# nju-websoft/OpenEA

Hardware: AMD Instinct MI355X
Metric: training triples/sec (k=10 truncated negatives + limited loss + Adagrad) (higher is better)
Workload: dtype f32; 1 GPU; BootEA/AlignE translational step, EN-FR-100K-V1 shape (synthetic), dim=100, GLOBAL batch=20000 positives (weak scaling: 20000 per GPU x 1 GPU), k=10, truncated eps=0.98; the same workload at every N (; global_batch=20000, entities=200000, parallelism=single

## Files before the change

### include/openea_hip.h

```cpp
#ifndef OPENEA_HIP_H
#define OPENEA_HIP_H

#include <stddef.h>
#include <stdint.h>

#ifdef __cplusplus
extern "C" {
#endif

#define OEA_OK 0
#define OEA_EINVAL (-1)
#define OEA_EHIP (-2)
#define OEA_ENOMEM (-3)
#define OEA_EUNSUPPORTED (-4)

int oea_version(void);
const char *oea_last_error(void);
int oea_device_count(void);

int oea_profile_begin(int32_t stride);
int oea_profile_end(int32_t group, double *out_ms_host, int32_t *n_calls_host);

typedef struct oea_store *oea_store_t;
int oea_store_create(int64_t rows, int32_t dim, oea_store_t *out);
// ... 6 lines not shown
int oea_store_save_host(oea_store_t s, float *dst_host, void *stream);

int oea_gather_rows(const float *table, int32_t dim, int32_t ld, const int32_t *ids, int64_t n,
                    int32_t normalize, float *out, int32_t out_ld, void *stream);
int oea_normalize_rows(float *table, int64_t rows, int32_t dim, int32_t ld, int32_t sk, void *stream);
int oea_fill_f32(float *p, int64_t n, float value, void *stream);
int oea_copy_to_host(const void *dev, void *host, size_t bytes, void *stream);
int oea_copy_from_host(void *dev, const void *host, size_t bytes, void *stream);

enum { OEA_LOSS_MARGIN = 0, OEA_LOSS_LIMITED = 1, OEA_LOSS_LOGISTIC = 2, OEA_LOSS_POSITIVE = 3,
       OEA_LOSS_ALIGN = 4 };
enum { OEA_OPT_SGD = 0, OEA_OPT_ADAGRAD = 1, OEA_OPT_ADAM = 2, OEA_OPT_ADADELTA = 3 };
enum { OEA_SCORE_TRANSE = 0, OEA_SCORE_TRANSH = 1, OEA_SCORE_TRANSD = 2 };

typedef struct oea_step_cfg {
    int32_t loss_kind;
    int32_t l1;
    float margin;
    float pos_margin;
    float neg_margin;
    float balance;
    int32_t ent_l2_norm;
    int32_t rel_l2_norm;
    int32_t opt_kind;
    float lr;
    int32_t neg_group_k;
    int32_t score_kind;
    float *normal;
    float *normal_acc;
    int32_t ent_transfer_base;
    int32_t rel_transfer_base;
    float beta1;
    float beta2;
    float eps;
    int32_t opt_t;
} oea_step_cfg;

size_t oea_step_workspace_bytes(int64_t n_ent, int64_t n_rel, int32_t ld);

int oea_triple_step(float *ent, float *ent_acc, int64_t n_ent, float *rel, float *rel_acc,
                    int64_t n_rel, int32_t dim, int32_t ld, const int32_t *pos, int64_t n_pos,
                    const int32_t *neg, int64_t n_neg, const oea_step_cfg *cfg, void *workspace,
                    double *loss_accum, void *stream);

enum { OEA_PHASE_BOTH = 0, OEA_PHASE_GRAD = 1, OEA_PHASE_APPLY = 2 };
size_t oea_step_exchange_floats(int64_t n_ent, int64_t n_rel, int32_t ld);
int32_t oea_step_scratch_elem_bytes(void);
int oea_triple_step_phase(float *ent, float *ent_acc, int64_t n_ent, float *rel, float *rel_acc,
                          int64_t n_rel, int32_t dim, int32_t ld, const int32_t *pos, int64_t n_pos,
                          const int32_t *neg, int64_t n_neg, const oea_step_cfg *cfg, void *workspace,
                          double *loss_accum, int32_t phase, void *stream);

int64_t oea_step_items(const oea_step_cfg *cfg, int64_t n_pos, int64_t n_neg);

int64_t oea_part_rows_per_rank(int64_t n_ent, int32_t world);
size_t oea_part_send_floats(int64_t n_ent, int32_t ld, int32_t world);
int oea_part_pack(void *workspace, int64_t n_ent, int64_t n_rel, int32_t ld, int32_t world, void *send, void *rel_x,
                  void *stream);
int oea_part_apply(float *ent, float *acc_own, int64_t n_ent, float *rel, float *rel_acc, int64_t n_rel, int32_t ld,
                   int32_t world, int32_t rank, void *own, void *rel_x, float *upd, const oea_step_cfg *cfg, void *workspace,
                   int64_t n_items, double *loss_accum, void *stream);
int oea_part_unpack(float *ent, int64_t n_ent, int32_t ld, int32_t world, int32_t rank, const float *all, void *stream);
int oea_step_normal_scratch(int64_t n_ent, int64_t n_rel, int32_t ld, int64_t *grad_offset_bytes, int64_t *touched_offset_bytes);
int oea_step_apply_normals(int64_t n_ent, int64_t n_rel, int32_t ld, const oea_step_cfg *cfg, void *workspace, void *stream);


int oea_step_scatter_ent_rows(void *workspace, int64_t n_ent, int64_t n_rel, int32_t ld, const int32_t *ids,
                              int64_t n, const float *src, int32_t src_ld, void *stream);

typedef struct oea_rotate_cfg {
    double gamma;
    double phase_scale;
    double lr;
    double beta1, beta2, eps;
    int64_t t;
    int32_t ent_l2_norm;
    int32_t rel_l2_norm;
    int32_t opt_kind;
    int32_t reserved;
} oea_rotate_cfg;
size_t oea_rotate_workspace_bytes(int64_t n_ent, int64_t n_rel, int32_t ld);
size_t oea_rotate_exchange_doubles(int64_t n_ent, int64_t n_rel, int32_t ld);
int oea_rotate_step(double *ent, double *ent_state, int64_t n_ent, double *rel, double *rel_state, int64_t n_rel,
                    int32_t dim, int32_t ld, const int32_t *pos, int64_t n_pos, const int32_t *neg, int64_t n_neg,
                    int32_t neg_group_k, const oea_rotate_cfg *cfg, void *workspace, double *loss_accum, int32_t phase,
                    void *stream);
int oea_rotate_lookup(const double *ent, int64_t n_ent, int32_t dim, int32_t ld, const int32_t *ids, int64_t n,
                      int32_t part_norm, int32_t sum_norm, float *out, int32_t out_ld, void *stream);

size_t oea_mapping_workspace_floats(int64_t n_links, int32_t ld, int32_t dim);
int oea_mapping_step(const float *ent, int32_t ld, int32_t dim, int32_t ent_l2_norm, const int32_t *ids1,
                     const int32_t *ids2, int64_t n, float *M, float *M_acc, float alpha, float lr, int32_t opt_kind,
                     void *ent_grad, void *ent_touched, float *work, double *loss_accum, void *stream);
int oea_mapping_epoch(float *ent, float *ent_acc, int64_t n_ent, float *rel, float *rel_acc, int64_t n_rel, int32_t dim,
                      int32_t ld, int32_t ent_l2_norm, const int32_t *batches, int32_t steps, int64_t n, float *M, float *M_acc,
                      float alpha, float lr, int32_t opt_kind, const oea_step_cfg *cfg, void *workspace, float *work,
                      double *mapping_loss_accum, double *step_loss_accum, void *stream);
size_t oea_sea_mapping_workspace_floats(int64_t n_l, int64_t n_u, int32_t ld, int32_t dim);
int oea_sea_mapping_step(const float *ent, int32_t ld, int32_t dim, const int32_t *ids_l1, const int32_t *ids_l2, int64_t n_l,
                         const int32_t *ids_u1, const int32_t *ids_u2, int64_t n_u, float *M1, float *M2, float *M_state,
                         float alpha_1, float alpha_2, const oea_step_cfg *cfg, void *ent_grad, void *ent_touched, float *work,
                         double *loss_accum, void *stream);
int oea_sea_mapping_epoch(float *ent, float *ent_acc, int64_t n_ent, float *rel, float *rel_acc, int64_t n_rel, int32_t dim,
                          int32_t ld, const int32_t *batches, int32_t steps, int64_t n_l, int64_t n_u, float *M1, float *M2,
                          float *M_state, float alpha_1, float alpha_2, const oea_step_cfg *cfg, void *workspace, float *work,
                          double *mapping_loss_accum, double *step_loss_accum, void *stream);
size_t oea_transr_workspace_bytes(int64_t n_ent, int64_t n_rel, int32_t dim, int64_t max_pos);
int oea_transr_step(float *ent, float *ent_acc, int64_t n_ent, float *rel, float *rel_acc, int64_t n_rel, float *rel_matrix,
                    float *rel_matrix_acc, int32_t dim, int32_t ld, const int32_t *pos, int64_t n_pos, const int32_t *neg,
                    int64_t n_neg, const oea_step_cfg *cfg, void *step_workspace, void *transr_workspace, double *loss_accum,
                    void *stream);
enum { OEA_SEMANTIC_HOLE = 0, OEA_SEMANTIC_SIMPLE = 1 };
int oea_semantic_step(int32_t model, float *ent, float *ent_acc, int64_t n_ent, float *rel, float *rel_acc, int64_t n_rel,
                      int32_t dim, int32_t ld, const int32_t *pos, int64_t n_pos, const int32_t *neg, int64_t n_neg,
                      const oea_step_cfg *cfg, void *step_workspace, double *loss_accum, void *stream);
int oea_step_entity_scratch(void *workspace, int64_t n_ent, int64_t n_rel, int32_t ld, void **ent_grad,
                            void **ent_touched);

uint64_t oea_tripleset_capacity(int64_t n);
int oea_tripleset_build(const int32_t *triples, int64_t n, uint64_t *table, uint64_t capacity,
                        void *stream);
int oea_sample_negatives(const int32_t *pos, int64_t n_pos, int32_t k, const uint64_t *table,
                         uint64_t capacity, const int32_t *entity_list, int32_t n_ent_list,
                         const int32_t *ent_pos, const int32_t *nbr, int32_t nbr_k, uint64_t seed,
                         uint32_t step, uint32_t pos_offset, int32_t max_try, int32_t *out,
                         int32_t *err_flag, void *stream);

int oea_sample_negatives_replay(const int32_t *pos, int64_t n_pos, int32_t k, const uint64_t *table, uint64_t capacity,
                                const int32_t *entity_list, int32_t n_ent_list, const int32_t *ent_pos, const int32_t *nbr,
                                int32_t nbr_k, int32_t max_try, const int32_t *replay, int32_t *out, int32_t *err_flag, void *stream);

typedef struct oea_sampler_side {
    const uint64_t *table;
    uint64_t capacity;
    const int32_t *entity_list;
    const int32_t *ent_pos;
    const int32_t *nbr;
    int32_t n_ent_list;
    int32_t nbr_k;
    const uint32_t *filter;
    uint64_t filter_bits;
} oea_sampler_side;
uint64_t oea_tripleset_filter_bits(uint64_t capacity);
int oea_tripleset_filter_build(const int32_t *triples, int64_t n, uint32_t *filter, uint64_t filter_bits, void *stream);
int oea_sample_negatives_pair(const int32_t *pos, int64_t n_pos, int64_t n_split, int32_t k,
                              const oea_sampler_side *side0, const oea_sampler_side *side1, uint64_t seed,
                              uint32_t step, uint32_t pos_offset, int32_t max_try, int32_t *out,
                              int32_t *err_flag, void *stream);

int oea_sample_negatives_epoch(const int32_t *pos_all, int64_t n_rows, const int64_t *offsets_dev,
                               const int64_t *splits_dev, int32_t steps, int32_t k, const oea_sampler_side *side0,
                               const oea_sampler_side *side1, uint64_t seed, uint32_t step_base, int32_t max_try,
                               int32_t *out_all, int32_t *err_flag, void *stream);

int oea_triple_epoch(float *ent, float *ent_acc, int64_t n_ent, float *rel, float *rel_acc, int64_t n_rel,
                     int32_t dim, int32_t ld, const int32_t *pos_all, const int64_t *offsets_host,
                     const int64_t *splits_host, int32_t steps, int32_t k, const oea_sampler_side *side0,
                     const oea_sampler_side *side1, uint64_t seed, uint32_t step_base, int32_t *neg_buf,
                     int32_t *err_flag, const oea_step_cfg *cfg, void *workspace, double *loss_accum,
                     const int64_t *offsets_dev, const int64_t *splits_dev, void *stream);
int oea_triple_epoch_range(float *ent, float *ent_acc, int64_t n_ent, float *rel, float *rel_acc, int64_t n_rel,
                           int32_t dim, int32_t ld, const int32_t *pos_all, const int64_t *offsets_host,
                           const int64_t *splits_host, int32_t steps, int32_t step_begin, int32_t step_end, int32_t k,
                           const oea_sampler_side *side0, const oea_sampler_side *side1, uint64_t seed,
                           uint32_t step_base, int32_t *neg_buf, int32_t *err_flag, const oea_step_cfg *cfg,
                           void *workspace, double *loss_accum, const int64_t *offsets_dev, const int64_t *splits_dev,
                           void *stream);

size_t oea_epoch_layout_bytes(int64_t n);
int oea_epoch_layout(const int32_t *triples, int64_t n1, int64_t n2, const int64_t *slot, int64_t n_slots, uint64_t seed, uint32_t epoch,
                     int32_t *dall, void *workspace, size_t ws_bytes, void *stream);

int32_t oea_step_plan_supported(const oea_step_cfg *cfg, int64_t n_ent, int64_t n_rel, int32_t ld, int32_t k);
size_t oea_step_plan_bytes(int64_t n_total, int32_t steps, int64_t max_batch, int64_t n_ent, int32_t ld);
int oea_step_plan_build(const int32_t *pos_all, const int32_t *neg_all, int32_t k, const int64_t *offsets_dev, int64_t n_total,
                        int32_t steps, int64_t max_batch, int64_t n_ent, int32_t ld, void *plan, size_t plan_bytes, void *stream);
int oea_step_plan_offsets(int64_t n_total, int32_t steps, int64_t max_batch, int64_t n_ent, int32_t ld, int64_t *out);
int oea_step_plan_rel_order_offset(int64_t n_total, int32_t steps, int64_t max_batch, int64_t n_ent, int32_t ld, int64_t *out);
int oea_triple_epoch_range_plan(float *ent, float *ent_acc, int64_t n_ent, float *rel, float *rel_acc, int64_t n_rel,
                                int32_t dim, int32_t ld, const int32_t *pos_all, const int64_t *offsets_host,
                                const int64_t *splits_host, int32_t steps, int32_t step_begin, int32_t step_end, int32_t k,
                                const oea_sampler_side *side0, const oea_sampler_side *side1, uint64_t seed,
                                uint32_t step_base, int32_t *neg_buf, int32_t *err_flag, const oea_step_cfg *cfg,
                                void *workspace, double *loss_accum, const int64_t *offsets_dev, const int64_t *splits_dev,
                                void *plan, size_t plan_bytes, int32_t plan_built, void *stream);

int oea_triple_epoch_range_shard(float *ent, float *ent_acc, int64_t n_ent, float *rel, float *rel_acc, int64_t n_rel,
                                 int32_t dim, int32_t ld, const int32_t *pos_all, const int64_t *offsets_host,
                                 const int64_t *splits_host, int32_t steps, int32_t step_begin, int32_t step_end, int32_t k,
                                 const oea_sampler_side *side0, const oea_sampler_side *side1, uint64_t seed,
                                 uint32_t step_base, int32_t *neg_buf, int32_t *err_flag, const oea_step_cfg *cfg,
                                 void *workspace, double *loss_accum, const int64_t *offsets_dev, const int64_t *splits_dev,
                                 int32_t rank, int32_t world, void *stream);

struct oea_comm;
int oea_triple_epoch_range_comm(struct oea_comm *comm, float *ent, float *acc_own, int64_t n_ent, float *rel, float *rel_acc,
                                int64_t n_rel, int32_t dim, int32_t ld, const int32_t *pos_all, const int64_t *offsets_host,
                                const int64_t *splits_host, int32_t steps, int32_t step_begin, int32_t step_end, int32_t k,
                                const oea_sampler_side *side0, const oea_sampler_side *side1, uint64_t seed, uint32_t step_base,
                                int32_t *neg_buf, int32_t *err_flag, const oea_step_cfg *cfg, void *workspace, double *loss_accum,
                                const int64_t *offsets_dev, const int64_t *splits_dev, void *send, void *own, void *rel_x,
                                float *upd, float *all, void *stream);


uint32_t oea_perm_index(uint32_t i, uint32_t n, uint32_t key);
int oea_sample_link_negatives(const int32_t *pos_links, int64_t n_pos, int32_t k, const int32_t *ents1, int32_t n1,
                              const int32_t *ents2, int32_t n2, const int32_t *nbr1, const int32_t *row1,
                              const int32_t *nbr2, const int32_t *row2, int32_t nbr_k, const uint64_t *exclude,
                              uint64_t exclude_cap, uint64_t seed, uint32_t step, int32_t *out_pairs, float *out_valid,
                              uint64_t *scratch_keys, int32_t *scratch_vals, uint64_t scratch_cap, void *stream);

int oea_greedy_matching(const int32_t *left, const int32_t *right, const float *weight, int64_t n_edges,
                        uint8_t *selected);
int oea_pair_dots(const float *e1, int32_t ld1, const float *e2, int32_t ld2, int32_t dim, const int32_t *ii,
                  const int32_t *jj, int64_t n, float *out, void *stream);

int oea_row_rank_select_f32(const float *vals, int64_t n_rows, int32_t nc, int64_t ld, int32_t k, int32_t largest, const int32_t *ids,
                            int64_t ld_ids, int32_t *out_sel, float *out_kth, void *stream);
int oea_row_rank_select_f64(const double *vals, int64_t n_rows, int32_t nc, int64_t ld, int32_t k, int32_t largest, const int32_t *ids,
                            int64_t ld_ids, int32_t *out_sel, double *out_kth, void *stream);

size_t oea_topk_workspace_bytes(int64_t nq, int64_t nc);
size_t oea_topk_sym_workspace_bytes(int64_t n, int32_t k);
int oea_topk_inner(const float *q, int64_t nq, int32_t ldq, const float *c, int64_t nc, int32_t ldc,
                   int32_t dim, int32_t k, const int32_t *id_map, int32_t *out_idx, void *workspace,
                   size_t ws_bytes, void *stream);

int oea_topk_rows(const float *s, int64_t n_rows, int64_t nc, int64_t ld, int32_t k, const int32_t *id_map,
                  int32_t *out_idx, void *stream);

enum { OEA_METRIC_INNER = 0, OEA_METRIC_MANHATTAN = 1, OEA_METRIC_EUCLIDEAN = 2,
       OEA_METRIC_MANHATTAN_F32 = 3  };
size_t oea_rank_workspace_bytes(int64_t n1);
int oea_rank_eval(const float *e1, int64_t n1, int32_t ld1, const float *e2, int64_t n2, int32_t ld2,
                  int32_t dim, int32_t metric, const float *csls_r, const float *csls_c, int64_t gold_offset,
                  int32_t *rank, int32_t *argmax, void *workspace, void *stream);
size_t oea_rank_eval_bf16_workspace_bytes(int64_t n1, int32_t dim);
int oea_rank_eval_bf16(const float *e1, int64_t n1, int32_t ld1, const float *e2, int64_t n2, int32_t ld2, int32_t dim,
                       int64_t gold_offset, int32_t *rank, int32_t *argmax, int32_t *status, void *workspace, void *stream);
int oea_rank_eval_bf16_csls(const float *e1, int64_t n1, int32_t ld1, const float *e2, int64_t n2, int32_t ld2, int32_t dim,
                            const float *csls_r, const float *csls_c, int64_t gold_offset, int32_t *rank, int32_t *argmax,
                            int32_t *status, void *workspace, void *stream);
int oea_rank_eval_metrics_bf16(const float *e1, int64_t n1, int32_t ld1, const float *e2, int64_t n2, int32_t ld2, int32_t dim,
                               const float *csls_r, const float *csls_c, int64_t gold_offset, const int32_t *top_k_host, int32_t nk,
                               int32_t *rank, int32_t *argmax, int64_t *out_dev, void *workspace, void *stream);
int oea_sim_bf16_matrix(const float *e1, int64_t n1, int32_t ld1, const float *e2, int64_t n2, int32_t ld2, int32_t dim, float *out,
                        int64_t ld_out, void *stream);
size_t oea_rank_eval_metrics_workspace_bytes(int64_t n1);
int oea_rank_eval_metrics(const float *e1, int64_t n1, int32_t ld1, const float *e2, int64_t n2, int32_t ld2, int32_t dim,
                          const float *csls_r, const float *csls_c, int64_t gold_offset, const int32_t *top_k_host, int32_t nk,
                          int32_t *rank, int32_t *argmax, int64_t *hits_and_rank_sum_dev, double *rr_sum_dev, void *workspace,
                          void *stream);
int oea_rank_metrics(const int32_t *rank, int64_t n, const int32_t *top_k_host, int32_t nk,
                     int64_t *hits_dev, int64_t *rank_sum_dev, double *rr_sum_dev, void *stream);

int oea_rank_rows(const float *s, int64_t n_rows, int64_t nc, int64_t ld, const int32_t *gold_idx,
                  int32_t *rank, int32_t *argmax, void *stream);

int oea_sim_matrix(const float *e1, int64_t n1, int32_t ld1, const float *e2, int64_t n2,
                   int32_t ld2, int32_t dim, int32_t metric, float *out, int64_t ld_out,
                   void *stream);
int oea_quantize_rows_u16(const float *src, int64_t n, int32_t ld, int32_t dim, float lo, float inv_step, uint16_t *dst,
                          int32_t ldq, void *stream);
int oea_l1_u16_strip(const uint16_t *q, int64_t nq, const uint16_t *c, int64_t nc, int32_t ldq, float *out, int64_t ld_out,
                     void *stream);
int oea_rank_l1_grid_rows(const float *strip, int64_t rows, int64_t row0, int64_t nc, int64_t ld, const float *e1, int32_t ld1,
                          const float *e2, int32_t ld2, int32_t dim, int64_t gold_offset, float step, float err, int32_t *rank,
                          int32_t *argmax, int32_t *n_exact_rows, void *stream);
int oea_rank_l1_grid_rows_csls(const float *strip, int64_t rows, int64_t row0, int64_t nc, int64_t ld, const float *e1, int32_t ld1,
                               const float *e2, int32_t ld2, int32_t dim, int64_t gold_offset, float step, float err,
                               const float *csls_r, const float *csls_c, int32_t *rank, int32_t *argmax, int32_t *n_exact_rows,
                               void *stream);
int oea_pair_l1_sim(const float *q, int64_t nq, int32_t ldq, const float *table, int64_t n, int32_t ldt, int32_t dim,
                    const int32_t *cand, int32_t c, float *out, void *stream);
int oea_pair_l1_f64(const float *q, int64_t nq, int32_t ldq, const float *table, int64_t n, int32_t ldt, int32_t dim,
                    const int32_t *cand, int32_t c, double *out, void *stream);

int oea_row_topk_mean(const float *s, int64_t n1, int64_t n2, int64_t ld, int32_t k, float *out,
                      void *stream);
size_t oea_csls_means_workspace_bytes(int64_t n1, int64_t n2, int32_t k);
int oea_csls_means(const float *e1, int64_t n1, int32_t ld1, const float *e2, int64_t n2, int32_t ld2, int32_t dim, int32_t k,
                   float *r_out, float *c_out, void *workspace, size_t ws_bytes, void *stream);
int oea_csls_apply(float *s, int64_t n1, int64_t n2, int64_t ld, const float *r, const float *c,
                   void *stream);

typedef struct oea_csr_split {
    const int32_t *chunk_row;
    const int32_t *chunk_e0;
    const int32_t *chunk_e1;
    const int32_t *rows;
    int32_t n_chunks, n_rows, threshold;
    const int32_t *row_chunk0;
    float *partials;
    int64_t partials_floats;
    uint32_t *tickets;
} oea_csr_split;
int oea_spmm_csr(const int32_t *rowptr, const int32_t *colidx, const float *vals, int64_t n_rows,
                 const float *x, int32_t dim, int32_t ldx, int32_t act, const float *mask_from,
                 float *y, int32_t ldy, const oea_csr_split *split, void *stream);

typedef struct oea_attn_graph {
    const int32_t *sub_ptr;
    const int32_t *sub_seg;
    const int32_t *seg_sub_ptr;
    const int32_t *seg_row;
    const int32_t *colidx;
    int64_t n_sub, n_seg, nnz;
    const int32_t *agg_rowptr;
    const int32_t *agg_colidx;
    const int32_t *agg_edge;
    int64_t agg_rows;
    const oea_csr_split *agg_split;
    const int32_t *t_rowptr;
    const int32_t *t_row;
    const int32_t *t_edge;
    int64_t t_rows;
    const oea_csr_split *t_split;
    int64_t sub0, sub1, seg0, seg1;
    int64_t agg_row0, agg_row1, agg_slot0, agg_slot1;
    int64_t t_row0, t_row1, t_slot0, t_slot1;
} oea_attn_graph;
#define OEA_ATTN_ALPHA 1
#define OEA_ATTN_AGGREGATE 2
#define OEA_ATTN_DZ 1
#define OEA_ATTN_DV 2
size_t oea_sparse_attn_workspace_floats(const oea_attn_graph *g);
int oea_sparse_attn_fwd(const oea_attn_graph *g, const float *z, const float *v, int32_t dim, int32_t ld,
                        float lrelu_slope, float *out, float *alpha, float *workspace, int32_t phases, void *stream);
int oea_sparse_attn_bwd(const oea_attn_graph *g, const float *z, const float *v, const float *alpha,
// ... 132 lines not shown
```

### openea_amd/_lib.py

```python
import ctypes as C
import os

_HERE = os.path.dirname(os.path.abspath(__file__))
DETERMINISTIC = os.environ.get("OEA_STEP_DETERMINISTIC", "0")[:1] == "1"
LIB_PATH = os.environ.get("OPENEA_HIP_LIB") or os.path.join(_HERE, "csrc",
                                                            "libopenea_hip_det.so" if DETERMINISTIC else "libopenea_hip.so")


class OpenEAHipError(RuntimeError):
    pass


class StepCfg(C.Structure):
    _fields_ = [("loss_kind", C.c_int32), ("l1", C.c_int32), ("margin", C.c_float),
                ("pos_margin", C.c_float), ("neg_margin", C.c_float), ("balance", C.c_float),
                ("ent_l2_norm", C.c_int32), ("rel_l2_norm", C.c_int32), ("opt_kind", C.c_int32),
                ("lr", C.c_float), ("neg_group_k", C.c_int32), ("score_kind", C.c_int32),
                ("normal", C.c_void_p), ("normal_acc", C.c_void_p),
                ("ent_transfer_base", C.c_int32), ("rel_transfer_base", C.c_int32),
                ("beta1", C.c_float), ("beta2", C.c_float), ("eps", C.c_float), ("opt_t", C.c_int32)]


class SamplerSide(C.Structure):
    _fields_ = [("table", C.c_void_p), ("capacity", C.c_uint64), ("entity_list", C.c_void_p),
                ("ent_pos", C.c_void_p), ("nbr", C.c_void_p), ("n_ent_list", C.c_int32), ("nbr_k", C.c_int32),
                ("filter", C.c_void_p), ("filter_bits", C.c_uint64)]


class CsrSplit(C.Structure):
    _fields_ = [("chunk_row", C.c_void_p), ("chunk_e0", C.c_void_p), ("chunk_e1", C.c_void_p), ("rows", C.c_void_p),
                ("n_chunks", C.c_int32), ("n_rows", C.c_int32), ("threshold", C.c_int32),
                ("row_chunk0", C.c_void_p), ("partials", C.c_void_p), ("partials_floats", C.c_int64), ("tickets", C.c_void_p)]


class AttnGraph(C.Structure):
    _fields_ = [("sub_ptr", C.c_void_p), ("sub_seg", C.c_void_p), ("seg_sub_ptr", C.c_void_p), ("seg_row", C.c_void_p),
                ("colidx", C.c_void_p), ("n_sub", C.c_int64), ("n_seg", C.c_int64), ("nnz", C.c_int64),
                ("agg_rowptr", C.c_void_p), ("agg_colidx", C.c_void_p), ("agg_edge", C.c_void_p), ("agg_rows", C.c_int64),
                ("agg_split", C.POINTER(CsrSplit)),
                ("t_rowptr", C.c_void_p), ("t_row", C.c_void_p), ("t_edge", C.c_void_p), ("t_rows", C.c_int64),
                ("t_split", C.POINTER(CsrSplit)),
                ("sub0", C.c_int64), ("sub1", C.c_int64), ("seg0", C.c_int64), ("seg1", C.c_int64),
                ("agg_row0", C.c_int64), ("agg_row1", C.c_int64), ("agg_slot0", C.c_int64), ("agg_slot1", C.c_int64),
                ("t_row0", C.c_int64), ("t_row1", C.c_int64), ("t_slot0", C.c_int64), ("t_slot1", C.c_int64)]


class GcnUnit(C.Structure):
    _fields_ = ([(pre + suf, t) for pre in ("a_", "at_", "f_", "ft_")
                 for suf, t in (("rowptr", C.c_void_p), ("colidx", C.c_void_p), ("vals", C.c_void_p), ("split", C.POINTER(CsrSplit)))]
                + [(nm, C.c_void_p) for nm in ("row_ids", "ill", "neg_left", "neg_right", "neg2_left", "neg2_right", "pair_rowptr",
                                               "pair_other", "pair_slot")]
                + [("n", C.c_int64), ("w_rows", C.c_int64), ("t", C.c_int64), ("dim", C.c_int32), ("ld", C.c_int32), ("k", C.c_int32),
                   ("gamma", C.c_float), ("lr", C.c_float)])


class GcnUnitBuffers(C.Structure):
    _fields_ = [(nm, C.c_void_p) for nm in ("t", "x", "h1", "out", "g_out", "g_pre1", "g_x", "g_t", "coef")]


class RotateCfg(C.Structure):
    _fields_ = [("gamma", C.c_double), ("phase_scale", C.c_double), ("lr", C.c_double), ("beta1", C.c_double),
                ("beta2", C.c_double), ("eps", C.c_double), ("t", C.c_int64), ("ent_l2_norm", C.c_int32),
                ("rel_l2_norm", C.c_int32), ("opt_kind", C.c_int32), ("reserved", C.c_int32)]


LOSS_KIND = {"margin-based": 0, "limited": 1, "logistic": 2, "positive": 3, "align": 4}
OPT_KIND = {"SGD": 0, "Adagrad": 1, "Adam": 2, "Adadelta": 3}
METRIC = {"inner": 0, "manhattan": 1, "euclidean": 2, "manhattan_f32": 3}

_vp, _i32, _i64, _u32, _u64, _f32, _sz = (C.c_void_p, C.c_int32, C.c_int64, C.c_uint32, C.c_uint64,
                                          C.c_float, C.c_size_t)

PROTOTYPES = {
    "oea_version": (C.c_int, []),
    "oea_last_error": (C.c_char_p, []),
    "oea_device_count": (C.c_int, []),
    "oea_profile_begin": (C.c_int, [_i32]),
    "oea_profile_end": (C.c_int, [_i32, C.POINTER(C.c_double), C.POINTER(_i32)]),
    "oea_store_create": (C.c_int, [_i64, _i32, C.POINTER(_vp)]),
    "oea_store_destroy": (C.c_int, [_vp]),
    "oea_store_rows": (_i64, [_vp]),
    "oea_store_dim": (_i32, [_vp]),
    "oea_store_ld": (_i32, [_vp]),
    "oea_store_rows_ptr": (_vp, [_vp]),
    "oea_store_load_host": (C.c_int, [_vp, _vp, _vp]),
    "oea_store_save_host": (C.c_int, [_vp, _vp, _vp]),
    "oea_gather_rows": (C.c_int, [_vp, _i32, _i32, _vp, _i64, _i32, _vp, _i32, _vp]),
    "oea_normalize_rows": (C.c_int, [_vp, _i64, _i32, _i32, _i32, _vp]),
    "oea_fill_f32": (C.c_int, [_vp, _i64, _f32, _vp]),
    "oea_copy_to_host": (C.c_int, [_vp, _vp, _sz, _vp]),
    "oea_copy_from_host": (C.c_int, [_vp, _vp, _sz, _vp]),
    "oea_step_workspace_bytes": (_sz, [_i64, _i64, _i32]),
    "oea_triple_step": (C.c_int, [_vp, _vp, _i64, _vp, _vp, _i64, _i32, _i32, _vp, _i64, _vp, _i64,
                                  C.POINTER(StepCfg), _vp, _vp, _vp]),
    "oea_step_exchange_floats": (_sz, [_i64, _i64, _i32]),
    "oea_step_scratch_elem_bytes": (_i32, []),
    "oea_triple_step_phase": (C.c_int, [_vp, _vp, _i64, _vp, _vp, _i64, _i32, _i32, _vp, _i64, _vp, _i64,
                                        C.POINTER(StepCfg), _vp, _vp, _i32, _vp]),
    "oea_part_rows_per_rank": (_i64, [_i64, _i32]),
    "oea_part_send_floats": (_sz, [_i64, _i32, _i32]),
    "oea_part_pack": (C.c_int, [_vp, _i64, _i64, _i32, _i32, _vp, _vp, _vp]),
    "oea_part_apply": (C.c_int, [_vp, _vp, _i64, _vp, _vp, _i64, _i32, _i32, _i32, _vp, _vp, _vp, C.POINTER(StepCfg), _vp, _i64,
                                 _vp, _vp]),
    "oea_step_normal_scratch": (C.c_int, [_i64, _i64, _i32, _vp, _vp]),
    "oea_step_apply_normals": (C.c_int, [_i64, _i64, _i32, _vp, _vp, _vp]),
    "oea_part_unpack": (C.c_int, [_vp, _i64, _i32, _i32, _i32, _vp, _vp]),
    "oea_step_scatter_ent_rows": (C.c_int, [_vp, _i64, _i64, _i32, _vp, _i64, _vp, _i32, _vp]),
    "oea_tripleset_capacity": (_u64, [_i64]),
    "oea_tripleset_build": (C.c_int, [_vp, _i64, _vp, _u64, _vp]),
    "oea_sample_negatives": (C.c_int, [_vp, _i64, _i32, _vp, _u64, _vp, _i32, _vp, _vp, _i32, _u64,
                                       _u32, _u32, _i32, _vp, _vp, _vp]),
    "oea_sample_negatives_replay": (C.c_int, [_vp, _i64, _i32, _vp, _u64, _vp, _i32, _vp, _vp, _i32, _i32, _vp, _vp, _vp, _vp]),
    "oea_tripleset_filter_bits": (C.c_uint64, [_u64]),
    "oea_tripleset_filter_build": (C.c_int, [_vp, _i64, _vp, _u64, _vp]),
    "oea_sample_negatives_pair": (C.c_int, [_vp, _i64, _i64, _i32, C.POINTER(SamplerSide), C.POINTER(SamplerSide),
                                            _u64, _u32, _u32, _i32, _vp, _vp, _vp]),
    "oea_sample_negatives_epoch": (C.c_int, [_vp, _i64, _vp, _vp, _i32, _i32, C.POINTER(SamplerSide),
                                             C.POINTER(SamplerSide), _u64, _u32, _i32, _vp, _vp, _vp]),
    "oea_triple_epoch": (C.c_int, [_vp, _vp, _i64, _vp, _vp, _i64, _i32, _i32, _vp, _vp, _vp, _i32, _i32,
                                   C.POINTER(SamplerSide), C.POINTER(SamplerSide), _u64, _u32, _vp, _vp,
                                   C.POINTER(StepCfg), _vp, _vp, _vp, _vp, _vp]),
    "oea_triple_epoch_range": (C.c_int, [_vp, _vp, _i64, _vp, _vp, _i64, _i32, _i32, _vp, _vp, _vp, _i32, _i32, _i32, _i32,
                                         C.POINTER(SamplerSide), C.POINTER(SamplerSide), _u64, _u32, _vp, _vp,
                                         C.POINTER(StepCfg), _vp, _vp, _vp, _vp, _vp]),
    "oea_triple_epoch_range_shard": (C.c_int, [_vp, _vp, _i64, _vp, _vp, _i64, _i32, _i32, _vp, _vp, _vp, _i32, _i32, _i32, _i32,
                                         C.POINTER(SamplerSide), C.POINTER(SamplerSide), _u64, _u32, _vp, _vp,
                                         C.POINTER(StepCfg), _vp, _vp, _vp, _vp, _i32, _i32, _vp]),
    "oea_epoch_layout_bytes": (_sz, [_i64]),
    "oea_epoch_layout": (C.c_int, [_vp, _i64, _i64, _vp, _i64, _u64, _u32, _vp, _vp, _sz, _vp]),
    "oea_step_plan_supported": (_i32, [C.POINTER(StepCfg), _i64, _i64, _i32, _i32]),
    "oea_step_plan_bytes": (_sz, [_i64, _i32, _i64, _i64, _i32]),
    "oea_step_plan_offsets": (C.c_int, [_i64, _i32, _i64, _i64, _i32, _vp]),
    "oea_step_plan_rel_order_offset": (C.c_int, [_i64, _i32, _i64, _i64, _i32, _vp]),
    "oea_step_plan_build": (C.c_int, [_vp, _vp, _i32, _vp, _i64, _i32, _i64, _i64, _i32, _vp, _sz, _vp]),
    "oea_triple_epoch_range_plan": (C.c_int, [_vp, _vp, _i64, _vp, _vp, _i64, _i32, _i32, _vp, _vp, _vp, _i32, _i32, _i32, _i32,
                                        C.POINTER(SamplerSide), C.POINTER(SamplerSide), _u64, _u32, _vp, _vp,
                                        C.POINTER(StepCfg), _vp, _vp, _vp, _vp, _vp, _sz, _i32, _vp]),
    "oea_triple_epoch_range_comm": (C.c_int, [_vp, _vp, _vp, _i64, _vp, _vp, _i64, _i32, _i32, _vp, _vp, _vp, _i32, _i32, _i32, _i32,
                                        C.POINTER(SamplerSide), C.POINTER(SamplerSide), _u64, _u32, _vp, _vp,
                                        C.POINTER(StepCfg), _vp, _vp, _vp, _vp, _vp, _vp, _vp, _vp, _vp, _vp]),
    "oea_rotate_workspace_bytes": (_sz, [_i64, _i64, _i32]),
    "oea_rotate_exchange_doubles": (_sz, [_i64, _i64, _i32]),
    "oea_rotate_step": (C.c_int, [_vp, _vp, _i64, _vp, _vp, _i64, _i32, _i32, _vp, _i64, _vp, _i64, _i32,
                                  C.POINTER(RotateCfg), _vp, _vp, _i32, _vp]),
    "oea_rotate_lookup": (C.c_int, [_vp, _i64, _i32, _i32, _vp, _i64, _i32, _i32, _vp, _i32, _vp]),
    "oea_mapping_workspace_floats": (_sz, [_i64, _i32, _i32]),
    "oea_mapping_step": (C.c_int, [_vp, _i32, _i32, _i32, _vp, _vp, _i64, _vp, _vp, C.c_float, C.c_float, _i32, _vp, _vp,
                                   _vp, _vp, _vp]),
    "oea_mapping_epoch": (C.c_int, [_vp, _vp, _i64, _vp, _vp, _i64, _i32, _i32, _i32, _vp, _i32, _i64, _vp, _vp, _f32, _f32, _i32,
                                    C.POINTER(StepCfg), _vp, _vp, _vp, _vp, _vp]),
    "oea_sea_mapping_workspace_floats": (_sz, [_i64, _i64, _i32, _i32]),
    "oea_sea_mapping_step": (C.c_int, [_vp, _i32, _i32, _vp, _vp, _i64, _vp, _vp, _i64, _vp, _vp, _vp, _f32, _f32, C.POINTER(StepCfg),
                                       _vp, _vp, _vp, _vp, _vp]),
    "oea_sea_mapping_epoch": (C.c_int, [_vp, _vp, _i64, _vp, _vp, _i64, _i32, _i32, _vp, _i32, _i64, _i64, _vp, _vp, _vp, _f32, _f32,
                                        C.POINTER(StepCfg), _vp, _vp, _vp, _vp, _vp]),
    "oea_step_entity_scratch": (C.c_int, [_vp, _i64, _i64, _i32, C.POINTER(C.c_void_p), C.POINTER(C.c_void_p)]),
    "oea_transr_workspace_bytes": (_sz, [_i64, _i64, _i32, _i64]),
    "oea_transr_step": (C.c_int, [_vp, _vp, _i64, _vp, _vp, _i64, _vp, _vp, _i32, _i32, _vp, _i64, _vp, _i64, C.POINTER(StepCfg),
                                  _vp, _vp, _vp, _vp]),
    "oea_semantic_step": (C.c_int, [_i32, _vp, _vp, _i64, _vp, _vp, _i64, _i32, _i32, _vp, _i64, _vp, _i64, C.POINTER(StepCfg),
                                    _vp, _vp, _vp]),
    "oea_greedy_matching": (C.c_int, [_vp, _vp, _vp, _i64, _vp]),
    "oea_pair_dots": (C.c_int, [_vp, _i32, _vp, _i32, _i32, _vp, _vp, _i64, _vp, _vp]),
    "oea_perm_index": (_u32, [_u32, _u32, _u32]),
    "oea_sample_link_negatives": (C.c_int, [_vp, _i64, _i32, _vp, _i32, _vp, _i32, _vp, _vp, _vp, _vp, _i32, _vp, _u64,
                                            _u64, _u32, _vp, _vp, _vp, _vp, _u64, _vp]),
    "oea_topk_sym_workspace_bytes": (_sz, [_i64, _i32]),
    "oea_topk_workspace_bytes": (_sz, [_i64, _i64]),
    "oea_topk_inner": (C.c_int, [_vp, _i64, _i32, _vp, _i64, _i32, _i32, _i32, _vp, _vp, _vp, _sz, _vp]),
    "oea_row_rank_select_f32": (C.c_int, [_vp, _i64, _i32, _i64, _i32, _i32, _vp, _i64, _vp, _vp, _vp]),
    "oea_row_rank_select_f64": (C.c_int, [_vp, _i64, _i32, _i64, _i32, _i32, _vp, _i64, _vp, _vp, _vp]),
    "oea_topk_rows": (C.c_int, [_vp, _i64, _i64, _i64, _i32, _vp, _vp, _vp]),
    "oea_rank_rows": (C.c_int, [_vp, _i64, _i64, _i64, _vp, _vp, _vp, _vp]),
    "oea_rank_workspace_bytes": (_sz, [_i64]),
    "oea_rank_eval": (C.c_int, [_vp, _i64, _i32, _vp, _i64, _i32, _i32, _i32, _vp, _vp, _i64, _vp, _vp, _vp, _vp]),
    "oea_quantize_rows_u16": (C.c_int, [_vp, _i64, _i32, _i32, C.c_float, C.c_float, _vp, _i32, _vp]),
    "oea_l1_u16_strip": (C.c_int, [_vp, _i64, _vp, _i64, _i32, _vp, _i64, _vp]),
    "oea_rank_l1_grid_rows": (C.c_int, [_vp, _i64, _i64, _i64, _i64, _vp, _i32, _vp, _i32, _i32, _i64, C.c_float, C.c_float, _vp, _vp, _vp, _vp]),
    "oea_pair_l1_f64": (C.c_int, [_vp, _i64, _i32, _vp, _i64, _i32, _i32, _vp, _i32, _vp, _vp]),
    "oea_rank_l1_grid_rows_csls": (C.c_int, [_vp, _i64, _i64, _i64, _i64, _vp, _i32, _vp, _i32, _i32, _i64, C.c_float, C.c_float, _vp, _vp,
                                             _vp, _vp, _vp, _vp]),
    "oea_pair_l1_sim": (C.c_int, [_vp, _i64, _i32, _vp, _i64, _i32, _i32, _vp, _i32, _vp, _vp]),
    "oea_rank_metrics": (C.c_int, [_vp, _i64, _vp, _i32, _vp, _vp, _vp, _vp]),
    "oea_rank_eval_bf16_workspace_bytes": (_sz, [_i64, _i32]),
    "oea_rank_eval_bf16": (C.c_int, [_vp, _i64, _i32, _vp, _i64, _i32, _i32, _i64, _vp, _vp, _vp, _vp, _vp]),
    "oea_rank_eval_bf16_csls": (C.c_int, [_vp, _i64, _i32, _vp, _i64, _i32, _i32, _vp, _vp, _i64, _vp, _vp, _vp, _vp, _vp]),
    "oea_sim_bf16_matrix": (C.c_int, [_vp, _i64, _i32, _vp, _i64, _i32, _i32, _vp, _i64, _vp]),
    "oea_rank_eval_metrics_bf16": (C.c_int, [_vp, _i64, _i32, _vp, _i64, _i32, _i32, _vp, _vp, _i64, _vp, _i32, _vp, _vp, _vp, _vp, _vp]),
    "oea_rank_eval_metrics_workspace_bytes": (_sz, [_i64]),
    "oea_rank_eval_metrics": (C.c_int, [_vp, _i64, _i32, _vp, _i64, _i32, _i32, _vp, _vp, _i64, _vp, _i32, _vp, _vp, _vp, _vp, _vp, _vp]),
    "oea_sim_matrix": (C.c_int, [_vp, _i64, _i32, _vp, _i64, _i32, _i32, _i32, _vp, _i64, _vp]),
    "oea_row_topk_mean": (C.c_int, [_vp, _i64, _i64, _i64, _i32, _vp, _vp]),
    "oea_csls_means_workspace_bytes": (_sz, [_i64, _i64, _i32]),
    "oea_csls_means": (C.c_int, [_vp, _i64, _i32, _vp, _i64, _i32, _i32, _i32, _vp, _vp, _vp, _sz, _vp]),
    "oea_csls_apply": (C.c_int, [_vp, _i64, _i64, _i64, _vp, _vp, _vp]),
    "oea_spmm_csr": (C.c_int, [_vp, _vp, _vp, _i64, _vp, _i32, _i32, _i32, _vp, _vp, _i32, C.POINTER(CsrSplit), _vp]),
    "oea_sparse_attn_workspace_floats": (_sz, [C.POINTER(AttnGraph)]),
    "oea_sparse_attn_fwd": (C.c_int, [C.POINTER(AttnGraph), _vp, _vp, _i32, _i32, _f32, _vp, _vp, _vp, _i32, _vp]),
    "oea_sparse_attn_bwd": (C.c_int, [C.POINTER(AttnGraph), _vp, _vp, _vp, _vp, _i32, _i32, _f32, _vp, _vp, _vp, _i32, _vp]),
    "oea_sparse_attn_dz": (C.c_int, [C.POINTER(AttnGraph), _vp, _vp, _vp, _f32, _vp, _vp]),
    "oea_concat_l2n_fwd": (C.c_int, [_vp, _vp, _vp, _i32, _i64, _vp, _i32, _vp, _vp, _vp]),
    "oea_concat_l2n_bwd": (C.c_int, [_vp, _vp, _vp, _i32, _i64, _vp, _vp, _i32, _vp, _vp, _vp]),
    "oea_pair_loss_l2_fwd": (C.c_int, [_vp, _i64, _i32, _i32, _vp, _i64, _i64, _vp, _f32, _f32, _vp, _vp, _vp]),
    "oea_pair_grad_rows": (C.c_int, [_vp, _i64, _i32, _i32, _vp, _vp, _vp, _vp, _vp, _i32, _vp, _vp]),
    "oea_align_loss_l1_coef": (C.c_int, [_vp, _i64, _i32, _i32, _vp, _i64, _i32, _f32, _vp, _vp, _vp, _vp, _vp, _vp, _vp, _vp]),
    "oea_segment_sum_f32": (C.c_int, [_vp, _vp, _vp, _i64, _vp, _vp]),
    "oea_pair_rows_build": (C.c_int, [_vp, _i64, _i64, _vp, _vp, _vp, _vp]),
    "oea_colsum_blocks": (_i32, [_i64]),
    "oea_highway_fwd": (C.c_int, [_vp, _vp, _vp, _vp, _vp, _i64, _i32, _vp, _vp]),
    "oea_highway_bwd": (C.c_int, [_vp, _vp, _vp, _vp, _vp, _vp, _vp, _i64, _i32, _vp, _vp, _vp, _vp, _vp]),
    "oea_gemm_tn_workspace_floats": (C.c_size_t, [_i64, _i32, _i32]),
    "oea_gemm_tn_f32": (C.c_int, [_vp, _i32, _i32, _vp, _i32, _i32, _i64, _vp, _i32, _vp, _vp]),
    "oea_gemm_tn_plan": (C.c_int, [_i64, _i32, _i32, C.POINTER(_i32), C.POINTER(_i64)]),
    "oea_gemm_tn_partial": (C.c_int, [_vp, _i32, _i32, _vp, _i32, _i32, _i64, _i32, _i32, _vp, _vp]),
    "oea_gemm_tn_reduce": (C.c_int, [_vp, _i32, _i32, _i32, _vp, _i32, _vp]),
    "oea_sigmoid_mix_fwd": (C.c_int, [_vp, _vp, _vp, _vp, _i64, _i32, _vp, _vp]),
    "oea_sigmoid_mix_bwd": (C.c_int, [_vp, _vp, _vp, _vp, _vp, _i64, _i32, _i32, _vp, _vp, _vp, _vp, _vp]),
    "oea_relu_axpy_fwd": (C.c_int, [_vp, _vp, C.c_float, _i64, _vp, _vp]),
    "oea_relu_axpy_bwd": (C.c_int, [_vp, _vp, C.c_float, _i64, _vp, _vp]),
    "oea_colsum_prod": (C.c_int, [_vp, _vp, _i64, _i32, _vp, _vp]),
    "oea_bias_tanh_fwd": (C.c_int, [_vp, _vp, _i64, _i32, _vp, _vp]),
    "oea_bias_tanh_bwd": (C.c_int, [_vp, _vp, _i64, _i32, _vp, _vp, _vp]),
    "oea_adam_dense": (C.c_int, [_vp, _vp, _vp, _vp, _i64, _f32, _f32, _f32, _f32, _i64, _vp]),
    "oea_align_loss_l1": (C.c_int, [_vp, _i64, _i32, _i32, _vp, _i64, _i32, _f32, _vp, _vp, _vp, _vp,
                                    _vp, _vp, _vp]),
    "oea_sgd_rows": (C.c_int, [_vp, _vp, _i64, _i32, _i32, _i32, _f32, _vp]),
    "oea_gcn_unit_epoch": (C.c_int, [C.POINTER(GcnUnit), _vp, C.POINTER(GcnUnitBuffers), _vp, _vp]),
    "oea_build_unweighted_adj": (C.c_int, [_vp, _i64, _i64, _vp, _vp, _vp, _i64, _vp, _vp]),
    "oea_build_weighted_adj": (C.c_int, [_vp, _i64, _i64, _i64, _vp, _vp, _vp, _vp, _vp, _vp, _vp, _vp, _vp, _i64, _vp, _vp]),
    "oea_build_primal_adj": (C.c_int, [_vp, _i64, _i64, _vp, _vp, _vp, _i64, _vp, _vp]),
    "oea_build_dual_adj": (C.c_int, [_vp, _i64, _i64, _vp, _vp]),
    "oea_build_2hop": (C.c_int, [_vp, _i64, _vp, _i64, _i64, _i64, _i32, _vp, _i64, _vp, C.POINTER(_i64), _vp]),
    "oea_comm_unique_id": (C.c_int, [_vp]),
    "oea_comm_init": (C.c_int, [_vp, _i32, _i32, C.POINTER(_vp)]),
    "oea_comm_destroy": (C.c_int, [_vp]),
    "oea_comm_rank": (_i32, [_vp]),
    "oea_comm_size": (_i32, [_vp]),
    "oea_allgather_rows": (C.c_int, [_vp, _vp, _vp, _i64, _i32, _vp]),
    "oea_comm_reduce_scatter_f32": (C.c_int, [_vp, _vp, _vp, _i64, _vp]),
    "oea_allreduce_f32": (C.c_int, [_vp, _vp, _i64, _vp]),
    "oea_allreduce_f64": (C.c_int, [_vp, _vp, _i64, _vp]),
    "oea_allreduce_i64": (C.c_int, [_vp, _vp, _i64, _vp]),
    "oea_comm_init_callbacks": (C.c_int, [_i32, _i32, _vp, _vp, C.POINTER(_vp)]),
    "oea_comm_allgather": (C.c_int, [_vp, _vp, _vp, _i64, _i32, _vp]),
    "oea_comm_reduce_scatter": (C.c_int, [_vp, _vp, _vp, _i64, _i32, _vp]),
    "oea_comm_allreduce": (C.c_int, [_vp, _vp, _i64, _i32, _vp]),
    "oea_step_items": (_i64, [C.POINTER(StepCfg), _i64, _i64]),
    "oea_comm_set_alltoallv": (C.c_int, [_vp, _vp]),
    "oea_comm_alltoallv": (C.c_int, [_vp, _vp, _vp, _vp, _vp, _vp, _vp, _i32, _vp]),
    "oea_halo_workspace_bytes": (_sz, [_i64, _i32, _i32, _i64, _i32]),
    "oea_halo_buffer_bytes": (_sz, [_i64, _i32, _i64, _i32, _i32]),
    "oea_halo_plan": (C.c_int, [_vp, _vp, _i32, _vp, _vp, _i32, _i32, _i32, _i64, _i32, _vp, _sz, _vp, _vp, C.POINTER(_i64), _vp]),
    "oea_triple_epoch_range_halo": (C.c_int, [_vp, _vp, _vp, _i64, _vp, _vp, _i64, _i32, _i32, _vp, _vp, _vp, _i32, _i32, _i32, _i32,
                                        C.POINTER(SamplerSide), C.POINTER(SamplerSide), _u64, _u32, _vp, _vp,
                                        C.POINTER(StepCfg), _vp, _vp, _vp, _vp, _vp, _sz, _vp, _vp, _sz, _vp, _vp, _vp, _vp, _vp]),
    "oea_comm_profile_begin": (C.c_int, [_vp]),
    "oea_comm_profile_end": (C.c_int, [_vp, C.POINTER(C.c_double), C.POINTER(_i32)]),
}

COMM_CALLBACK = C.CFUNCTYPE(C.c_int, _vp, _i32, _vp, _vp, _i64, _i32, _vp)
COMM_ALLTOALLV_CALLBACK = C.CFUNCTYPE(C.c_int, _vp, _vp, C.POINTER(_i64), C.POINTER(_i64), _vp, C.POINTER(_i64), C.POINTER(_i64), _i32, _vp)
COMM_ALLREDUCE, COMM_ALLGATHER, COMM_REDUCE_SCATTER = 0, 1, 2
COMM_F32, COMM_F64, COMM_I64 = 0, 1, 2
COMM_PHASES = ("grad", "pack", "reduce_scatter", "apply", "all_gather", "unpack")

_lib = None


def load(require_device=True):
    global _lib
    if _lib is None:
        if not os.path.exists(LIB_PATH):
            raise OpenEAHipError(
                "libopenea_hip.so not found at %s -- run `python -c 'import __graft_entry__ as g; "
                "g.build()'` (there is no CPU fallback)" % LIB_PATH)
        try:
            lib = C.CDLL(LIB_PATH)
        except OSError as e:
            raise OpenEAHipError("cannot load %s: %s" % (LIB_PATH, e))
        for name, (res, args) in PROTOTYPES.items():
            fn = getattr(lib, name)
            fn.restype = res
            fn.argtypes = args
        _lib = lib
    if require_device and _lib.oea_device_count() <= 0:
        raise OpenEAHipError("no HIP device visible: the OpenEA hot path runs on MI355X only "
                             "(there is no CPU fallback)")
# ... 8 lines not shown
```

### openea_amd/csrc/sampler.hip

```cpp
#include <stdlib.h>

#include <algorithm>

#include "common.h"

namespace {

__global__ void tripleset_clear(uint64_t *table, uint64_t capacity) {
    for (uint64_t i = (uint64_t)blockIdx.x * blockDim.x + threadIdx.x; i < capacity; i += (uint64_t)gridDim.x * blockDim.x)
        table[i] = OEA_EMPTY_KEY;
}

__global__ void tripleset_insert(const int32_t *__restrict__ triples, int64_t n, uint64_t *table, uint64_t capacity) {
    for (int64_t i = (int64_t)blockIdx.x * blockDim.x + threadIdx.x; i < n; i += (int64_t)gridDim.x * blockDim.x) {
        const uint64_t key = oea::pack_triple((uint32_t)triples[3 * i], (uint32_t)triples[3 * i + 1], (uint32_t)triples[3 * i + 2]);
        uint64_t s = oea::mix64(key) & (capacity - 1);
        for (;;) {
            const unsigned long long prev = atomicCAS((unsigned long long *)&table[s], (unsigned long long)OEA_EMPTY_KEY, (unsigned long long)key);
            if (prev == OEA_EMPTY_KEY || prev == key) break;
            s = (s + 1) & (capacity - 1);
        }
    }
}

__device__ __forceinline__ uint64_t filter_bit(uint64_t key, uint64_t bits) { return oea::mix64(key ^ 0x9E3779B97F4A7C15ull) & (bits - 1); }

__global__ void tripleset_filter_insert(const int32_t *__restrict__ triples, int64_t n, uint32_t *__restrict__ filter, uint64_t bits) {
    for (int64_t i = (int64_t)blockIdx.x * blockDim.x + threadIdx.x; i < n; i += (int64_t)gridDim.x * blockDim.x) {
        const uint64_t b = filter_bit(oea::pack_triple((uint32_t)triples[3 * i], (uint32_t)triples[3 * i + 1], (uint32_t)triples[3 * i + 2]), bits);
        atomicOr(&filter[b >> 5], 1u << (b & 31));
    }
}

__device__ __forceinline__ bool contains(const uint64_t *__restrict__ table, uint64_t capacity, const uint32_t *__restrict__ filter,
                                         uint64_t filter_bits, uint32_t h, uint32_t r, uint32_t t) {
    const uint64_t key = oea::pack_triple(h, r, t);
    if (filter) {
        const uint64_t b = filter_bit(key, filter_bits);
        if (!((filter[b >> 5] >> (b & 31)) & 1u)) return false;
    }
    uint64_t s = oea::mix64(key) & (capacity - 1);
    for (;;) {
        const uint64_t cur = table[s];
        if (cur == key) return true;
        if (cur == OEA_EMPTY_KEY) return false;
        s = (s + 1) & (capacity - 1);
    }
}

constexpr int kMaxK = 64;

template <int G>
__global__ __launch_bounds__(256) void sample_negatives_kernel(
    const int32_t *__restrict__ pos, int64_t n_pos, int64_t n_split, int k, oea_sampler_side side0,
    oea_sampler_side side1, uint32_t k0, uint32_t k1, uint32_t step, uint32_t pos_offset,
    int max_try, int32_t *__restrict__ out, int32_t *__restrict__ err_flag,
    const int64_t *__restrict__ seg_off, const int64_t *__restrict__ seg_split, int n_seg, const int32_t *__restrict__ replay) {
    const int lane = threadIdx.x % G;
    const uint32_t step_in = step;
    const int64_t n_split_in = n_split;
    for (int64_t p = ((int64_t)blockIdx.x * blockDim.x + threadIdx.x) / G; p < n_pos; p += (int64_t)gridDim.x * blockDim.x / G) {
    step = step_in;
    n_split = n_split_in;
    int64_t pl = p;
    if (seg_off) {
        const int64_t p0 = ((int64_t)(uint32_t)__builtin_amdgcn_readfirstlane((int)(p >> 32)) << 32) | (uint32_t)__builtin_amdgcn_readfirstlane((int)p);
        int lo = 0, hi = n_seg;
        while (hi - lo > 1) {
            const int mid = (lo + hi) >> 1;
            if (seg_off[mid] <= p0) lo = mid; else hi = mid;
        }
        int64_t first = seg_off[lo], split = seg_split[lo];
        int seg = lo;
        if (p >= seg_off[lo + 1]) {
            int l2 = lo;
            hi = n_seg;
            while (hi - l2 > 1) {
                const int mid = (l2 + hi) >> 1;
                if (seg_off[mid] <= p) l2 = mid; else hi = mid;
            }
            seg = l2; first = seg_off[l2]; split = seg_split[l2];
        }
        pl = p - first;
        n_split = split;
        step += (uint32_t)seg;
    }
    const oea_sampler_side &sd = pl < n_split ? side0 : side1;
    const uint64_t *__restrict__ table = sd.table;
    const uint64_t capacity = sd.capacity;
    const int32_t *__restrict__ entity_list = sd.entity_list;
    const int32_t *__restrict__ ent_pos = sd.ent_pos;
    const int32_t *__restrict__ nbr = sd.nbr;
    const uint32_t *__restrict__ filter = sd.filter;
    const uint64_t filter_bits = sd.filter_bits;
    const int n_ent_list = sd.n_ent_list, nbr_k = sd.nbr_k;
    const int32_t h = pos[3 * p], r = pos[3 * p + 1], t = pos[3 * p + 2];
    const bool h_has = nbr && ent_pos[h] >= 0, t_has = nbr && ent_pos[t] >= 0;
    const int32_t *hc = h_has ? nbr + (int64_t)ent_pos[h] * nbr_k : entity_list;
    const int32_t *tc = t_has ? nbr + (int64_t)ent_pos[t] * nbr_k : entity_list;
    const int hn = h_has ? nbr_k : n_ent_list, tn = t_has ? nbr_k : n_ent_list;
    const uint32_t c0 = (uint32_t)pl + pos_offset;
    const int gbase = (threadIdx.x & 63) / G * G;
    const unsigned long long gmask = (G == 64 ? ~0ull : ((1ull << G) - 1ull)) << gbase;
    int got = 0;
    for (int tr = 0; tr < max_try && got < k; ++tr) {
        const bool spare = k < G;
        uint4 w = oea::philox4x32_10(c0, step, (uint32_t)tr, (spare && lane != G - 1) ? 1u + (uint32_t)lane : 0u, k0, k1);
        const uint32_t side_word = spare ? (uint32_t)__shfl((int)w.x, (int)((threadIdx.x & 63) / G * G) + G - 1, 64) : w.x;
        const int32_t *rp = replay ? replay + ((int64_t)p * max_try + tr) * (1 + k) : nullptr;
        const bool corrupt_head = rp ? rp[0] != 0 : (side_word & 1u) != 0u;
        const int32_t *cand = corrupt_head ? hc : tc;
        const int nc = corrupt_head ? hn : tn;
        const int need = k - got;
        if (need > nc) { if (lane == 0) *err_flag = 1; break; }
        const bool active = lane < need;
        uint32_t att = 0;
        int32_t v = -1 - lane;
        if (active) {
            if (!spare) w = oea::philox4x32_10(c0, step, (uint32_t)tr, 1u + (uint32_t)lane, k0, k1);
            v = rp ? rp[1 + lane] : (int32_t)__umulhi(w.x, (uint32_t)nc);
            if (rp && (v < 0 || v >= nc)) { *err_flag = 2; v = 0; }
        }
        for (;;) {
            bool conflict = false;
            for (int q = 0; q < need; ++q) {
                const int32_t vq = __shfl(v, gbase + q, 64);
                conflict |= (q < lane) && (vq == v);
            }
            conflict &= active;
            if ((__ballot(conflict) & gmask) == 0ull) break;
            if (conflict) {
                ++att;
                w = oea::philox4x32_10(c0, step, (uint32_t)tr, 1u + (uint32_t)lane + 64u * att, k0, k1);
                v = (int32_t)__umulhi(w.x, (uint32_t)nc);
            }
        }
        bool accept = false;
        int32_t nh = h, nt = t;
        if (active) {
            const int32_t e = cand[v];
            nh = corrupt_head ? e : h;
            nt = corrupt_head ? t : e;
            accept = (tr == max_try - 1) || !contains(table, capacity, filter, filter_bits, (uint32_t)nh, (uint32_t)r, (uint32_t)nt);
        }
        const unsigned long long acc_mask = (__ballot(accept) & gmask) >> gbase;
        if (accept) {
            const int slot = got + __popcll(acc_mask & ((1ull << lane) - 1ull));
            struct __attribute__((packed, aligned(4))) Triple { int32_t h, r, t; };
            *reinterpret_cast<Triple *>(out + ((int64_t)p * k + slot) * 3) = Triple{nh, r, nt};
        }
        got += __popcll(acc_mask);
    }
    }
}

}

extern "C" {

uint64_t oea_tripleset_capacity(int64_t n) {
    uint64_t cap = 16;
    while (cap < 2ull * (uint64_t)(n > 1 ? n : 1)) cap *= 2;
    return cap;
}

int oea_tripleset_build(const int32_t *triples, int64_t n, uint64_t *table, uint64_t capacity, void *stream) {
    OEA_REQUIRE(table && (triples || n == 0), "null pointer");
    OEA_REQUIRE(capacity >= 2ull * (uint64_t)n && (capacity & (capacity - 1)) == 0, "capacity: power of two >= 2n");
    hipStream_t st = oea::as_stream(stream);
    tripleset_clear<<<1024, 256, 0, st>>>(table, capacity);
    if (n > 0) tripleset_insert<<<(unsigned)std::min<int64_t>(oea::ceil_div(n, 256), 4096), 256, 0, st>>>(triples, n, table, capacity);
    OEA_CHECK_HIP(hipGetLastError());
    return OEA_OK;
}

uint64_t oea_tripleset_filter_bits(uint64_t capacity) { return 8ull * capacity; }

int oea_tripleset_filter_build(const int32_t *triples, int64_t n, uint32_t *filter, uint64_t filter_bits, void *stream) {
    OEA_REQUIRE(filter && (triples || n == 0), "null pointer");
    OEA_REQUIRE(filter_bits >= 32 && (filter_bits & (filter_bits - 1)) == 0, "filter_bits: a power of two >= 32");
    hipStream_t st = oea::as_stream(stream);
    OEA_CHECK_HIP(hipMemsetAsync(filter, 0, (size_t)(filter_bits / 8), st));
    if (n > 0) tripleset_filter_insert<<<(unsigned)std::min<int64_t>(oea::ceil_div(n, 256), 4096), 256, 0, st>>>(triples, n, filter, filter_bits);
    OEA_CHECK_HIP(hipGetLastError());
    return OEA_OK;
}

int oea_sample_negatives(const int32_t *pos, int64_t n_pos, int32_t k, const uint64_t *table,
                         uint64_t capacity, const int32_t *entity_list, int32_t n_ent_list,
                         const int32_t *ent_pos, const int32_t *nbr, int32_t nbr_k, uint64_t seed,
                         uint32_t step, uint32_t pos_offset, int32_t max_try, int32_t *out,
                         int32_t *err_flag, void *stream) {
    oea_sampler_side sd{};
    sd.table = table; sd.capacity = capacity; sd.entity_list = entity_list; sd.ent_pos = ent_pos; sd.nbr = nbr;
    sd.n_ent_list = n_ent_list; sd.nbr_k = nbr_k;
    return oea_sample_negatives_pair(pos, n_pos, n_pos, k, &sd, &sd, seed, step, pos_offset, max_try, out, err_flag,
                                     stream);
}

static int check_side(const oea_sampler_side *s, int k) {
    OEA_REQUIRE(s && s->table && s->entity_list, "sampler side: null pointer");
    OEA_REQUIRE(s->nbr == nullptr || (s->ent_pos != nullptr && s->nbr_k > 0), "nbr needs ent_pos and nbr_k");
    OEA_REQUIRE((s->nbr ? s->nbr_k : s->n_ent_list) >= k && s->n_ent_list >= k, "Sample larger than population");
    return OEA_OK;
}

static int sample_impl(const int32_t *pos, int64_t n_pos, int64_t n_split, int32_t k,
                       const oea_sampler_side *side0, const oea_sampler_side *side1, uint64_t seed,
                       uint32_t step, uint32_t pos_offset, int32_t max_try, int32_t *out,
                       int32_t *err_flag, const int64_t *seg_off_dev, const int64_t *seg_split_dev, int n_seg,
                       void *stream, const int32_t *replay = nullptr) {
    OEA_REQUIRE(pos && out && err_flag, "null pointer");
    OEA_REQUIRE(k >= 1 && k <= kMaxK, "1 <= k <= 64");
    OEA_REQUIRE(max_try >= 1, "max_try >= 1");
    OEA_REQUIRE(n_split >= 0 && n_split <= n_pos, "0 <= n_split <= n_pos");
    int rc = check_side(side0, k);
    if (rc != OEA_OK) return rc;
    rc = check_side(side1, k);
    if (rc != OEA_OK) return rc;
    if (n_pos == 0) return OEA_OK;
    hipStream_t st = oea::as_stream(stream);
    static const int64_t cap_env = [] { const char *e = getenv("OEA_SAMPLER_CAP"); return e ? (int64_t)atoll(e) : (int64_t)0; }();
    const int64_t cap = (seg_off_dev && cap_env > 0) ? cap_env : ((int64_t)1 << 30);
    if (k <= 16)
        sample_negatives_kernel<16><<<(unsigned)std::min<int64_t>(oea::ceil_div(n_pos, 256 / 16), cap), 256, 0, st>>>(
            pos, n_pos, n_split, k, *side0, *side1, (uint32_t)seed, (uint32_t)(seed >> 32), step, pos_offset, max_try,
            out, err_flag, seg_off_dev, seg_split_dev, n_seg, replay);
    else
        sample_negatives_kernel<64><<<(unsigned)std::min<int64_t>(oea::ceil_div(n_pos, 256 / 64), cap), 256, 0, st>>>(
            pos, n_pos, n_split, k, *side0, *side1, (uint32_t)seed, (uint32_t)(seed >> 32), step, pos_offset, max_try,
            out, err_flag, seg_off_dev, seg_split_dev, n_seg, replay);
    OEA_CHECK_HIP(hipGetLastError());
    return OEA_OK;
}

int oea_sample_negatives_pair(const int32_t *pos, int64_t n_pos, int64_t n_split, int32_t k,
                              const oea_sampler_side *side0, const oea_sampler_side *side1, uint64_t seed,
                              uint32_t step, uint32_t pos_offset, int32_t max_try, int32_t *out,
                              int32_t *err_flag, void *stream) {
    return sample_impl(pos, n_pos, n_split, k, side0, side1, seed, step, pos_offset, max_try, out, err_flag, nullptr,
                       nullptr, 0, stream);
}

int oea_sample_negatives_replay(const int32_t *pos, int64_t n_pos, int32_t k, const uint64_t *table, uint64_t capacity,
                                const int32_t *entity_list, int32_t n_ent_list, const int32_t *ent_pos, const int32_t *nbr,
                                int32_t nbr_k, int32_t max_try, const int32_t *replay, int32_t *out, int32_t *err_flag, void *stream) {
    OEA_REQUIRE(replay, "replay record");
    oea_sampler_side sd{};
    sd.table = table; sd.capacity = capacity; sd.entity_list = entity_list; sd.ent_pos = ent_pos; sd.nbr = nbr;
    sd.n_ent_list = n_ent_list; sd.nbr_k = nbr_k;
    return sample_impl(pos, n_pos, n_pos, k, &sd, &sd, 0, 0u, 0u, max_try, out, err_flag, nullptr, nullptr, 0, stream, replay);
}

int oea_sample_negatives_epoch(const int32_t *pos_all, int64_t n_rows, const int64_t *offsets_dev,
                               const int64_t *splits_dev, int32_t steps, int32_t k, const oea_sampler_side *side0,
                               const oea_sampler_side *side1, uint64_t seed, uint32_t step_base, int32_t max_try,
                               int32_t *out_all, int32_t *err_flag, void *stream) {
    OEA_REQUIRE(offsets_dev && splits_dev && steps >= 1, "offsets / splits / steps");
    return sample_impl(pos_all, n_rows, 0, k, side0, side1, seed, step_base, 0u, max_try, out_all, err_flag, offsets_dev,
                       splits_dev, steps, stream);
}

}
```

### openea_amd/csrc/step_plan.h

```cpp
#pragma once
#include <hip/hip_runtime.h>
#include <stddef.h>
#include <stdint.h>

namespace oea {

struct StepPlanView {
    uint64_t *keys_a, *keys_b;
    uint32_t *vals_a, *vals_b;
    uint64_t *ukeys;
    uint32_t *ucount;
    uint32_t *uoff;
    int32_t *n_unique;
    int32_t *step_first;
    uint32_t *pflags;
    uint4 *recs;
    uint8_t *inplan;
    float *contrib;
    void *temp;
    size_t temp_bytes;
    uint32_t *rel_order;
    int row_bits;
};

constexpr uint32_t kPlanHubEntries = 8;

size_t step_plan_layout(int64_t n_total, int32_t steps, int64_t max_batch, int64_t n_ent, int32_t ld, void *base, StepPlanView *v);

}
```

### openea_amd/csrc/step_plan.hip

```cpp
#include <string.h>

#include <rocprim/rocprim.hpp>

#include <algorithm>

#include "common.h"
#include "step_plan.h"

namespace oea {

static size_t al256(size_t x) { return (x + 255) / 256 * 256; }
static int bits_for(uint64_t max_value) { int b = 1; while (b < 64 && (max_value >> b) != 0) ++b; return b; }

size_t step_plan_layout(int64_t n_total, int32_t steps, int64_t max_batch, int64_t n_ent, int32_t ld, void *base, StepPlanView *v) {
    const size_t m = (size_t)std::max<int64_t>(2 * n_total, 1);
    size_t off = 0;
    char *b = static_cast<char *>(base);
    auto take = [&](size_t bytes) { size_t o = off; off += al256(bytes); return b ? b + o : nullptr; };
    StepPlanView w{};
    w.keys_a = (uint64_t *)take(8 * m);
    w.keys_b = (uint64_t *)take(8 * m);
    w.vals_a = (uint32_t *)take(4 * m);
    w.vals_b = (uint32_t *)take(4 * m);
    w.ukeys = (uint64_t *)take(8 * m);
    w.ucount = (uint32_t *)take(4 * (m + 1));
    w.uoff = (uint32_t *)take(4 * (m + 1));
    w.n_unique = (int32_t *)take(4);
    w.step_first = (int32_t *)take(4 * ((size_t)steps + 1));
    w.pflags = (uint32_t *)take(4 * (size_t)std::max<int64_t>(n_total, 1));
    w.recs = (uint4 *)take(16 * m);
    w.inplan = (uint8_t *)take((size_t)std::max<int32_t>(steps, 1) * (size_t)n_ent);
    w.contrib = (float *)take(sizeof(float) * 2 * (size_t)std::max<int64_t>(max_batch, 1) * (size_t)ld);
    size_t t1 = 0, t2 = 0, t3 = 0;
    (void)rocprim::radix_sort_pairs(nullptr, t1, (const uint64_t *)nullptr, (uint64_t *)nullptr, (const uint32_t *)nullptr,
                                    (uint32_t *)nullptr, m, 0, 64, (hipStream_t)0);
    (void)rocprim::run_length_encode(nullptr, t2, (const uint64_t *)nullptr, m, (uint64_t *)nullptr, (uint32_t *)nullptr,
                                     (int32_t *)nullptr, (hipStream_t)0);
    (void)rocprim::exclusive_scan(nullptr, t3, (const uint32_t *)nullptr, (uint32_t *)nullptr, 0u, m + 1, rocprim::plus<uint32_t>(),
                                  (hipStream_t)0);
    const size_t n1 = (size_t)std::max<int64_t>(n_total, 1);
    w.temp_bytes = std::max(std::max(t1, std::max(t2, t3)), al256(4 * n1)) + 256;
    w.temp = take(w.temp_bytes);
    w.rel_order = (uint32_t *)take(4 * n1);
    w.row_bits = bits_for((uint64_t)std::max<int64_t>(n_ent - 1, 1));
    if (v) *v = w;
    return off;
}

namespace {

__global__ void plan_emit_kernel(const int32_t *__restrict__ pos_all, const int32_t *__restrict__ neg_all, int k,
                                 const int64_t *__restrict__ offsets, int steps, int64_t n_total, int row_bits,
                                 uint64_t *__restrict__ keys, uint32_t *__restrict__ vals) {
    const int64_t p = (int64_t)blockIdx.x * blockDim.x + threadIdx.x;
    if (p >= n_total) return;
    int lo = 0, hi = steps;
    while (hi - lo > 1) {
        const int mid = (lo + hi) >> 1;
        if (offsets[mid] <= p) lo = mid; else hi = mid;
    }
    const uint32_t pl = (uint32_t)(p - offsets[lo]);
    const int h = pos_all[3 * p], r = pos_all[3 * p + 1], t = pos_all[3 * p + 2];
    unsigned bad = 0, xh = 0, xt = 0;
    const int32_t *ng = neg_all + p * k * 3;
    for (int j = 0; j < k; ++j) {
        const unsigned a = (unsigned)(ng[3 * j] ^ h), b = (unsigned)(ng[3 * j + 2] ^ t), c = (unsigned)(ng[3 * j + 1] ^ r);
        bad |= c | min(a, b);
        xh |= a;
        xt |= b;
    }
    if (bad | min(xh, xt)) {
        keys[2 * p] = keys[2 * p + 1] = (uint64_t)steps << row_bits;
        vals[2 * p] = vals[2 * p + 1] = 0u;
        return;
    }
    const bool tails = xh == 0;
    const uint64_t sk = (uint64_t)lo << row_bits;
    keys[2 * p] = sk | (uint64_t)(uint32_t)h;
    vals[2 * p] = 2u * pl + (tails ? 0u : 1u);
    keys[2 * p + 1] = sk | (uint64_t)(uint32_t)t;
    vals[2 * p + 1] = 0x80000000u | (2u * pl + (tails ? 1u : 0u));
}

constexpr int kRelSortWaves = 8, kRelDigitBits = 10, kRelBins = 1 << kRelDigitBits, kRelAhead = 8;
__global__ __launch_bounds__(kRelSortWaves * 64) void plan_rel_order_kernel(const int32_t *__restrict__ pos_all, const int64_t *__restrict__ offsets,
                                                                            uint32_t *__restrict__ tmp, uint32_t *__restrict__ rel_order) {
    __shared__ uint32_t hist[kRelSortWaves][kRelBins];
    __shared__ uint32_t dbase[kRelBins];
    __shared__ uint32_t wsum[kRelSortWaves];
    __shared__ uint32_t rmax;
    const int64_t first = offsets[blockIdx.x];
    const uint32_t n = (uint32_t)(offsets[blockIdx.x + 1] - first);
    if (n == 0) return;
    const int32_t *rel = pos_all + 3 * first + 1;
    const uint32_t t = threadIdx.x, lane = t & 63u, w = t >> 6;
    const uint32_t slice = (n + kRelSortWaves - 1) / kRelSortWaves, c0 = min(w * slice, n), c1 = min(c0 + slice, n);
    const uint32_t groups = (c1 - c0 + 63u) / 64u;
    if (t == 0) rmax = 0u;
    int passes = 1;
    uint32_t *src = nullptr, *dst = nullptr;
    for (int pass = 0; pass < passes; ++pass) {
        const int shift = pass * kRelDigitBits;
        for (uint32_t i = t; i < kRelSortWaves * kRelBins; i += blockDim.x) (&hist[0][0])[i] = 0u;
        __syncthreads();
        uint32_t m = 0u;
        for (uint32_t g0 = 0; g0 < groups; g0 += kRelAhead) {
            uint32_t r[kRelAhead];
#pragma unroll
            for (int u = 0; u < kRelAhead; ++u) {
                const uint32_t i = c0 + (g0 + u) * 64u + lane;
                r[u] = i < c1 ? (uint32_t)rel[3 * (int64_t)(src ? src[i] : i)] : 0xffffffffu;
            }
#pragma unroll
            for (int u = 0; u < kRelAhead; ++u)
                if (c0 + (g0 + u) * 64u + lane < c1) {
                    m = max(m, r[u]);
                    atomicAdd(&hist[w][(r[u] >> shift) & (kRelBins - 1)], 1u);
                }
        }
        if (pass == 0) {
            for (int o = 32; o > 0; o >>= 1) m = max(m, (uint32_t)__shfl_xor((int)m, o));
            if (lane == 0) atomicMax(&rmax, m);
        }
        __syncthreads();
        if (pass == 0) {
            while (passes * kRelDigitBits < 32 && (rmax >> (passes * kRelDigitBits)) != 0u) ++passes;
            dst = (passes & 1) ? rel_order + first : tmp + first;
        }
        constexpr int DPT = kRelBins / (kRelSortWaves * 64);
        uint32_t tot[DPT], mine = 0u;
#pragma unroll
        for (int j = 0; j < DPT; ++j) {
            uint32_t run = 0u;
            for (int x = 0; x < kRelSortWaves; ++x) { const uint32_t c = hist[x][t * DPT + j]; hist[x][t * DPT + j] = run; run += c; }
            tot[j] = run;
            mine += run;
        }
        uint32_t inc = mine;
        for (int o = 1; o < 64; o <<= 1) { const uint32_t y = (uint32_t)__shfl_up((int)inc, o); if (lane >= (uint32_t)o) inc += y; }
        if (lane == 63u) wsum[w] = inc;
        __syncthreads();
        uint32_t before = inc - mine;
        for (uint32_t x = 0; x < w; ++x) before += wsum[x];
#pragma unroll
        for (int j = 0; j < DPT; ++j) { dbase[t * DPT + j] = before; before += tot[j]; }
        __syncthreads();
        for (uint32_t g0 = 0; g0 < groups; g0 += kRelAhead) {
            uint32_t idx[kRelAhead], dg[kRelAhead];
#pragma unroll
            for (int u = 0; u < kRelAhead; ++u) {
                const uint32_t i = c0 + (g0 + u) * 64u + lane;
                idx[u] = i < c1 ? (src ? src[i] : i) : 0u;
                dg[u] = i < c1 ? ((uint32_t)rel[3 * (int64_t)idx[u]] >> shift) & (kRelBins - 1) : 0u;
            }
#pragma unroll
            for (int u = 0; u < kRelAhead; ++u) {
                const bool on = c0 + (g0 + u) * 64u + lane < c1;
                const uint32_t d = dg[u];
                unsigned long long same = __ballot(on);
#pragma unroll
                for (int b = 0; b < kRelDigitBits; ++b) {
                    const unsigned long long has = __ballot(on && ((d >> b) & 1u));
                    same &= ((d >> b) & 1u) ? has : ~has;
                }
                if (on) {
                    const uint32_t rank = (uint32_t)__popcll(same & ((1ull << lane) - 1ull));
                    const uint32_t slot = hist[w][d] + dbase[d] + rank;
                    dst[slot] = idx[u];
                    __builtin_amdgcn_wave_barrier();
                    if (rank == 0u) hist[w][d] += (uint32_t)__popcll(same);
                }
                __builtin_amdgcn_wave_barrier();
            }
        }
        __threadfence_block();
        __syncthreads();
        src = dst;
        dst = (dst == tmp + first) ? rel_order + first : tmp + first;
    }
}

__global__ void plan_step_first_kernel(const uint64_t *__restrict__ ukeys, const int32_t *__restrict__ n_unique, int steps, int row_bits,
                                       int32_t *__restrict__ step_first) {
    const int s = blockIdx.x * blockDim.x + threadIdx.x;
    if (s > steps) return;
    const uint64_t key = (uint64_t)s << row_bits;
    int lo = 0, hi = *n_unique;
    while (lo < hi) {
        const int mid = (lo + hi) >> 1;
        if (ukeys[mid] < key) lo = mid + 1; else hi = mid;
    }
    step_first[s] = lo;
}

__global__ void plan_records_kernel(const uint64_t *__restrict__ ukeys, const uint32_t *__restrict__ uoff, const uint32_t *__restrict__ vals,
                                    const int32_t *__restrict__ n_unique, int steps, int row_bits, int64_t n_ent, uint4 *__restrict__ recs,
                                    uint8_t *__restrict__ inplan) {
    const int nu = *n_unique;
    for (int64_t i = (int64_t)blockIdx.x * blockDim.x + threadIdx.x; i < nu; i += (int64_t)gridDim.x * blockDim.x) {
        const uint64_t key = ukeys[i];
        const uint32_t row = (uint32_t)(key & (((uint64_t)1 << row_bits) - 1)), e0 = uoff[i], cnt = uoff[i + 1] - e0;
        recs[i] = make_uint4(row, e0, cnt, vals[e0]);
        const int64_t step = (int64_t)(key >> row_bits);
        if (step < steps && cnt <= kPlanHubEntries) inplan[step * n_ent + row] = 1;
    }
}

__global__ void plan_hub_kernel(const uint64_t *__restrict__ keys, const uint32_t *__restrict__ vals, int64_t m,
                                const int64_t *__restrict__ offsets, int steps, int row_bits, uint32_t *__restrict__ pflags) {
    const int64_t e = (int64_t)blockIdx.x * blockDim.x + threadIdx.x;
    if (e >= m) return;
    const uint64_t key = keys[e];
    const int64_t step = (int64_t)(key >> row_bits);
    if (step >= steps) return;
    int left = 0, right = 0;
    while (left < (int)kPlanHubEntries && e - left - 1 >= 0 && keys[e - left - 1] == key) ++left;
    while (left + right < (int)kPlanHubEntries && e + right + 1 < m && keys[e + right + 1] == key) ++right;
    if (left + right < (int)kPlanHubEntries) return;
    const uint32_t v = vals[e];
    atomicOr(&pflags[offsets[step] + ((v & 0x7fffffffu) >> 1)], (v >> 31) ? 2u : 1u);
}

__device__ __forceinline__ uint32_t mix32(uint32_t x) {
    x ^= x >> 16; x *= 0x7feb352du; x ^= x >> 15; x *= 0x846ca68bu; x ^= x >> 16;
    return x;
}
__device__ __forceinline__ uint32_t feistel_perm(uint32_t i, uint32_t n, int lbits, int rbits, const uint32_t (&key)[6]) {
    const uint32_t lmask = (1u << lbits) - 1u, rmask = (1u << rbits) - 1u;
    uint32_t x = i;
    do {
        uint32_t l = x >> rbits, r = x & rmask;
#pragma unroll
        for (int q = 0; q < 6; q += 2) {
            l = (l ^ mix32(r ^ key[q])) & lmask;
            r = (r ^ mix32(l ^ key[q + 1])) & rmask;
        }
        x = (l << rbits) | r;
    } while (x >= n);
    return x;
}
__global__ void layout_perm_kernel(const int32_t *__restrict__ triples, int64_t n1, int64_t n2, const int64_t *__restrict__ slot, int64_t n_slots,
                                   uint32_t k0, uint32_t k1, uint32_t epoch, int32_t *__restrict__ dall) {
    const int64_t j = (int64_t)blockIdx.x * blockDim.x + threadIdx.x;
    if (j >= n_slots) return;
    const int64_t sj = slot[j];
    const bool second = sj >= n1;
    const uint32_t n = (uint32_t)(second ? n2 : n1), i = (uint32_t)(second ? sj - n1 : sj);
    int bits = 1;
    while (bits < 32 && (1ull << bits) < (unsigned long long)n) ++bits;
    if (bits < 2) bits = 2;
    const int rbits = bits / 2, lbits = bits - rbits;
    const uint4 wa = philox4x32_10(epoch, second ? 1u : 0u, 0x5eedu, 0u, k0, k1), wb = philox4x32_10(epoch, second ? 1u : 0u, 0x5eedu, 1u, k0, k1);
    const uint32_t key[6] = {wa.x, wa.y, wa.z, wa.w, wb.x, wb.y};
    const int64_t src = (int64_t)feistel_perm(i, n, lbits, rbits, key) + (second ? n1 : 0);
    dall[3 * j] = triples[3 * src]; dall[3 * j + 1] = triples[3 * src + 1]; dall[3 * j + 2] = triples[3 * src + 2];
}

}
}

extern "C" {

size_t oea_step_plan_bytes(int64_t n_total, int32_t steps, int64_t max_batch, int64_t n_ent, int32_t ld) {
    if (n_total < 0 || steps < 0 || max_batch < 0 || n_ent <= 0 || ld <= 0) return 0;
    return oea::step_plan_layout(n_total, steps, max_batch, n_ent, ld, nullptr, nullptr);
}

int oea_step_plan_offsets(int64_t n_total, int32_t steps, int64_t max_batch, int64_t n_ent, int32_t ld, int64_t *out) {
    OEA_REQUIRE(out && n_total >= 0 && steps >= 0 && n_ent > 0 && ld > 0, "arguments");
    oea::StepPlanView v;
    char *base = reinterpret_cast<char *>(4096);
    const size_t total = oea::step_plan_layout(n_total, steps, max_batch, n_ent, ld, base, &v);
    out[0] = (char *)v.vals_b - base; out[1] = (char *)v.ukeys - base; out[2] = (char *)v.uoff - base;
    out[3] = (char *)v.n_unique - base; out[4] = (char *)v.step_first - base; out[5] = (char *)v.contrib - base;
    out[6] = v.row_bits; out[7] = (int64_t)total; out[8] = (char *)v.pflags - base;
    return OEA_OK;
}

int oea_step_plan_rel_order_offset(int64_t n_total, int32_t steps, int64_t max_batch, int64_t n_ent, int32_t ld, int64_t *out) {
    OEA_REQUIRE(out && n_total >= 0 && steps >= 0 && n_ent > 0 && ld > 0, "arguments");
    oea::StepPlanView v;
    char *base = reinterpret_cast<char *>(4096);
    (void)oea::step_plan_layout(n_total, steps, max_batch, n_ent, ld, base, &v);
    *out = (char *)v.rel_order - base;
    return OEA_OK;
}

size_t oea_epoch_layout_bytes(int64_t n) {
    return n < 0 ? 0 : 256;
}

int oea_epoch_layout(const int32_t *triples, int64_t n1, int64_t n2, const int64_t *slot, int64_t n_slots, uint64_t seed, uint32_t epoch,
                     int32_t *dall, void *workspace, size_t ws_bytes, void *stream) {
    OEA_REQUIRE(triples && (slot || n_slots == 0) && (dall || n_slots == 0), "null pointer");
    OEA_REQUIRE(n1 >= 0 && n2 >= 0 && n_slots >= 0 && n1 < ((int64_t)1 << 32) && n2 < ((int64_t)1 << 32), "sizes");
    (void)workspace; (void)ws_bytes;
    if (n1 + n2 == 0 || n_slots == 0) return OEA_OK;
    hipStream_t st = oea::as_stream(stream);
    oea::layout_perm_kernel<<<(unsigned)oea::ceil_div(n_slots, 256), 256, 0, st>>>(triples, n1, n2, slot, n_slots, (uint32_t)seed,
                                                                                   (uint32_t)(seed >> 32), epoch, dall);
    OEA_CHECK_HIP(hipGetLastError());
    return OEA_OK;
}

int oea_step_plan_build(const int32_t *pos_all, const int32_t *neg_all, int32_t k, const int64_t *offsets_dev, int64_t n_total,
                        int32_t steps, int64_t max_batch, int64_t n_ent, int32_t ld, void *plan, size_t plan_bytes, void *stream) {
    OEA_REQUIRE(pos_all && offsets_dev && plan && (neg_all || k == 0), "null pointer");
    OEA_REQUIRE(n_total >= 0 && steps >= 1 && k >= 0 && n_ent > 0 && ld > 0, "sizes");
    OEA_REQUIRE(2 * n_total < ((int64_t)1 << 31) && 2 * max_batch < ((int64_t)1 << 31), "entries and slots are 31-bit");
    oea::StepPlanView v;
    const size_t need = oea::step_plan_layout(n_total, steps, max_batch, n_ent, ld, plan, &v);
    OEA_REQUIRE(plan_bytes >= need, "plan workspace smaller than oea_step_plan_bytes");
    hipStream_t st = oea::as_stream(stream);
    const size_t m = (size_t)(2 * n_total);
    if (m == 0) {
        OEA_CHECK_HIP(hipMemsetAsync(v.n_unique, 0, sizeof(int32_t), st));
        OEA_CHECK_HIP(hipMemsetAsync(v.step_first, 0, sizeof(int32_t) * ((size_t)steps + 1), st));
        return OEA_OK;
    }
    oea::plan_rel_order_kernel<<<(unsigned)steps, oea::kRelSortWaves * 64, 0, st>>>(pos_all, offsets_dev, (uint32_t *)v.temp, v.rel_order);
    oea::plan_emit_kernel<<<(unsigned)oea::ceil_div(n_total, 256), 256, 0, st>>>(pos_all, neg_all, k, offsets_dev, steps, n_total, v.row_bits,
                                                                                 v.keys_a, v.vals_a);
    const int end_bit = std::min(64, v.row_bits + oea::bits_for((uint64_t)steps));
    size_t tb = v.temp_bytes;
    OEA_CHECK_HIP(rocprim::radix_sort_pairs(v.temp, tb, (const uint64_t *)v.keys_a, v.keys_b, (const uint32_t *)v.vals_a, v.vals_b, m, 0,
                                            (unsigned)end_bit, st));
    OEA_CHECK_HIP(hipMemsetAsync(v.ucount, 0, sizeof(uint32_t) * (m + 1), st));
    tb = v.temp_bytes;
    OEA_CHECK_HIP(rocprim::run_length_encode(v.temp, tb, (const uint64_t *)v.keys_b, m, v.ukeys, v.ucount, v.n_unique, st));
    tb = v.temp_bytes;
    OEA_CHECK_HIP(rocprim::exclusive_scan(v.temp, tb, (const uint32_t *)v.ucount, v.uoff, 0u, m + 1, rocprim::plus<uint32_t>(), st));
    oea::plan_step_first_kernel<<<(unsigned)oea::ceil_div(steps + 1, 256), 256, 0, st>>>(v.ukeys, v.n_unique, steps, v.row_bits, v.step_first);
    OEA_CHECK_HIP(hipMemsetAsync(v.pflags, 0, sizeof(uint32_t) * (size_t)n_total, st));
    OEA_CHECK_HIP(hipMemsetAsync(v.inplan, 0, (size_t)steps * (size_t)n_ent, st));
    oea::plan_records_kernel<<<(unsigned)std::min<int64_t>(oea::ceil_div((int64_t)m, 256), 4096), 256, 0, st>>>(
        v.ukeys, v.uoff, v.vals_b, v.n_unique, steps, v.row_bits, n_ent, v.recs, v.inplan);
    oea::plan_hub_kernel<<<(unsigned)oea::ceil_div((int64_t)m, 256), 256, 0, st>>>(v.keys_b, v.vals_b, (int64_t)m, offsets_dev, steps, v.row_bits,
                                                                                   v.pflags);
    OEA_CHECK_HIP(hipGetLastError());
    return OEA_OK;
}

}
```

### openea_amd/csrc/triple_step.hip

```cpp
#include <stdlib.h>

#include <algorithm>
#include <vector>

#include "common.h"
#include "step_plan.h"

namespace {

using oea::group_sum;

using oea::flag_t;
using oea::grad_t;

struct StepWs {
    grad_t *ent_grad, *rel_grad;
    grad_t *rel_extra;
    int64_t rel_copy_stride;
    flag_t *ent_touched, *rel_touched;
    grad_t *nrm_grad, *nrm_extra;
    flag_t *nrm_touched;
    double *partials;
    __device__ __forceinline__ grad_t *rel_copy(int64_t c) const {
        return c == 0 ? rel_grad : rel_extra + (c - 1) * rel_copy_stride;
// ... 2118 lines not shown
#define OEA_CALL(G, IT) apply_normal_rows<G, IT><<<(unsigned)std::max<int64_t>(oea::ceil_div(n_rel, 256 / G), 1), 256, 0, st>>>(n_rel, ld, *cfg, ws, 1);
    OEA_PART_DISPATCH(OEA_CALL)
#undef OEA_CALL
    OEA_CHECK_HIP(hipGetLastError());
    return OEA_OK;
}

int64_t oea_step_items(const oea_step_cfg *cfg, int64_t n_pos, int64_t n_neg) { return cfg ? step_items(*cfg, n_pos, n_neg) : -1; }


int oea_part_pack(void *workspace, int64_t n_ent, int64_t n_rel, int32_t ld, int32_t world, void *send_, void *rel_x_,
                  void *stream) {
    grad_t *send = static_cast<grad_t *>(send_), *rel_x = static_cast<grad_t *>(rel_x_);
    OEA_REQUIRE(workspace && send && rel_x && world >= 1 && ld % 4 == 0, "arguments");
    StepWs ws;
    ws_layout(n_ent, n_rel, ld, workspace, &ws);
    const int64_t rpr = oea_part_rows_per_rank(n_ent, world);
    hipStream_t st = oea::as_stream(stream);
#define OEA_CALL(G, IT)                                                                                                   \
    part_pack_kernel<G, IT><<<(unsigned)std::min<int64_t>(oea::ceil_div(world * rpr + n_rel, 256 / G), 16384), 256, 0, st>>>( \
        ws, n_ent, n_rel, ld, world, rpr, send, rel_x)
    OEA_PART_DISPATCH(OEA_CALL)
#undef OEA_CALL
    OEA_CHECK_HIP(hipGetLastError());
    return OEA_OK;
}

int oea_part_apply(float *ent, float *acc_own, int64_t n_ent, float *rel, float *rel_acc, int64_t n_rel, int32_t ld,
                   int32_t world, int32_t rank, void *own_, void *rel_x_, float *upd, const oea_step_cfg *cfg, void *workspace,
                   int64_t n_items, double *loss_accum, void *stream) {
    grad_t *own = static_cast<grad_t *>(own_), *rel_x = static_cast<grad_t *>(rel_x_);
    OEA_REQUIRE(ent && rel && own && rel_x && upd && cfg && workspace && loss_accum, "null pointer");
    OEA_REQUIRE(world >= 1 && rank >= 0 && rank < world && ld % 4 == 0, "world / rank / ld");
    OEA_REQUIRE(cfg->opt_kind == OEA_OPT_SGD || (cfg->opt_kind == OEA_OPT_ADAGRAD && acc_own && rel_acc), "SGD or Adagrad (+ state)");
    OEA_REQUIRE(cfg->score_kind >= OEA_SCORE_TRANSE && cfg->score_kind <= OEA_SCORE_TRANSD, "score_kind");
    StepWs ws;
    ws_layout(n_ent, n_rel, ld, workspace, &ws);
    const int64_t rpr = oea_part_rows_per_rank(n_ent, world);
    hipStream_t st = oea::as_stream(stream);
#define OEA_CALL(G, IT)                                                                                                       \
    {                                                                                                                         \
        const int gpb = 256 / G;                                                                                              \
             \
        const int grad_gpb = 256 / (ld <= 128 ? 32 : 64);                                                                     \
        const int n_part = n_items > 0 ? (int)std::min<int64_t>(std::max<int64_t>(oea::ceil_div(n_items, grad_gpb), 1), kMaxBlocks) : 0; \
         \
        oea::launch_timed(part_apply_kernel<G, IT>, (unsigned)std::min<int64_t>(std::max<int64_t>(oea::ceil_div(rpr + n_rel, gpb), 1), 16384), 256, st, \
            ent, acc_own, n_ent, rel, rel_acc, n_rel, ld, world, rank, rpr, own, rel_x, upd, *cfg, ws, n_part, loss_accum);   \
    }
    if (ld <= 128 && apply_g16(n_ent, n_rel, ld)) {
        const int it16 = (ld + 15) / 16;
        if (it16 <= 2) OEA_CALL(16, 2)
        else if (it16 <= 4) OEA_CALL(16, 4)
        else if (it16 == 5) OEA_CALL(16, 5)
        else if (it16 == 6) OEA_CALL(16, 6)
        else if (it16 == 7) OEA_CALL(16, 7)
        else OEA_CALL(16, 8)
    } else {
        OEA_PART_DISPATCH(OEA_CALL)
    }
#undef OEA_CALL
    OEA_CHECK_HIP(hipGetLastError());
    return OEA_OK;
}

int oea_part_unpack(float *ent, int64_t n_ent, int32_t ld, int32_t world, int32_t rank, const float *all, void *stream) {
    OEA_REQUIRE(ent && all && world >= 1 && rank >= 0 && rank < world && ld % 4 == 0, "arguments");
    if (world == 1) return OEA_OK;
    const int64_t rpr = oea_part_rows_per_rank(n_ent, world);
    part_unpack_kernel<<<(unsigned)std::min<int64_t>(oea::ceil_div(n_ent * (ld / 4), 256), 16384), 256, 0, oea::as_stream(stream)>>>(
        ent, n_ent, ld, world, rank, rpr, all);
    OEA_CHECK_HIP(hipGetLastError());
    return OEA_OK;
}

int oea_triple_epoch(float *ent, float *ent_acc, int64_t n_ent, float *rel, float *rel_acc, int64_t n_rel,
                     int32_t dim, int32_t ld, const int32_t *pos_all, const int64_t *offsets_host,
                     const int64_t *splits_host, int32_t steps, int32_t k, const oea_sampler_side *side0,
                     const oea_sampler_side *side1, uint64_t seed, uint32_t step_base, int32_t *neg_buf,
                     int32_t *err_flag, const oea_step_cfg *cfg, void *workspace, double *loss_accum,
                     const int64_t *offsets_dev, const int64_t *splits_dev, void *stream) {
    return oea_triple_epoch_range(ent, ent_acc, n_ent, rel, rel_acc, n_rel, dim, ld, pos_all, offsets_host, splits_host,
                                  steps, 0, steps, k, side0, side1, seed, step_base, neg_buf, err_flag, cfg, workspace,
                                  loss_accum, offsets_dev, splits_dev, stream);
}

int oea_triple_epoch_range(float *ent, float *ent_acc, int64_t n_ent, float *rel, float *rel_acc, int64_t n_rel,
                           int32_t dim, int32_t ld, const int32_t *pos_all, const int64_t *offsets_host,
                           const int64_t *splits_host, int32_t steps, int32_t step_begin, int32_t step_end, int32_t k,
                           const oea_sampler_side *side0, const oea_sampler_side *side1, uint64_t seed,
                           uint32_t step_base, int32_t *neg_buf, int32_t *err_flag, const oea_step_cfg *cfg,
                           void *workspace, double *loss_accum, const int64_t *offsets_dev, const int64_t *splits_dev,
                           void *stream) {
    return oea_triple_epoch_range_shard(ent, ent_acc, n_ent, rel, rel_acc, n_rel, dim, ld, pos_all, offsets_host, splits_host,
                                        steps, step_begin, step_end, k, side0, side1, seed, step_base, neg_buf, err_flag, cfg,
                                        workspace, loss_accum, offsets_dev, splits_dev, 0, 1, stream);
}

static int epoch_range_impl(float *ent, float *ent_acc, int64_t n_ent, float *rel, float *rel_acc, int64_t n_rel,
                            int32_t dim, int32_t ld, const int32_t *pos_all, const int64_t *offsets_host,
                            const int64_t *splits_host, int32_t steps, int32_t step_begin, int32_t step_end, int32_t k,
                            const oea_sampler_side *side0, const oea_sampler_side *side1, uint64_t seed,
                            uint32_t step_base, int32_t *neg_buf, int32_t *err_flag, const oea_step_cfg *cfg,
                            void *workspace, double *loss_accum, const int64_t *offsets_dev, const int64_t *splits_dev,
                            int32_t rank, int32_t world, void *plan, size_t plan_bytes, int32_t plan_built, void *stream);

int oea_triple_epoch_range_shard(float *ent, float *ent_acc, int64_t n_ent, float *rel, float *rel_acc, int64_t n_rel,
                                 int32_t dim, int32_t ld, const int32_t *pos_all, const int64_t *offsets_host,
                                 const int64_t *splits_host, int32_t steps, int32_t step_begin, int32_t step_end, int32_t k,
                                 const oea_sampler_side *side0, const oea_sampler_side *side1, uint64_t seed,
                                 uint32_t step_base, int32_t *neg_buf, int32_t *err_flag, const oea_step_cfg *cfg,
                                 void *workspace, double *loss_accum, const int64_t *offsets_dev, const int64_t *splits_dev,
                                 int32_t rank, int32_t world, void *stream) {
    return epoch_range_impl(ent, ent_acc, n_ent, rel, rel_acc, n_rel, dim, ld, pos_all, offsets_host, splits_host, steps, step_begin,
                            step_end, k, side0, side1, seed, step_base, neg_buf, err_flag, cfg, workspace, loss_accum, offsets_dev,
                            splits_dev, rank, world, nullptr, 0, 0, stream);
}

int32_t oea_step_plan_supported(const oea_step_cfg *cfg, int64_t n_ent, int64_t n_rel, int32_t ld, int32_t k) {
    static const int env = [] { const char *e = getenv("OEA_STEP_PLAN"); return e ? atoi(e) : 1; }();
    if (!cfg || env == 0 || oea::kDetScratch) return 0;
    if (env != 2 && !apply_g16(n_ent, n_rel, ld)) return 0;
    return wave_rule(*cfg, n_ent, n_rel, ld) && cfg->neg_group_k == k && (cfg->opt_kind == OEA_OPT_SGD || cfg->opt_kind == OEA_OPT_ADAGRAD);
}

int oea_triple_epoch_range_plan(float *ent, float *ent_acc, int64_t n_ent, float *rel, float *rel_acc, int64_t n_rel,
                                int32_t dim, int32_t ld, const int32_t *pos_all, const int64_t *offsets_host,
                                const int64_t *splits_host, int32_t steps, int32_t step_begin, int32_t step_end, int32_t k,
                                const oea_sampler_side *side0, const oea_sampler_side *side1, uint64_t seed,
                                uint32_t step_base, int32_t *neg_buf, int32_t *err_flag, const oea_step_cfg *cfg,
                                void *workspace, double *loss_accum, const int64_t *offsets_dev, const int64_t *splits_dev,
                                void *plan, size_t plan_bytes, int32_t plan_built, void *stream) {
    return epoch_range_impl(ent, ent_acc, n_ent, rel, rel_acc, n_rel, dim, ld, pos_all, offsets_host, splits_host, steps, step_begin,
                            step_end, k, side0, side1, seed, step_base, neg_buf, err_flag, cfg, workspace, loss_accum, offsets_dev,
                            splits_dev, 0, 1, plan, plan_bytes, plan_built, stream);
}

static int epoch_range_impl(float *ent, float *ent_acc, int64_t n_ent, float *rel, float *rel_acc, int64_t n_rel,
                            int32_t dim, int32_t ld, const int32_t *pos_all, const int64_t *offsets_host,
                            const int64_t *splits_host, int32_t steps, int32_t step_begin, int32_t step_end, int32_t k,
                            const oea_sampler_side *side0, const oea_sampler_side *side1, uint64_t seed,
                            uint32_t step_base, int32_t *neg_buf, int32_t *err_flag, const oea_step_cfg *cfg,
                            void *workspace, double *loss_accum, const int64_t *offsets_dev, const int64_t *splits_dev,
                            int32_t rank, int32_t world, void *plan, size_t plan_bytes, int32_t plan_built, void *stream) {
    OEA_REQUIRE(pos_all && offsets_host && splits_host && cfg, "null pointer");
    OEA_REQUIRE(steps >= 0 && k >= 0, "steps, k >= 0");
    OEA_REQUIRE(0 <= step_begin && step_begin <= step_end && step_end <= steps, "0 <= step_begin <= step_end <= steps");
    OEA_REQUIRE((offsets_dev == nullptr) == (splits_dev == nullptr), "offsets_dev and splits_dev go together");
    OEA_REQUIRE(world >= 1 && rank >= 0 && rank < world, "0 <= rank < world");
    const bool presampled = k > 0 && side0 == nullptr && side1 == nullptr && offsets_dev != nullptr;
    OEA_REQUIRE(k == 0 || (neg_buf && (presampled || (err_flag && side0 && side1))), "sampling needs neg_buf, err_flag and both sides");
    const bool ahead = k > 0 && offsets_dev != nullptr && steps > 0;
    const bool sample_all = ahead && !presampled && step_begin == 0;
    if (sample_all) {
        const int rc = oea_sample_negatives_epoch(pos_all, offsets_host[steps], offsets_dev, splits_dev, steps, k, side0,
                                                  side1, seed, step_base, 10, neg_buf, err_flag, stream);
        if (rc != OEA_OK) return rc;
    }
    oea::StepPlanView pv;
    const bool use_plan = plan && world == 1 && ahead && (presampled || sample_all) && oea_step_plan_supported(cfg, n_ent, n_rel, ld, k);
    if (use_plan) {
        int64_t max_batch = 0;
        for (int32_t s = 0; s < steps; ++s) max_batch = std::max(max_batch, offsets_host[s + 1] - offsets_host[s]);
        const size_t need = oea::step_plan_layout(offsets_host[steps], steps, max_batch, n_ent, ld, plan, &pv);
        OEA_REQUIRE(plan_bytes >= need, "plan workspace smaller than oea_step_plan_bytes");
        if (!plan_built) {
            const int rc = oea_step_plan_build(pos_all, neg_buf, k, offsets_dev, offsets_host[steps], steps, max_batch, n_ent, ld, plan,
                                               plan_bytes, stream);
            if (rc != OEA_OK) return rc;
        }
    }
    oea_step_cfg step_cfg = *cfg;
    for (int32_t s = step_begin; s < step_end; ++s) {
        const int64_t b0 = offsets_host[s], nb = offsets_host[s + 1] - b0;
        if (nb <= 0) continue;
        const int64_t r_lo = nb * rank / world, r_hi = nb * (rank + 1) / world;
        const int64_t lo = b0 + r_lo, n = r_hi - r_lo;
        int64_t split = splits_host[s] - r_lo;
        split = split < 0 ? 0 : (split > n ? n : split);
        const int32_t *pos = pos_all + 3 * lo;
        int32_t *negs = ahead ? neg_buf + 3 * lo * (int64_t)k : neg_buf;
        if (n > 0 && k > 0 && !presampled && !sample_all) {
            const int rc = oea_sample_negatives_pair(pos, n, split, k, side0, side1, seed, step_base + (uint32_t)s,
                                                     (uint32_t)r_lo, 10, negs, err_flag, stream);
            if (rc != OEA_OK) return rc;
        }
        if (n > 0) {
            const int rc = step_phase_impl(ent, ent_acc, n_ent, rel, rel_acc, n_rel, dim, ld, pos, n,
                                           k > 0 ? negs : nullptr, n * (int64_t)k, &step_cfg, workspace, loss_accum,
                                           OEA_PHASE_BOTH, stream, use_plan ? &pv : nullptr, s, lo);
            if (rc != OEA_OK) return rc;
        }
        ++step_cfg.opt_t;
    }
    return OEA_OK;
}

int oea_triple_epoch_range_comm(oea_comm_t comm, float *ent, float *acc_own, int64_t n_ent, float *rel, float *rel_acc,
                                int64_t n_rel, int32_t dim, int32_t ld, const int32_t *pos_all, const int64_t *offsets_host,
                                const int64_t *splits_host, int32_t steps, int32_t step_begin, int32_t step_end, int32_t k,
                                const oea_sampler_side *side0, const oea_sampler_side *side1, uint64_t seed, uint32_t step_base,
                                int32_t *neg_buf, int32_t *err_flag, const oea_step_cfg *cfg, void *workspace, double *loss_accum,
                                const int64_t *offsets_dev, const int64_t *splits_dev, void *send, void *own, void *rel_x,
                                float *upd, float *all, void *stream) {
    OEA_REQUIRE(comm && pos_all && offsets_host && splits_host && cfg && send && own && rel_x && upd && all, "null pointer");
    OEA_REQUIRE(steps >= 0 && k >= 0 && 0 <= step_begin && step_begin <= step_end && step_end <= steps, "step range");
    OEA_REQUIRE((offsets_dev == nullptr) == (splits_dev == nullptr), "offsets_dev and splits_dev go together");
    OEA_REQUIRE(cfg->opt_kind == OEA_OPT_SGD || cfg->opt_kind == OEA_OPT_ADAGRAD, "the partition runs SGD / Adagrad");
    const int32_t world = oea_comm_size(comm), rank = oea_comm_rank(comm);
    const bool presampled = k > 0 && side0 == nullptr && side1 == nullptr && offsets_dev != nullptr;
    OEA_REQUIRE(k == 0 || (neg_buf && (presampled || (err_flag && side0 && side1))), "sampling needs neg_buf, err_flag and both sides");
    const bool ahead = k > 0 && offsets_dev != nullptr && steps > 0;
    const bool sample_all = ahead && !presampled && step_begin == 0;
    if (sample_all) {
        const int rc = oea_sample_negatives_epoch(pos_all, offsets_host[steps], offsets_dev, splits_dev, steps, k, side0, side1, seed,
                                                  step_base, 10, neg_buf, err_flag, stream);
        if (rc != OEA_OK) return rc;
    }
    const int64_t rpr = oea_part_rows_per_rank(n_ent, world);
    const int64_t chunk = rpr * (ld + 1);
    const bool transh = cfg->score_kind == OEA_SCORE_TRANSH;
    void *nrm_grad = nullptr, *nrm_touched = nullptr;
    if (transh) {
        int64_t g_off = 0, t_off = 0;
        int rc = oea_step_normal_scratch(n_ent, n_rel, ld, &g_off, &t_off);
        if (rc != OEA_OK) return rc;
        nrm_grad = static_cast<char *>(workspace) + g_off;
        nrm_touched = static_cast<char *>(workspace) + t_off;
    }
    const int32_t gdt = oea::kDetScratch ? OEA_COMM_I64 : OEA_COMM_F32;
    hipStream_t st = oea::as_stream(stream);
    oea_step_cfg step_cfg = *cfg;
#define OEA_TRY_RC(call) do { const int _rc = (call); if (_rc != OEA_OK) return _rc; } while (0)
    for (int32_t s = step_begin; s < step_end; ++s) {
        const int64_t b0 = offsets_host[s], nb = offsets_host[s + 1] - b0;
        if (nb <= 0) continue;
        const int64_t r_lo = nb * rank / world, r_hi = nb * (rank + 1) / world;
        const int64_t lo = b0 + r_lo, n = r_hi - r_lo;
        int64_t split = splits_host[s] - r_lo;
        split = split < 0 ? 0 : (split > n ? n : split);
        const int32_t *pos = pos_all + 3 * lo;
        int32_t *negs = ahead ? neg_buf + 3 * lo * (int64_t)k : neg_buf;
        if (n > 0 && k > 0 && !presampled && !sample_all)
            OEA_TRY_RC(oea_sample_negatives_pair(pos, n, split, k, side0, side1, seed, step_base + (uint32_t)s, (uint32_t)r_lo, 10, negs,
                                                 err_flag, stream));
        OEA_TRY_RC(oea::comm_phase_mark(comm, st));
        OEA_TRY_RC(oea_triple_step_phase(ent, nullptr, n_ent, rel, rel_acc, n_rel, dim, ld, pos, n, k > 0 ? negs : nullptr, n * (int64_t)k,
                                         &step_cfg, workspace, loss_accum, OEA_PHASE_GRAD, stream));
        OEA_TRY_RC(oea::comm_phase_mark(comm, st));
        OEA_TRY_RC(oea_part_pack(workspace, n_ent, n_rel, ld, world, send, rel_x, stream));
        OEA_TRY_RC(oea::comm_phase_mark(comm, st));
        OEA_TRY_RC(oea_comm_reduce_scatter(comm, send, own, chunk, gdt, stream));
        OEA_TRY_RC(oea_comm_allreduce(comm, rel_x, n_rel * (int64_t)(ld + 1), gdt, stream));
        if (transh) {
            OEA_TRY_RC(oea_comm_allreduce(comm, nrm_grad, n_rel * (int64_t)ld, gdt, stream));
            OEA_TRY_RC(oea_comm_allreduce(comm, nrm_touched, n_rel, gdt, stream));
        }
        OEA_TRY_RC(oea::comm_phase_mark(comm, st));
        const int64_t n_items = step_items(step_cfg, n, n * (int64_t)k);
        OEA_TRY_RC(oea_part_apply(ent, acc_own, n_ent, rel, rel_acc, n_rel, ld, world, rank, own, rel_x, upd, &step_cfg, workspace, n_items,
                                  loss_accum, stream));
        if (transh) OEA_TRY_RC(oea_step_apply_normals(n_ent, n_rel, ld, &step_cfg, workspace, stream));
        OEA_TRY_RC(oea::comm_phase_mark(comm, st));
        OEA_TRY_RC(oea_allgather_rows(comm, upd, all, rpr, ld, stream));
        OEA_TRY_RC(oea::comm_phase_mark(comm, st));
        OEA_TRY_RC(oea_part_unpack(ent, n_ent, ld, world, rank, all, stream));
        OEA_TRY_RC(oea::comm_phase_mark(comm, st));
        ++step_cfg.opt_t;
    }
#undef OEA_TRY_RC
    return OEA_OK;
}

}

static HaloGeom halo_geom(int64_t n_ent, int32_t world, int32_t rank, int64_t max_batch, int32_t k) {
    HaloGeom g;
    g.world = world; g.rank = rank;
    g.rpr = oea_part_rows_per_rank(n_ent, world);
    g.rpr32 = (g.rpr + 31) / 32 * 32;
    g.nwords = (int)((int64_t)world * g.rpr32 / 32);
    const int64_t share = oea::ceil_div(max_batch, world) + 1;
    g.cap = std::min<int64_t>(2 * share * (1 + (int64_t)k), (int64_t)world * g.rpr);
    g.cap = (g.cap + 3) / 4 * 4;
    return g;
}
struct HaloWs { uint32_t *bitmaps; int32_t *lists, *counts, *tables, *err; };
static size_t halo_ws_layout(const HaloGeom &g, int32_t steps, void *base, HaloWs *ws) {
    size_t off = 0;
    char *b = static_cast<char *>(base);
    auto take = [&](size_t bytes) { size_t o = off; off += align256(bytes); return b ? b + o : nullptr; };
    uint32_t *bm = (uint32_t *)take(4 * (size_t)steps * g.world * g.nwords);
    int32_t *li = (int32_t *)take(4 * (size_t)steps * g.world * g.cap);
    int32_t *co = (int32_t *)take(4 * (size_t)steps * g.world * g.world);
    int32_t *ta = (int32_t *)take(4 * (size_t)steps * 4 * (g.world + 1));
    int32_t *er = (int32_t *)take(256);
    if (ws) { ws->bitmaps = bm; ws->lists = li; ws->counts = co; ws->tables = ta; ws->err = er; }
    return off;
}

extern "C" {

size_t oea_halo_workspace_bytes(int64_t n_ent, int32_t world, int32_t steps, int64_t max_batch, int32_t k) {
    if (world < 1 || steps < 0) return 0;
    return halo_ws_layout(halo_geom(n_ent, world, 0, max_batch, k), steps, nullptr, nullptr);
}

size_t oea_halo_buffer_bytes(int64_t n_ent, int32_t world, int64_t max_batch, int32_t k, int32_t ld) {
    if (world < 1) return 0;
    const HaloGeom g = halo_geom(n_ent, world, 0, max_batch, k);
    const int64_t rows = std::max<int64_t>(g.cap, (int64_t)(world - 1) * std::min<int64_t>(g.cap, g.rpr));
    return align256((size_t)rows * (ld + 1) * sizeof(grad_t));
}

int oea_halo_plan(const int32_t *pos_all, const int32_t *neg_all, int32_t k, const int64_t *offsets_host, const int64_t *offsets_dev,
                  int32_t steps, int32_t step_begin, int32_t step_end, int64_t n_ent, int32_t world, void *halo_ws, size_t halo_ws_bytes,
                  int32_t *counts_host, int32_t *lists_host, int64_t *cap_out, void *stream) {
    OEA_REQUIRE(pos_all && offsets_host && offsets_dev && halo_ws && counts_host, "null pointer");
    OEA_REQUIRE(steps >= 0 && k >= 0 && (k == 0 || neg_all) && 0 <= step_begin && step_begin <= step_end && step_end <= steps && world >= 1, "arguments");
    hipStream_t st = oea::as_stream(stream);
    const int32_t nS = step_end - step_begin;
// ... 214 lines not shown
```

### openea_amd/models/trainer.py

```python
import os

import numpy as np
import torch

from .. import ops
from ..modules.train.batch import EpochBatches, TripleSampler, neighbours_device


class EmbeddingTable:

    def __init__(self, host_init, is_l2_norm, name, dev=None, visible_rows=None):
        host_init = np.asarray(host_init, np.float32)
        self.name = name
        self.rows, self.dim = host_init.shape
        self.visible_rows = self.rows if visible_rows is None else int(visible_rows)
        self.is_l2_norm = bool(is_l2_norm)
        self.var = ops.to_table(host_init, dev=dev)
        self.ld = self.var.shape[1]

    def lookup(self, ids):
        if not hasattr(ids, "is_cuda"):
            ids = ops.to_ids(np.asarray(ids, np.int32), self.var.device)
        return ops.gather_rows(self.var, self.dim, ids, normalize=self.is_l2_norm)

# ... 293 lines not shown
        self._epoch_negs_ready = False
        self._plan_ready = False

    def batch(self, step):
        if getattr(self, "_prefetch", None) is not None and self.in_epoch == 0:
            self._take_prefetch(torch.cuda.current_stream())
        pos, n_split = self.batches.pos(step)
        off = 0
        if self.world > 1:
            from .dist import shard_batch
            lo, hi, n_split = shard_batch(pos.shape[0], n_split, self.rank, self.world)
            pos, off = pos[lo:hi], lo
        neg = None
        if self.k > 0 and pos.shape[0] > 0:
            if self._sides is None:
                self._sides = (self.s1.side(), self.s2.side())
            neg = self.neg_buf[: pos.shape[0] * self.k]
            ops.sample_negatives_pair(pos, n_split, self.k, self._sides[0], self._sides[1], self.seed,
                                      self.global_step, off, neg, self.err)
        self.global_step += 1
        return pos, neg

    def run_epoch(self, trainer):
        assert self.in_epoch == 0, "run_epoch in the middle of an epoch: use run_steps"
        return self.run_steps(trainer, len(self.batches.splits))

    @property
    def in_epoch(self):
        return self.global_step - self._epoch_base

    def run_steps(self, trainer, n_steps):
        S = len(self.batches.splits)
        n = done = 0
        while done < n_steps:
            lo = self.in_epoch
            hi = min(S, lo + n_steps - done)
            n += self._run_range(trainer, lo, hi)
            done += hi - lo
        return n

    def _run_range(self, trainer, lo, hi):
        S = len(self.batches.splits)
        b = self.batches
        local = self.world > 1 and getattr(trainer, "local_epochs", False)
        c_part = getattr(trainer, "comm", None) is not None and getattr(trainer, "part", None) is not None
        if local and lo == 0:
            trainer.epoch_begin()
        if (self.world == 1 or local or c_part) and getattr(trainer, "fused_epoch", True):
            if self._sides is None:
                self._sides = (self.s1.side(), self.s2.side())
            main = torch.cuda.current_stream()
            if lo == 0:
                self._epoch_negs_ready = self._take_prefetch(main)
            if self.k:
                self._epoch_neg_buf()
            ev_start = None
            if lo == 0:
                ev_start = torch.cuda.Event()
                ev_start.record(main)
            have = self.k and self._epoch_negs_ready
            if hasattr(trainer, "count_steps"):
                trainer.count_steps(int((np.diff(b.offsets[lo:hi + 1]) > 0).sum()))
            halo_ok = (not self.k) or have or lo == 0
            if c_part and getattr(trainer, "exchange", None) == "halo" and halo_ok:
                halo = trainer.halo_buffers(S, int(np.diff(b.offsets).max()), self.k)
                if getattr(self, "_off_dev", None) is None:
                    self._off_dev = torch.from_numpy(b.offsets).to(self.dev)
                    self._spl_dev = torch.from_numpy(b.splits).to(self.dev)
                st = ops.triple_epoch_halo(trainer.comm.handle, trainer.ent.var, trainer.part['acc_own'], trainer.rel.var, trainer.rel_acc,
                                           trainer.ent.dim, b.dall, b.offsets, b.splits, self.k,
                                           None if (have or not self.k) else self._sides[0],
                                           None if (have or not self.k) else self._sides[1], self.seed, self._epoch_base,
                                           self._neg_all if self.k else None, self.err if self.k else None, trainer.cfg,
                                           trainer.ws, trainer.loss, self._off_dev, self._spl_dev, trainer.part, halo, step_range=(lo, hi))
                trainer.halo_stats = [trainer.halo_stats[0] + st[0], trainer.halo_stats[1] + st[1], max(trainer.halo_stats[2], st[2]),
                                      trainer.halo_stats[3] + st[3]]
            elif c_part:
                ops.triple_epoch_comm(trainer.comm.handle, trainer.ent.var, trainer.part['acc_own'], trainer.rel.var, trainer.rel_acc,
                                      trainer.ent.dim, b.dall, b.offsets, b.splits, self.k,
                                      None if (have or not self.k) else self._sides[0],
                                      None if (have or not self.k) else self._sides[1], self.seed, self._epoch_base,
                                      self._neg_all if self.k else None, self.err if self.k else None, trainer.cfg,
                                      trainer.ws, trainer.loss, self._off_dev if self.k else None,
                                      self._spl_dev if self.k else None, trainer.part, step_range=(lo, hi))
            else:
                plan = None
                if self.world == 1 and not local and self.k and self._plan_wanted(trainer):
                    plan = (self._plan, self._plan_ready and bool(have))
                ops.triple_epoch(trainer.ent.var, trainer.ent_acc, trainer.rel.var, trainer.rel_acc, trainer.ent.dim,
                                 b.dall, b.offsets, b.splits, self.k,
                                 None if (have or not self.k) else self._sides[0],
                                 None if (have or not self.k) else self._sides[1], self.seed, self._epoch_base,
                                 self._neg_all if self.k else None, self.err if self.k else None, trainer.cfg,
                                 trainer.ws, trainer.loss, self._off_dev if self.k else None,
                                 self._spl_dev if self.k else None, step_range=(lo, hi),
                                 shard=(self.rank, self.world) if local else (0, 1), plan=plan)
                if plan is not None and (have or lo == 0):
                    self._plan_ready = True
            if lo == 0 and self.k:
                self._epoch_negs_ready = True
            self.global_step += hi - lo
            n = int(b.offsets[hi] - b.offsets[lo])
            if local or (c_part and self.world > 1):
                nb = np.diff(b.offsets[lo:hi + 1])
                n = int((nb * (self.rank + 1) // self.world - nb * self.rank // self.world).sum())
            if ev_start is not None:
                self._prefetch_next(ev_start, trainer)
            if hi == S:
                self._epoch_base = self.global_step
                if local:
                    trainer.epoch_sync()
            return n
        n = 0
        for step in range(lo, hi):
            pos, neg = self.batch(step)
            if pos.shape[0] or trainer.dist is not None:
                trainer.step(pos, neg)
            n += pos.shape[0]
        if hi == S:
            self.end_epoch()
        return n

    def _epoch_neg_buf(self):
        b = self.batches
        if getattr(self, "_neg_all", None) is None:
            self._neg_all = torch.empty((int(b.offsets[-1]) * self.k, 3), dtype=torch.int32, device=self.dev)
            self._off_dev = torch.from_numpy(b.offsets).to(self.dev)
            self._spl_dev = torch.from_numpy(b.splits).to(self.dev)
        return self._neg_all

    def _plan_wanted(self, trainer):
        ent, rel = trainer.ent, trainer.rel
        if not ops.step_plan_supported(trainer.cfg, ent.rows, rel.rows, ent.ld, self.k):
            return False
        key = (ent.rows, ent.ld)
        if self._plan is None or self._plan_key != key:
            b = self.batches
            mb = int(np.diff(b.offsets).max()) if len(b.splits) else 0
            self._plan_dims = (int(b.offsets[-1]), len(b.splits), mb, ent.rows, ent.ld)
            self._plan = ops.step_plan_buffer(*self._plan_dims, dev=self.dev)
            self._plan_next = ops.step_plan_buffer(*self._plan_dims, dev=self.dev)
            self._plan_key, self._plan_ready = key, False
        return True

    def _prefetch_next(self, ev_start, trainer=None):
        if getattr(self, "_side", None) is None:
            self._side = torch.cuda.Stream(device=self.dev)
            self._neg_next = torch.empty_like(self._neg_all) if self.k else None
        side = self._side
        next_base = self._epoch_base + len(self.batches.splits)
        side.wait_event(ev_start)
        with torch.cuda.stream(side):
            self.batches.shuffle(self.gen, into_next=True)
            if self.k:
                ops.sample_negatives_epoch(self.batches.dall_next, self._off_dev, self._spl_dev, len(self.batches.splits), self.k,
                                           self._sides[0], self._sides[1], self.seed, next_base, self._neg_next, self.err)
            planned = False
            if (self.k and trainer is not None and self.world == 1 and not getattr(trainer, "local_epochs", False)
                    and getattr(trainer, "part", None) is None and self._plan_wanted(trainer)):
                n_total, steps, mb, n_ent, ld = self._plan_dims
                ops.step_plan_build(self.batches.dall_next, self._neg_next, self.k, self._off_dev, n_total, steps, mb, n_ent, ld,
                                    self._plan_next)
                planned = True
            self._prefetch_ev = torch.cuda.Event()
            self._prefetch_ev.record(side)
        self._prefetch = (self._sides, next_base, planned)

    def _take_prefetch(self, main):
        pf = getattr(self, "_prefetch", None)
        if pf is None:
            return False
        self._prefetch = None
        main.wait_event(self._prefetch_ev)
        self.batches.swap()
        ok = self.k > 0 and pf[0] is self._sides and pf[1] == self._epoch_base
        if ok:
            self._neg_all, self._neg_next = self._neg_next, self._neg_all
        self._plan_ready = bool(ok and len(pf) > 2 and pf[2])
        if self._plan_ready:
            self._plan, self._plan_next = self._plan_next, self._plan
        return ok

    def end_epoch(self):
        self._epoch_base = self.global_step
        self._epoch_negs_ready = False
        self._plan_ready = False
        if getattr(self, "_prefetch", None) is not None:
            self._take_prefetch(torch.cuda.current_stream())
            return
        self.batches.shuffle(self.gen)

    def check(self):
        torch.cuda.synchronize(self.dev)
        if int(self.err.item()) != 0:
            raise ValueError("Sample larger than population or is negative")


_IDS_CACHE = {}


def _entity_ids_on_device(entity_list, device):
    n = len(entity_list)
    key = (id(entity_list), str(device))
    ends = (n, int(entity_list[0]), int(entity_list[n // 2]), int(entity_list[-1])) if n else (0,)
    hit = _IDS_CACHE.get(key)
    if hit is not None and hit[0] is entity_list and hit[1] == ends:
        return hit[2]
    ids = ops.to_ids(np.asarray(entity_list, np.int32), device)
    if len(_IDS_CACHE) > 16:
        _IDS_CACHE.clear()
    _IDS_CACHE[key] = (entity_list, ends, ids)
    return ids


def refresh_is_sharded(n, k, world_size):
    if world_size <= 1:
        return False
    mode = os.environ.get("OEA_REFRESH_MODE", "")
    if mode in ("shard", "replicate"):
        return mode == "shard"
    if n < 12288:
        return True
    scale = (n / 1.0e5) ** 2
    sharded_ms = 16.0 * scale / world_size + 4.0 * n * k * (world_size - 1) / world_size / 300.0e6
    return sharded_ms < 10.3 * scale


def refresh_neighbours(ent, entity_list, k):
    ids = _entity_ids_on_device(entity_list, ent.var.device)
    emb = ent.lookup(ids)
    from . import dist as mdist
    if refresh_is_sharded(emb.shape[0], k, mdist.world()[1]):
        return mdist.sharded_neighbours(emb, ent.dim, ids, k,
                                        lambda q, cand, d, kk, id_map: ops.topk_inner(q.contiguous(), cand, d, kk, id_map=id_map))
    return neighbours_device(emb, ent.dim, ids, k)
```

### openea_amd/ops.py

```python
import ctypes as C
import os

import numpy as np
import torch

from . import _lib
from ._lib import LOSS_KIND, METRIC, OPT_KIND, OpenEAHipError, RotateCfg, StepCfg, check


def lib():
    return _lib.load(require_device=True)


def _p(t):
    if t is None:
        return None
    assert t.is_cuda and t.is_contiguous(), "device-resident contiguous tensor required"
    return C.c_void_p(t.data_ptr())


def _stream():
    return C.c_void_p(torch.cuda.current_stream().cuda_stream)


# ... 202 lines not shown
    return work


TRANSR_MAX_DIM = 128


def transr_workspace(n_ent, n_rel, dim, max_pos, dev=None):
    return torch.empty(lib().oea_transr_workspace_bytes(n_ent, n_rel, dim, max_pos), dtype=torch.uint8, device=dev or device())


def transr_step(ent, ent_acc, rel, rel_acc, rel_matrix, rel_matrix_acc, dim, pos, neg, cfg, workspace, transr_ws, loss_accum):
    assert rel_matrix.shape == (rel.shape[0], dim * dim) and rel_matrix.dtype == torch.float32
    n_neg = 0 if neg is None else neg.shape[0]
    check(lib().oea_transr_step(_p(ent), _p(ent_acc), ent.shape[0], _p(rel), _p(rel_acc), rel.shape[0], _p(rel_matrix),
                                _p(rel_matrix_acc), dim, ent.shape[1], _p(pos), pos.shape[0], _p(neg), n_neg, C.byref(cfg),
                                _p(workspace), _p(transr_ws), _p(loss_accum), _stream()))


SEMANTIC_HOLE, SEMANTIC_SIMPLE = 0, 1
SEMANTIC_MAX_DIM = 128


def semantic_step(model, ent, ent_acc, rel, rel_acc, dim, pos, neg, cfg, workspace, loss_accum):
    n_neg = 0 if neg is None else neg.shape[0]
    check(lib().oea_semantic_step(int(model), _p(ent), _p(ent_acc), ent.shape[0], _p(rel), _p(rel_acc), rel.shape[0], dim,
                                  ent.shape[1], _p(pos), pos.shape[0], _p(neg), n_neg, C.byref(cfg), _p(workspace),
                                  _p(loss_accum), _stream()))


def part_rows_per_rank(n_ent, world):
    return int(lib().oea_part_rows_per_rank(int(n_ent), int(world)))


def part_pack(workspace, n_ent, n_rel, ld, world, send, rel_x):
    check(lib().oea_part_pack(_p(workspace), n_ent, n_rel, ld, world, _p(send), _p(rel_x), _stream()))


def part_apply(ent, acc_own, rel, rel_acc, world, rank, own, rel_x, upd, cfg, workspace, n_items, loss_accum):
    check(lib().oea_part_apply(_p(ent), _p(acc_own), ent.shape[0], _p(rel), _p(rel_acc), rel.shape[0], ent.shape[1], world, rank,
                               _p(own), _p(rel_x), _p(upd), C.byref(cfg), _p(workspace), int(n_items), _p(loss_accum), _stream()))


def part_unpack(ent, world, rank, all_rows):
    check(lib().oea_part_unpack(_p(ent), ent.shape[0], ent.shape[1], world, rank, _p(all_rows), _stream()))


def step_exchange_view(workspace, n_ent, n_rel, ld):
    n = lib().oea_step_exchange_floats(n_ent, n_rel, ld)
    dt = scratch_dtype()
    return workspace[: dt.itemsize * n].view(dt)


def step_entity_flags(workspace, n_ent, n_rel, ld):
    eg, et = C.c_void_p(), C.c_void_p()
    check(lib().oea_step_entity_scratch(_p(workspace), int(n_ent), int(n_rel), int(ld), C.byref(eg), C.byref(et)))
    dt = scratch_dtype()
    off = et.value - workspace.data_ptr()
    return workspace[off: off + dt.itemsize * int(n_ent)].view(dt)


def step_normal_views(workspace, n_ent, n_rel, ld):
    g_off, t_off = C.c_int64(0), C.c_int64(0)
    check(lib().oea_step_normal_scratch(int(n_ent), int(n_rel), int(ld), C.byref(g_off), C.byref(t_off)))
    dt = scratch_dtype()
    grad = workspace[g_off.value: g_off.value + dt.itemsize * n_rel * ld].view(dt)
    touched = workspace[t_off.value: t_off.value + dt.itemsize * n_rel].view(dt)
    return grad, touched


def step_apply_normals(n_ent, n_rel, ld, cfg, workspace):
    check(lib().oea_step_apply_normals(int(n_ent), int(n_rel), int(ld), C.byref(cfg), _p(workspace), _stream()))


def profile_begin(stride=1):
    check(lib().oea_profile_begin(int(stride)))


def profile_end(group=4):
    ms = (C.c_double * (group - 1))()
    n = C.c_int32(0)
    check(lib().oea_profile_end(group, ms, C.byref(n)))
    return [float(x) for x in ms], int(n.value)




def tripleset_build(triples):
    n = triples.shape[0]
    if n:
        mx = triples.max(dim=0).values.cpu()
        if int(mx[0]) >= 1 << 24 or int(mx[2]) >= 1 << 24 or int(mx[1]) >= 1 << 16 or int(triples.min().item()) < 0:
            raise OpenEAHipError("triple ids out of range for the packed membership keys "
                                 "(entity ids < 16,777,216, relation ids < 65,536)")
    cap = lib().oea_tripleset_capacity(n)
    table = torch.empty(cap, dtype=torch.int64, device=triples.device)
    check(lib().oea_tripleset_build(_p(triples), n, _p(table), cap, _stream()))
    return table


def sample_negatives(pos, k, table, entity_list, ent_pos=None, nbr=None, seed=0, step=0,
                     pos_offset=0, max_try=10, out=None, err_flag=None):
    n_pos = pos.shape[0]
    if out is None:
        out = torch.empty((n_pos * k, 3), dtype=torch.int32, device=pos.device)
    if err_flag is None:
        err_flag = torch.zeros(1, dtype=torch.int32, device=pos.device)
    nbr_k = 0 if nbr is None else nbr.shape[1]
    check(lib().oea_sample_negatives(_p(pos), n_pos, k, _p(table), table.numel(), _p(entity_list),
                                     entity_list.numel(), _p(ent_pos), _p(nbr), nbr_k, int(seed),
                                     int(step), int(pos_offset), int(max_try), _p(out), _p(err_flag),
                                     _stream()))
    return out, err_flag


def sample_negatives_replay(pos, k, table, entity_list, replay, ent_pos=None, nbr=None, max_try=10):
    n_pos = pos.shape[0]
    out = torch.zeros((n_pos * k, 3), dtype=torch.int32, device=pos.device)
    err_flag = torch.zeros(1, dtype=torch.int32, device=pos.device)
    nbr_k = 0 if nbr is None else nbr.shape[1]
    assert tuple(replay.shape) == (n_pos, max_try, 1 + k) and replay.dtype == torch.int32 and replay.is_contiguous()
    check(lib().oea_sample_negatives_replay(_p(pos), n_pos, k, _p(table), table.numel(), _p(entity_list), entity_list.numel(),
                                            _p(ent_pos), _p(nbr), nbr_k, int(max_try), _p(replay), _p(out), _p(err_flag), _stream()))
    return out, err_flag


def tripleset_filter(triples, capacity):
    bits = int(lib().oea_tripleset_filter_bits(int(capacity)))
    filt = torch.empty(bits // 32, dtype=torch.int32, device=triples.device)
    check(lib().oea_tripleset_filter_build(_p(triples), triples.shape[0], _p(filt), bits, _stream()))
    return filt


def sampler_side(table, entity_list, ent_pos, nbr, filt=None):
    side = _lib.SamplerSide(table.data_ptr(), table.numel(), entity_list.data_ptr(),
                            ent_pos.data_ptr() if ent_pos is not None else None,
                            nbr.data_ptr() if nbr is not None else None, entity_list.numel(),
                            0 if nbr is None else nbr.shape[1],
                            filt.data_ptr() if filt is not None else None, 0 if filt is None else 32 * filt.numel())
    side._keep = (table, entity_list, ent_pos, nbr, filt)
    return side


def sample_negatives_pair(pos, n_split, k, side0, side1, seed, step, pos_offset, out, err_flag, max_try=10):
    check(lib().oea_sample_negatives_pair(_p(pos), pos.shape[0], int(n_split), k, C.byref(side0), C.byref(side1),
                                          int(seed), int(step), int(pos_offset), int(max_try), _p(out), _p(err_flag),
                                          _stream()))
    return out


def sample_negatives_epoch(pos_all, offsets_dev, splits_dev, steps, k, side0, side1, seed, step_base, out, err_flag, max_try=10):
    check(lib().oea_sample_negatives_epoch(_p(pos_all), pos_all.shape[0], _p(offsets_dev), _p(splits_dev), int(steps), int(k),
                                           C.byref(side0), C.byref(side1), int(seed), int(step_base), int(max_try), _p(out),
                                           _p(err_flag), _stream()))
    return out


def triple_epoch(ent, ent_acc, rel, rel_acc, dim, pos_all, offsets, splits, k, side0, side1, seed, step_base,
                 neg_buf, err_flag, cfg, workspace, loss_accum, offsets_dev=None, splits_dev=None, step_range=None, shard=(0, 1),
                 plan=None):
    steps = len(splits)
    lo, hi = (0, steps) if step_range is None else step_range
    if plan is not None and tuple(shard) == (0, 1):
        check(lib().oea_triple_epoch_range_plan(_p(ent), _p(ent_acc), ent.shape[0], _p(rel), _p(rel_acc), rel.shape[0], dim,
                                                ent.shape[1], _p(pos_all), offsets.ctypes.data_as(C.c_void_p),
                                                splits.ctypes.data_as(C.c_void_p), steps, int(lo), int(hi), int(k),
                                                C.byref(side0) if side0 is not None else None,
                                                C.byref(side1) if side1 is not None else None, int(seed), int(step_base),
                                                _p(neg_buf), _p(err_flag), C.byref(cfg), _p(workspace), _p(loss_accum),
                                                _p(offsets_dev), _p(splits_dev), _p(plan[0]), plan[0].numel(), int(bool(plan[1])),
                                                _stream()))
        return
    check(lib().oea_triple_epoch_range_shard(_p(ent), _p(ent_acc), ent.shape[0], _p(rel), _p(rel_acc), rel.shape[0], dim,
                                       ent.shape[1], _p(pos_all), offsets.ctypes.data_as(C.c_void_p),
                                       splits.ctypes.data_as(C.c_void_p), steps, int(lo), int(hi), int(k),
                                       C.byref(side0) if side0 is not None else None,
                                       C.byref(side1) if side1 is not None else None, int(seed), int(step_base),
                                       _p(neg_buf), _p(err_flag), C.byref(cfg), _p(workspace), _p(loss_accum),
                                       _p(offsets_dev), _p(splits_dev), int(shard[0]), int(shard[1]), _stream()))


def epoch_layout(triples, n1, n2, slot, seed, epoch, dall, workspace=None):
    n = int(n1) + int(n2)
    if workspace is None:
        workspace = torch.empty(lib().oea_epoch_layout_bytes(n), dtype=torch.uint8, device=triples.device)
    check(lib().oea_epoch_layout(_p(triples), int(n1), int(n2), _p(slot), slot.numel(), int(seed) & 0xFFFFFFFFFFFFFFFF, int(epoch) & 0xFFFFFFFF,
                                 _p(dall), _p(workspace), workspace.numel(), _stream()))
    return workspace


def step_plan_supported(cfg, n_ent, n_rel, ld, k):
    return bool(lib().oea_step_plan_supported(C.byref(cfg), int(n_ent), int(n_rel), int(ld), int(k)))


def step_plan_buffer(n_total, steps, max_batch, n_ent, ld, dev=None):
    nbytes = lib().oea_step_plan_bytes(int(n_total), int(steps), int(max_batch), int(n_ent), int(ld))
    return torch.empty(nbytes, dtype=torch.uint8, device=dev or device())


def step_plan_build(pos_all, neg_all, k, offsets_dev, n_total, steps, max_batch, n_ent, ld, plan):
    check(lib().oea_step_plan_build(_p(pos_all), _p(neg_all), int(k), _p(offsets_dev), int(n_total), int(steps), int(max_batch),
                                    int(n_ent), int(ld), _p(plan), plan.numel(), _stream()))


def step_plan_arrays(plan, n_total, steps, max_batch, n_ent, ld):
    off = (C.c_int64 * 9)()
    check(lib().oea_step_plan_offsets(int(n_total), int(steps), int(max_batch), int(n_ent), int(ld), C.cast(off, C.c_void_p)))
    raw = plan.cpu().numpy()
    m = 2 * int(n_total)
    nu = int(raw[off[3]: off[3] + 4].view(np.int32)[0])
    return dict(vals=raw[off[0]: off[0] + 4 * m].view(np.uint32).copy(), ukeys=raw[off[1]: off[1] + 8 * nu].view(np.uint64).copy(),
                uoff=raw[off[2]: off[2] + 4 * (nu + 1)].view(np.uint32).copy(),
                step_first=raw[off[4]: off[4] + 4 * (steps + 1)].view(np.int32).copy(), row_bits=int(off[6]), n_unique=nu,
                pflags=raw[off[8]: off[8] + 4 * int(n_total)].view(np.uint32).copy())


def step_plan_rel_order(plan, n_total, steps, max_batch, n_ent, ld):
    off = C.c_int64(0)
    check(lib().oea_step_plan_rel_order_offset(int(n_total), int(steps), int(max_batch), int(n_ent), int(ld), C.cast(C.byref(off), C.c_void_p)))
    n = int(n_total)
    return plan[off.value: off.value + 4 * n].cpu().numpy().view(np.uint32).copy()


def step_plan_stats(plan, n_total, steps, max_batch, n_ent, ld):
    a = step_plan_arrays(plan, n_total, steps, max_batch, n_ent, ld)
    last = int(a["step_first"][steps])
    cnt = np.diff(a["uoff"].astype(np.int64))[:last]
    listed = int(a["uoff"][last])
    hub = cnt > 8
    return dict(positives=int(n_total), outside_rule=int(n_total - listed // 2), rows_per_step=float(last) / max(steps, 1),
                refs_per_row_mean=float(cnt.mean()) if last else 0.0, refs_per_row_max=int(cnt.max()) if last else 0,
                hub_rows_per_step=float(hub.sum()) / max(steps, 1), refs_to_hub_rows=int(cnt[hub].sum()),
                refs_listed=listed)


def comm_single_or_none():
    uid = (C.c_char * 128)()
    check(lib().oea_comm_unique_id(uid))
    comm = C.c_void_p()
    check(lib().oea_comm_init(uid, 0, 1, C.byref(comm)))
    return comm


def part_buffers(n_ent, n_rel, ld, world, dev, adagrad=True):
    rpr = lib().oea_part_rows_per_rank(int(n_ent), int(world))
    chunk = rpr * (ld + 1)
    f = dict(dtype=torch.float32, device=dev)
    g = dict(dtype=scratch_dtype(), device=dev)
    return dict(rpr=rpr, chunk=chunk, send=torch.empty(world * chunk, **g), own=torch.empty(chunk, **g),
                rel_x=torch.empty(n_rel * (ld + 1), **g), upd=torch.empty((rpr, ld), **f), all=torch.empty((world, rpr, ld), **f),
                acc_own=torch.full((rpr, ld), 0.1, **f) if adagrad else None)


def triple_epoch_comm(comm, ent, acc_own, rel, rel_acc, dim, pos_all, offsets, splits, k, side0, side1, seed, step_base, neg_buf,
                      err_flag, cfg, workspace, loss_accum, offsets_dev, splits_dev, bufs, step_range=None):
    offsets, splits = np.ascontiguousarray(offsets, np.int64), np.ascontiguousarray(splits, np.int64)
    steps = len(splits)
    lo, hi = (0, steps) if step_range is None else step_range
    check(lib().oea_triple_epoch_range_comm(comm, _p(ent), _p(acc_own), ent.shape[0], _p(rel), _p(rel_acc), rel.shape[0], dim,
                                            ent.shape[1], _p(pos_all), offsets.ctypes.data_as(C.c_void_p),
                                            splits.ctypes.data_as(C.c_void_p), steps, int(lo), int(hi), int(k),
                                            C.byref(side0) if side0 is not None else None,
                                            C.byref(side1) if side1 is not None else None, int(seed), int(step_base),
                                            _p(neg_buf), _p(err_flag), C.byref(cfg), _p(workspace), _p(loss_accum),
                                            _p(offsets_dev), _p(splits_dev), _p(bufs['send']), _p(bufs['own']), _p(bufs['rel_x']),
                                            _p(bufs['upd']), _p(bufs['all']), _stream()))


def halo_buffers(n_ent, ld, world, steps, max_batch, k, dev):
    wsb = lib().oea_halo_workspace_bytes(int(n_ent), int(world), int(steps), int(max_batch), int(k))
    xb = lib().oea_halo_buffer_bytes(int(n_ent), int(world), int(max_batch), int(k), int(ld))
    u8 = dict(dtype=torch.uint8, device=dev)
    return dict(ws=torch.empty(wsb, **u8), a=torch.empty(xb, **u8), b=torch.empty(xb, **u8), key=(int(steps), int(max_batch), int(k)))


def halo_plan(pos_all, neg_all, k, offsets, n_ent, world, step_range=None, with_lists=True):
    offsets = np.ascontiguousarray(offsets, np.int64)
    steps = len(offsets) - 1
    lo, hi = (0, steps) if step_range is None else step_range
    max_batch = int(np.diff(offsets).max()) if steps else 0
    dev = pos_all.device
    ws = torch.empty(lib().oea_halo_workspace_bytes(int(n_ent), int(world), hi - lo, max_batch, int(k)), dtype=torch.uint8, device=dev)
    off_dev = torch.from_numpy(offsets).to(dev)
    counts = np.zeros((hi - lo, world, world), np.int32)
    cap = C.c_int64(0)
    check(lib().oea_halo_plan(_p(pos_all), _p(neg_all), int(k), offsets.ctypes.data_as(C.c_void_p), _p(off_dev), steps, int(lo), int(hi),
                              int(n_ent), int(world), _p(ws), ws.numel(), counts.ctypes.data_as(C.c_void_p), None, C.byref(cap), _stream()))
    lists = None
    if with_lists:
        lists = np.zeros((hi - lo, world, int(cap.value)), np.int32)
        check(lib().oea_halo_plan(_p(pos_all), _p(neg_all), int(k), offsets.ctypes.data_as(C.c_void_p), _p(off_dev), steps, int(lo), int(hi),
                                  int(n_ent), int(world), _p(ws), ws.numel(), counts.ctypes.data_as(C.c_void_p),
                                  lists.ctypes.data_as(C.c_void_p), C.byref(cap), _stream()))
    return counts, lists


def triple_epoch_halo(comm, ent, acc_own, rel, rel_acc, dim, pos_all, offsets, splits, k, side0, side1, seed, step_base, neg_buf,
                      err_flag, cfg, workspace, loss_accum, offsets_dev, splits_dev, bufs, halo, step_range=None):
    offsets, splits = np.ascontiguousarray(offsets, np.int64), np.ascontiguousarray(splits, np.int64)
    steps = len(splits)
    lo, hi = (0, steps) if step_range is None else step_range
    stats = (C.c_int64 * 4)()
    check(lib().oea_triple_epoch_range_halo(comm, _p(ent), _p(acc_own), ent.shape[0], _p(rel), _p(rel_acc), rel.shape[0], dim,
                                            ent.shape[1], _p(pos_all), offsets.ctypes.data_as(C.c_void_p),
                                            splits.ctypes.data_as(C.c_void_p), steps, int(lo), int(hi), int(k),
                                            C.byref(side0) if side0 is not None else None,
                                            C.byref(side1) if side1 is not None else None, int(seed), int(step_base),
                                            _p(neg_buf), _p(err_flag), C.byref(cfg), _p(workspace), _p(loss_accum),
                                            _p(offsets_dev), _p(splits_dev), _p(halo['ws']), halo['ws'].numel(), _p(halo['a']),
                                            _p(halo['b']), halo['a'].numel(), _p(bufs['rel_x']), _p(bufs['upd']), _p(bufs['all']),
                                            C.cast(stats, C.c_void_p), _stream()))
    return tuple(int(x) for x in stats)


def sample_link_negatives(n_pos, k, pos_links=None, ents1=None, ents2=None, nbr1=None, row1=None, nbr2=None, row2=None,
                          exclude=None, seed=0, step=0, scratch=None):
    truncated = nbr1 is not None
    m = (2 if truncated else 1) * k * n_pos
    dev = (nbr1 if truncated else ents1).device
    pairs = torch.empty((m, 2), dtype=torch.int32, device=dev)
    valid = torch.empty(m, dtype=torch.float32, device=dev)
    cap = 2
    while cap < 2 * max(m, 1):
        cap *= 2
    if scratch is None or scratch[0].numel() < cap:
        scratch = (torch.empty(cap, dtype=torch.int64, device=dev), torch.empty(cap, dtype=torch.int32, device=dev))
    check(lib().oea_sample_link_negatives(_p(pos_links), n_pos, k, _p(ents1), 0 if ents1 is None else ents1.numel(),
                                          _p(ents2), 0 if ents2 is None else ents2.numel(), _p(nbr1), _p(row1), _p(nbr2),
                                          _p(row2), nbr1.shape[1] if truncated else 0, _p(exclude),
                                          0 if exclude is None else exclude.numel(), int(seed), int(step), _p(pairs),
                                          _p(valid), _p(scratch[0]), _p(scratch[1]), cap, _stream()))
    return pairs, valid, scratch


def greedy_matching(left, right, weight):
    left = np.ascontiguousarray(left, np.int32)
    right = np.ascontiguousarray(right, np.int32)
    weight = np.ascontiguousarray(weight, np.float32)
    sel = np.zeros(len(left), np.uint8)
    check(_lib.load(require_device=False).oea_greedy_matching(left.ctypes.data_as(C.c_void_p), right.ctypes.data_as(C.c_void_p),
                                                              weight.ctypes.data_as(C.c_void_p), len(left),
                                                              sel.ctypes.data_as(C.c_void_p)))
    return sel.astype(bool)


def pair_dots(e1, e2, dim, ii, jj):
    out = torch.empty(ii.numel(), dtype=torch.float32, device=e1.device)
    check(lib().oea_pair_dots(_p(e1), e1.shape[1], _p(e2), e2.shape[1], dim, _p(ii), _p(jj), ii.numel(), _p(out), _stream()))
    return out




def topk_inner(q, c, dim, k, id_map=None, ws_bytes=None):
    nq, nc = q.shape[0], c.shape[0]
# ... 677 lines not shown
```

Before: 279.3 million triples/s.

## Fuse step-plan key emission into negative sampler and use 32-bit sort keys

The negative sampler kernel now optionally emits step-plan sort keys, values and flags directly while it draws negatives. This removes the separate plan_emit pass that re-read all sampled negatives. The plan build also gains a 32-bit key mode when row and step bits fit, which shortens the radix sort. The sampler pays for this with extra shuffles and stores, and the work happens on the prefetch side stream.

```diff
diff --git a/include/openea_hip.h b/include/openea_hip.h
--- a/include/openea_hip.h
+++ b/include/openea_hip.h
@@ -182,6 +182,10 @@
                                const int64_t *splits_dev, int32_t steps, int32_t k, const oea_sampler_side *side0,
                                const oea_sampler_side *side1, uint64_t seed, uint32_t step_base, int32_t max_try,
                                int32_t *out_all, int32_t *err_flag, void *stream);
+int oea_sample_negatives_epoch_plan(const int32_t *pos_all, int64_t n_rows, const int64_t *offsets_dev, const int64_t *splits_dev,
+                                    int32_t steps, int32_t k, const oea_sampler_side *side0, const oea_sampler_side *side1, uint64_t seed,
+                                    uint32_t step_base, int32_t max_try, int32_t *out_all, int32_t *err_flag, int64_t max_batch,
+                                    int64_t n_ent, int32_t ld, void *plan, size_t plan_bytes, void *stream);
 
 int oea_triple_epoch(float *ent, float *ent_acc, int64_t n_ent, float *rel, float *rel_acc, int64_t n_rel,
                      int32_t dim, int32_t ld, const int32_t *pos_all, const int64_t *offsets_host,
@@ -205,6 +209,10 @@
 size_t oea_step_plan_bytes(int64_t n_total, int32_t steps, int64_t max_batch, int64_t n_ent, int32_t ld);
 int oea_step_plan_build(const int32_t *pos_all, const int32_t *neg_all, int32_t k, const int64_t *offsets_dev, int64_t n_total,
                         int32_t steps, int64_t max_batch, int64_t n_ent, int32_t ld, void *plan, size_t plan_bytes, void *stream);
+int oea_step_plan_build_emitted(const int32_t *pos_all, const int64_t *offsets_dev, int64_t n_total, int32_t steps, int64_t max_batch,
+                                int64_t n_ent, int32_t ld, void *plan, size_t plan_bytes, void *stream);
+int32_t oea_step_plan_fused_emit(void);
+int oea_step_plan_emit_offsets(int64_t n_total, int32_t steps, int64_t max_batch, int64_t n_ent, int32_t ld, int64_t *out);
 int oea_step_plan_offsets(int64_t n_total, int32_t steps, int64_t max_batch, int64_t n_ent, int32_t ld, int64_t *out);
 int oea_step_plan_rel_order_offset(int64_t n_total, int32_t steps, int64_t max_batch, int64_t n_ent, int32_t ld, int64_t *out);
 int oea_triple_epoch_range_plan(float *ent, float *ent_acc, int64_t n_ent, float *rel, float *rel_acc, int64_t n_rel,
diff --git a/openea_amd/_lib.py b/openea_amd/_lib.py
--- a/openea_amd/_lib.py
+++ b/openea_amd/_lib.py
@@ -117,6 +117,8 @@
                                             _u64, _u32, _u32, _i32, _vp, _vp, _vp]),
     "oea_sample_negatives_epoch": (C.c_int, [_vp, _i64, _vp, _vp, _i32, _i32, C.POINTER(SamplerSide),
                                              C.POINTER(SamplerSide), _u64, _u32, _i32, _vp, _vp, _vp]),
+    "oea_sample_negatives_epoch_plan": (C.c_int, [_vp, _i64, _vp, _vp, _i32, _i32, C.POINTER(SamplerSide), C.POINTER(SamplerSide), _u64, _u32,
+                                                  _i32, _vp, _vp, _i64, _i64, _i32, _vp, _sz, _vp]),
     "oea_triple_epoch": (C.c_int, [_vp, _vp, _i64, _vp, _vp, _i64, _i32, _i32, _vp, _vp, _vp, _i32, _i32,
                                    C.POINTER(SamplerSide), C.POINTER(SamplerSide), _u64, _u32, _vp, _vp,
                                    C.POINTER(StepCfg), _vp, _vp, _vp, _vp, _vp]),
@@ -133,6 +135,9 @@
     "oea_step_plan_offsets": (C.c_int, [_i64, _i32, _i64, _i64, _i32, _vp]),
     "oea_step_plan_rel_order_offset": (C.c_int, [_i64, _i32, _i64, _i64, _i32, _vp]),
     "oea_step_plan_build": (C.c_int, [_vp, _vp, _i32, _vp, _i64, _i32, _i64, _i64, _i32, _vp, _sz, _vp]),
+    "oea_step_plan_build_emitted": (C.c_int, [_vp, _vp, _i64, _i32, _i64, _i64, _i32, _vp, _sz, _vp]),
+    "oea_step_plan_fused_emit": (_i32, []),
+    "oea_step_plan_emit_offsets": (C.c_int, [_i64, _i32, _i64, _i64, _i32, _vp]),
     "oea_triple_epoch_range_plan": (C.c_int, [_vp, _vp, _i64, _vp, _vp, _i64, _i32, _i32, _vp, _vp, _vp, _i32, _i32, _i32, _i32,
                                         C.POINTER(SamplerSide), C.POINTER(SamplerSide), _u64, _u32, _vp, _vp,
                                         C.POINTER(StepCfg), _vp, _vp, _vp, _vp, _vp, _sz, _i32, _vp]),
diff --git a/openea_amd/csrc/sampler.hip b/openea_amd/csrc/sampler.hip
--- a/openea_amd/csrc/sampler.hip
+++ b/openea_amd/csrc/sampler.hip
@@ -3,6 +3,7 @@
 #include <algorithm>
 
 #include "common.h"
+#include "step_plan.h"
 
 namespace {
 
@@ -50,12 +51,13 @@
 
 constexpr int kMaxK = 64;
 
-template <int G>
+template <int G, bool PLAN>
 __global__ __launch_bounds__(256) void sample_negatives_kernel(
     const int32_t *__restrict__ pos, int64_t n_pos, int64_t n_split, int k, oea_sampler_side side0,
     oea_sampler_side side1, uint32_t k0, uint32_t k1, uint32_t step, uint32_t pos_offset,
     int max_try, int32_t *__restrict__ out, int32_t *__restrict__ err_flag,
-    const int64_t *__restrict__ seg_off, const int64_t *__restrict__ seg_split, int n_seg, const int32_t *__restrict__ replay) {
+    const int64_t *__restrict__ seg_off, const int64_t *__restrict__ seg_split, int n_seg, const int32_t *__restrict__ replay,
+    oea::PlanEmitTarget plan) {
     const int lane = threadIdx.x % G;
     const uint32_t step_in = step;
     const int64_t n_split_in = n_split;
@@ -63,6 +65,7 @@
     step = step_in;
     n_split = n_split_in;
     int64_t pl = p;
+    int seg = 0;
     if (seg_off) {
         const int64_t p0 = ((int64_t)(uint32_t)__builtin_amdgcn_readfirstlane((int)(p >> 32)) << 32) | (uint32_t)__builtin_amdgcn_readfirstlane((int)p);
         int lo = 0, hi = n_seg;
@@ -71,7 +74,7 @@
             if (seg_off[mid] <= p0) lo = mid; else hi = mid;
         }
         int64_t first = seg_off[lo], split = seg_split[lo];
-        int seg = lo;
+        seg = lo;
         if (p >= seg_off[lo + 1]) {
             int l2 = lo;
             hi = n_seg;
@@ -103,6 +106,7 @@
     const int gbase = (threadIdx.x & 63) / G * G;
     const unsigned long long gmask = (G == 64 ? ~0ull : ((1ull << G) - 1ull)) << gbase;
     int got = 0;
+    uint32_t xh = 0u, xt = 0u;
     for (int tr = 0; tr < max_try && got < k; ++tr) {
         const bool spare = k < G;
         uint4 w = oea::philox4x32_10(c0, step, (uint32_t)tr, (spare && lane != G - 1) ? 1u + (uint32_t)lane : 0u, k0, k1);
@@ -148,8 +152,16 @@
             const int slot = got + __popcll(acc_mask & ((1ull << lane) - 1ull));
             struct __attribute__((packed, aligned(4))) Triple { int32_t h, r, t; };
             *reinterpret_cast<Triple *>(out + ((int64_t)p * k + slot) * 3) = Triple{nh, r, nt};
+            if (PLAN) { xh |= (uint32_t)(nh ^ h); xt |= (uint32_t)(nt ^ t); }
         }
         got += __popcll(acc_mask);
+    }
+    if (PLAN) {
+#pragma unroll
+        for (int o = G / 2; o > 0; o >>= 1) { xh |= (uint32_t)__shfl_xor((int)xh, o, 64); xt |= (uint32_t)__shfl_xor((int)xt, o, 64); }
+        if (lane == 0)
+            oea::plan_emit_store(plan.keys, plan.vals, plan.pflags, plan.key32, p, (uint32_t)pl, seg, plan.steps, plan.row_bits, h, t,
+                                 xh != 0u && xt != 0u, xh == 0u);
     }
     }
 }
@@ -209,7 +221,7 @@
                        const oea_sampler_side *side0, const oea_sampler_side *side1, uint64_t seed,
                        uint32_t step, uint32_t pos_offset, int32_t max_try, int32_t *out,
                        int32_t *err_flag, const int64_t *seg_off_dev, const int64_t *seg_split_dev, int n_seg,
-                       void *stream, const int32_t *replay = nullptr) {
+                       void *stream, const int32_t *replay = nullptr, const oea::PlanEmitTarget *plan = nullptr) {
     OEA_REQUIRE(pos && out && err_flag, "null pointer");
     OEA_REQUIRE(k >= 1 && k <= kMaxK, "1 <= k <= 64");
     OEA_REQUIRE(max_try >= 1, "max_try >= 1");
@@ -222,14 +234,12 @@
     hipStream_t st = oea::as_stream(stream);
     static const int64_t cap_env = [] { const char *e = getenv("OEA_SAMPLER_CAP"); return e ? (int64_t)atoll(e) : (int64_t)0; }();
     const int64_t cap = (seg_off_dev && cap_env > 0) ? cap_env : ((int64_t)1 << 30);
-    if (k <= 16)
-        sample_negatives_kernel<16><<<(unsigned)std::min<int64_t>(oea::ceil_div(n_pos, 256 / 16), cap), 256, 0, st>>>(
-            pos, n_pos, n_split, k, *side0, *side1, (uint32_t)seed, (uint32_t)(seed >> 32), step, pos_offset, max_try,
-            out, err_flag, seg_off_dev, seg_split_dev, n_seg, replay);
-    else
-        sample_negatives_kernel<64><<<(unsigned)std::min<int64_t>(oea::ceil_div(n_pos, 256 / 64), cap), 256, 0, st>>>(
-            pos, n_pos, n_split, k, *side0, *side1, (uint32_t)seed, (uint32_t)(seed >> 32), step, pos_offset, max_try,
-            out, err_flag, seg_off_dev, seg_split_dev, n_seg, replay);
+#define OEA_SAMPLE(G, PLAN) sample_negatives_kernel<G, PLAN><<<(unsigned)std::min<int64_t>(oea::ceil_div(n_pos, 256 / G), cap), 256, 0, st>>>( \
+        pos, n_pos, n_split, k, *side0, *side1, (uint32_t)seed, (uint32_t)(seed >> 32), step, pos_offset, max_try, out, err_flag, seg_off_dev, \
+        seg_split_dev, n_seg, replay, plan ? *plan : oea::PlanEmitTarget{})
+    if (plan) { if (k <= 16) OEA_SAMPLE(16, true); else OEA_SAMPLE(64, true); }
+    else { if (k <= 16) OEA_SAMPLE(16, false); else OEA_SAMPLE(64, false); }
+#undef OEA_SAMPLE
     OEA_CHECK_HIP(hipGetLastError());
     return OEA_OK;
 }
@@ -261,4 +271,19 @@
                        splits_dev, steps, stream);
 }
 
-}
+int oea_sample_negatives_epoch_plan(const int32_t *pos_all, int64_t n_rows, const int64_t *offsets_dev, const int64_t *splits_dev,
+                                    int32_t steps, int32_t k, const oea_sampler_side *side0, const oea_sampler_side *side1, uint64_t seed,
+                                    uint32_t step_base, int32_t max_try, int32_t *out_all, int32_t *err_flag, int64_t max_batch,
+                                    int64_t n_ent, int32_t ld, void *plan, size_t plan_bytes, void *stream) {
+    OEA_REQUIRE(offsets_dev && splits_dev && steps >= 1, "offsets / splits / steps");
+    OEA_REQUIRE(plan && n_rows >= 0 && max_batch >= 0 && n_ent > 0 && ld > 0, "plan workspace and its sizes");
+    OEA_REQUIRE(2 * n_rows < ((int64_t)1 << 31) && 2 * max_batch < ((int64_t)1 << 31), "entries and slots are 31-bit");
+    oea::StepPlanView v;
+    const size_t need = oea::step_plan_layout(n_rows, steps, max_batch, n_ent, ld, plan, &v);
+    OEA_REQUIRE(plan_bytes >= need, "plan workspace smaller than oea_step_plan_bytes");
+    const oea::PlanEmitTarget target{v.keys_a, v.vals_a, v.pflags, v.key32, steps, v.row_bits};
+    return sample_impl(pos_all, n_rows, 0, k, side0, side1, seed, step_base, 0u, max_try, out_all, err_flag, offsets_dev, splits_dev, steps,
+                       stream, nullptr, &target);
+}
+
+}
diff --git a/openea_amd/csrc/step_plan.h b/openea_amd/csrc/step_plan.h
--- a/openea_amd/csrc/step_plan.h
+++ b/openea_amd/csrc/step_plan.h
@@ -21,10 +21,29 @@
     size_t temp_bytes;
     uint32_t *rel_order;
     int row_bits;
+    int key32;
 };
 
 constexpr uint32_t kPlanHubEntries = 8;
 
 size_t step_plan_layout(int64_t n_total, int32_t steps, int64_t max_batch, int64_t n_ent, int32_t ld, void *base, StepPlanView *v);
 
+__device__ __forceinline__ void plan_emit_store(void *keys, uint32_t *vals, uint32_t *pflags, int key32, int64_t p, uint32_t pl, int step,
+                                                int steps, int row_bits, int32_t h, int32_t t, bool outside, bool tails) {
+    const uint64_t sk = (uint64_t)(outside ? steps : step) << row_bits;
+    const uint64_t kh = outside ? sk : sk | (uint64_t)(uint32_t)h, kt = outside ? sk : sk | (uint64_t)(uint32_t)t;
+    if (key32) *reinterpret_cast<uint2 *>(static_cast<uint32_t *>(keys) + 2 * p) = make_uint2((uint32_t)kh, (uint32_t)kt);
+    else *reinterpret_cast<ulonglong2 *>(static_cast<uint64_t *>(keys) + 2 * p) = make_ulonglong2(kh, kt);
+    const uint32_t vh = outside ? 0u : 2u * pl + (tails ? 0u : 1u);
+    const uint32_t vt = outside ? 0u : 0x80000000u | (2u * pl + (tails ? 1u : 0u));
+    *reinterpret_cast<uint2 *>(vals + 2 * p) = make_uint2(vh, vt);
+    pflags[p] = 0u;
 }
+
+struct PlanEmitTarget {
+    void *keys;
+    uint32_t *vals, *pflags;
+    int key32, steps, row_bits;
+};
+
+}
diff --git a/openea_amd/csrc/step_plan.hip b/openea_amd/csrc/step_plan.hip
--- a/openea_amd/csrc/step_plan.hip
+++ b/openea_amd/csrc/step_plan.hip
@@ -1,3 +1,4 @@
+#include <stdlib.h>
 #include <string.h>
 
 #include <rocprim/rocprim.hpp>
@@ -11,6 +12,30 @@
 
 static size_t al256(size_t x) { return (x + 255) / 256 * 256; }
 static int bits_for(uint64_t max_value) { int b = 1; while (b < 64 && (max_value >> b) != 0) ++b; return b; }
+static bool env_on(const char *name) { const char *e = getenv(name); return !(e && atoi(e) == 0); }
+
+using PlanSortConfig = rocprim::radix_sort_config<rocprim::default_config, rocprim::default_config, rocprim::default_config, 0>;
+
+template <typename K>
+struct PlanHeadFlag {
+    const K *keys;
+    __host__ __device__ uint32_t operator()(uint32_t e) const { return (e == 0u || keys[e] != keys[e - 1u]) ? 1u : 0u; }
+};
+template <typename K>
+static hipError_t plan_rank_heads(void *temp, size_t &temp_bytes, const K *keys, uint32_t *rank, size_t m, hipStream_t st) {
+    return rocprim::inclusive_scan(temp, temp_bytes, rocprim::make_transform_iterator(rocprim::make_counting_iterator(0u), PlanHeadFlag<K>{keys}),
+                                   rank, m, rocprim::plus<uint32_t>(), st);
+}
+template <typename K>
+static size_t plan_temp_bytes(size_t m) {
+    size_t t1 = 0, t2 = 0, t3 = 0, t4 = 0;
+    (void)rocprim::radix_sort_pairs<PlanSortConfig>(nullptr, t1, (const K *)nullptr, (K *)nullptr, (const uint32_t *)nullptr, (uint32_t *)nullptr, m, 0,
+                                                    8 * sizeof(K), (hipStream_t)0);
+    (void)rocprim::run_length_encode(nullptr, t2, (const K *)nullptr, m, (K *)nullptr, (uint32_t *)nullptr, (int32_t *)nullptr, (hipStream_t)0);
+    (void)rocprim::exclusive_scan(nullptr, t3, (const uint32_t *)nullptr, (uint32_t *)nullptr, 0u, m + 1, rocprim::plus<uint32_t>(), (hipStream_t)0);
+    (void)plan_rank_heads<K>(nullptr, t4, nullptr, nullptr, m, (hipStream_t)0);
+    return std::max(std::max(t1, t2), std::max(t3, t4));
+}
 
 size_t step_plan_layout(int64_t n_total, int32_t steps, int64_t max_batch, int64_t n_ent, int32_t ld, void *base, StepPlanView *v) {
     const size_t m = (size_t)std::max<int64_t>(2 * n_total, 1);
@@ -31,18 +56,13 @@
     w.recs = (uint4 *)take(16 * m);
     w.inplan = (uint8_t *)take((size_t)std::max<int32_t>(steps, 1) * (size_t)n_ent);
     w.contrib = (float *)take(sizeof(float) * 2 * (size_t)std::max<int64_t>(max_batch, 1) * (size_t)ld);
-    size_t t1 = 0, t2 = 0, t3 = 0;
-    (void)rocprim::radix_sort_pairs(nullptr, t1, (const uint64_t *)nullptr, (uint64_t *)nullptr, (const uint32_t *)nullptr,
-                                    (uint32_t *)nullptr, m, 0, 64, (hipStream_t)0);
-    (void)rocprim::run_length_encode(nullptr, t2, (const uint64_t *)nullptr, m, (uint64_t *)nullptr, (uint32_t *)nullptr,
-                                     (int32_t *)nullptr, (hipStream_t)0);
-    (void)rocprim::exclusive_scan(nullptr, t3, (const uint32_t *)nullptr, (uint32_t *)nullptr, 0u, m + 1, rocprim::plus<uint32_t>(),
-                                  (hipStream_t)0);
     const size_t n1 = (size_t)std::max<int64_t>(n_total, 1);
-    w.temp_bytes = std::max(std::max(t1, std::max(t2, t3)), al256(4 * n1)) + 256;
+    w.temp_bytes = std::max(std::max(plan_temp_bytes<uint64_t>(m), plan_temp_bytes<uint32_t>(m)), al256(4 * n1)) + 256;
     w.temp = take(w.temp_bytes);
     w.rel_order = (uint32_t *)take(4 * n1);
     w.row_bits = bits_for((uint64_t)std::max<int64_t>(n_ent - 1, 1));
+    static const bool key32_on = env_on("OEA_PLAN_KEY32");
+    w.key32 = key32_on && w.row_bits + bits_for((uint64_t)steps) <= 32;
     if (v) *v = w;
     return off;
 }
@@ -50,8 +70,8 @@
 namespace {
 
 __global__ void plan_emit_kernel(const int32_t *__restrict__ pos_all, const int32_t *__restrict__ neg_all, int k,
-                                 const int64_t *__restrict__ offsets, int steps, int64_t n_total, int row_bits,
-                                 uint64_t *__restrict__ keys, uint32_t *__restrict__ vals) {
+                                 const int64_t *__restrict__ offsets, int steps, int64_t n_total, int row_bits, int key32,
+                                 void *__restrict__ keys, uint32_t *__restrict__ vals, uint32_t *__restrict__ pflags) {
     const int64_t p = (int64_t)blockIdx.x * blockDim.x + threadIdx.x;
     if (p >= n_total) return;
     int lo = 0, hi = steps;
@@ -69,29 +89,21 @@
         xh |= a;
         xt |= b;
     }
-    if (bad | min(xh, xt)) {
-        keys[2 * p] = keys[2 * p + 1] = (uint64_t)steps << row_bits;
-        vals[2 * p] = vals[2 * p + 1] = 0u;
-        return;
-    }
-    const bool tails = xh == 0;
-    const uint64_t sk = (uint64_t)lo << row_bits;
-    keys[2 * p] = sk | (uint64_t)(uint32_t)h;
-    vals[2 * p] = 2u * pl + (tails ? 0u : 1u);
-    keys[2 * p + 1] = sk | (uint64_t)(uint32_t)t;
-    vals[2 * p + 1] = 0x80000000u | (2u * pl + (tails ? 1u : 0u));
-}
-
-constexpr int kRelSortWaves = 8, kRelDigitBits = 10, kRelBins = 1 << kRelDigitBits, kRelAhead = 8;
+    plan_emit_store(keys, vals, pflags, key32, p, pl, lo, steps, row_bits, h, t, (bad | min(xh, xt)) != 0u, xh == 0u);
+}
+
+constexpr int kRelSortWaves = 16, kRelDigitBits = 10, kRelBins = 1 << kRelDigitBits, kRelAhead = 8, kRelCacheEntries = 20480;
 __global__ __launch_bounds__(kRelSortWaves * 64) void plan_rel_order_kernel(const int32_t *__restrict__ pos_all, const int64_t *__restrict__ offsets,
-                                                                            uint32_t *__restrict__ tmp, uint32_t *__restrict__ rel_order) {
+                                                                            uint32_t *__restrict__ tmp, uint32_t *__restrict__ rel_order, int cache) {
     __shared__ uint32_t hist[kRelSortWaves][kRelBins];
+    __shared__ uint16_t dig[kRelCacheEntries];
     __shared__ uint32_t dbase[kRelBins];
     __shared__ uint32_t wsum[kRelSortWaves];
     __shared__ uint32_t rmax;
     const int64_t first = offsets[blockIdx.x];
     const uint32_t n = (uint32_t)(offsets[blockIdx.x + 1] - first);
     if (n == 0) return;
+    const bool cached = cache != 0 && n <= (uint32_t)kRelCacheEntries;
     const int32_t *rel = pos_all + 3 * first + 1;
     const uint32_t t = threadIdx.x, lane = t & 63u, w = t >> 6;
     const uint32_t slice = (n + kRelSortWaves - 1) / kRelSortWaves, c0 = min(w * slice, n), c1 = min(c0 + slice, n);
@@ -114,8 +126,10 @@
 #pragma unroll
             for (int u = 0; u < kRelAhead; ++u)
                 if (c0 + (g0 + u) * 64u + lane < c1) {
+                    const uint32_t d = (r[u] >> shift) & (kRelBins - 1);
                     m = max(m, r[u]);
-                    atomicAdd(&hist[w][(r[u] >> shift) & (kRelBins - 1)], 1u);
+                    atomicAdd(&hist[w][d], 1u);
+                    if (cached) dig[c0 + (g0 + u) * 64u + lane] = (uint16_t)d;
                 }
         }
         if (pass == 0) {
@@ -151,7 +165,7 @@
             for (int u = 0; u < kRelAhead; ++u) {
                 const uint32_t i = c0 + (g0 + u) * 64u + lane;
                 idx[u] = i < c1 ? (src ? src[i] : i) : 0u;
-                dg[u] = i < c1 ? ((uint32_t)rel[3 * (int64_t)idx[u]] >> shift) & (kRelBins - 1) : 0u;
+                dg[u] = i >= c1 ? 0u : cached ? (uint32_t)dig[i] : ((uint32_t)rel[3 * (int64_t)idx[u]] >> shift) & (kRelBins - 1);
             }
 #pragma unroll
             for (int u = 0; u < kRelAhead; ++u) {
@@ -180,11 +194,12 @@
     }
 }
 
-__global__ void plan_step_first_kernel(const uint64_t *__restrict__ ukeys, const int32_t *__restrict__ n_unique, int steps, int row_bits,
+template <typename K>
+__global__ void plan_step_first_kernel(const K *__restrict__ ukeys, const int32_t *__restrict__ n_unique, int steps, int row_bits,
                                        int32_t *__restrict__ step_first) {
     const int s = blockIdx.x * blockDim.x + threadIdx.x;
     if (s > steps) return;
-    const uint64_t key = (uint64_t)s << row_bits;
+    const K key = (K)((uint64_t)s << row_bits);
     int lo = 0, hi = *n_unique;
     while (lo < hi) {
         const int mid = (lo + hi) >> 1;
@@ -193,12 +208,14 @@
     step_first[s] = lo;
 }
 
-__global__ void plan_records_kernel(const uint64_t *__restrict__ ukeys, const uint32_t *__restrict__ uoff, const uint32_t *__restrict__ vals,
+template <typename K>
+__global__ void plan_records_kernel(const K *uk, uint64_t *ukeys, const uint32_t *__restrict__ uoff, const uint32_t *__restrict__ vals,
                                     const int32_t *__restrict__ n_unique, int steps, int row_bits, int64_t n_ent, uint4 *__restrict__ recs,
                                     uint8_t *__restrict__ inplan) {
     const int nu = *n_unique;
     for (int64_t i = (int64_t)blockIdx.x * blockDim.x + threadIdx.x; i < nu; i += (int64_t)gridDim.x * blockDim.x) {
-        const uint64_t key = ukeys[i];
+        const uint64_t key = uk[i];
+        if (sizeof(K) != sizeof(uint64_t)) ukeys[i] = key;
         const uint32_t row = (uint32_t)(key & (((uint64_t)1 << row_bits) - 1)), e0 = uoff[i], cnt = uoff[i + 1] - e0;
         recs[i] = make_uint4(row, e0, cnt, vals[e0]);
         const int64_t step = (int64_t)(key >> row_bits);
@@ -206,17 +223,55 @@
     }
 }
 
-__global__ void plan_hub_kernel(const uint64_t *__restrict__ keys, const uint32_t *__restrict__ vals, int64_t m,
+template <typename K>
+__global__ void plan_hub_kernel(const K *__restrict__ keys, const uint32_t *__restrict__ vals, int64_t m,
                                 const int64_t *__restrict__ offsets, int steps, int row_bits, uint32_t *__restrict__ pflags) {
     const int64_t e = (int64_t)blockIdx.x * blockDim.x + threadIdx.x;
     if (e >= m) return;
-    const uint64_t key = keys[e];
-    const int64_t step = (int64_t)(key >> row_bits);
+    const K key = keys[e];
+    const int64_t step = (int64_t)((uint64_t)key >> row_bits);
     if (step >= steps) return;
     int left = 0, right = 0;
     while (left < (int)kPlanHubEntries && e - left - 1 >= 0 && keys[e - left - 1] == key) ++left;
     while (left + right < (int)kPlanHubEntries && e + right + 1 < m && keys[e + right + 1] == key) ++right;
     if (left + right < (int)kPlanHubEntries) return;
+    const uint32_t v = vals[e];
+    atomicOr(&pflags[offsets[step] + ((v & 0x7fffffffu) >> 1)], (v >> 31) ? 2u : 1u);
+}
+
+template <typename K>
+__global__ void plan_finish_kernel(const K *__restrict__ keys, const uint32_t *__restrict__ vals, const uint32_t *__restrict__ rank, int64_t m,
+                                   const int64_t *__restrict__ offsets, int steps, int row_bits, int64_t n_ent, uint64_t *__restrict__ ukeys,
+                                   uint32_t *__restrict__ uoff, int32_t *__restrict__ n_unique, int32_t *__restrict__ step_first,
+                                   uint4 *__restrict__ recs, uint8_t *__restrict__ inplan, uint32_t *__restrict__ pflags) {
+    const int64_t e = (int64_t)blockIdx.x * blockDim.x + threadIdx.x;
+    if (e >= m) return;
+    constexpr int H = (int)kPlanHubEntries;
+    const K key = keys[e];
+    const K prev = e > 0 ? keys[e - 1] : key;
+    const bool head = e == 0 || prev != key;
+    const int64_t step = (int64_t)((uint64_t)key >> row_bits);
+    const uint32_t u = rank[e] - 1u;
+    int right = 0;
+    while (right < H && e + right + 1 < m && keys[e + right + 1] == key) ++right;
+    if (head) {
+        const uint32_t row = (uint32_t)((uint64_t)key & (((uint64_t)1 << row_bits) - 1)), cnt = (uint32_t)right + 1u;
+        ukeys[u] = (uint64_t)key;
+        uoff[u] = (uint32_t)e;
+        recs[u] = make_uint4(row, (uint32_t)e, cnt, vals[e]);
+        if (step < steps && cnt <= kPlanHubEntries) inplan[step * n_ent + row] = 1;
+        const int64_t before = e == 0 ? -1 : (int64_t)((uint64_t)prev >> row_bits);
+        for (int64_t s = before + 1; s <= step; ++s) step_first[s] = (int32_t)u;
+    }
+    if (e == m - 1) {
+        *n_unique = (int32_t)(u + 1u);
+        uoff[u + 1u] = (uint32_t)m;
+        for (int64_t s = step + 1; s <= steps; ++s) step_first[s] = (int32_t)(u + 1u);
+    }
+    if (step >= steps) return;
+    int left = 0;
+    if (!head) while (left + right < H && e - left - 1 >= 0 && keys[e - left - 1] == key) ++left;
+    if (left + right < H) return;
     const uint32_t v = vals[e];
     atomicOr(&pflags[offsets[step] + ((v & 0x7fffffffu) >> 1)], (v >> 31) ? 2u : 1u);
 }
@@ -303,41 +358,93 @@
     return OEA_OK;
 }
 
-int oea_step_plan_build(const int32_t *pos_all, const int32_t *neg_all, int32_t k, const int64_t *offsets_dev, int64_t n_total,
-                        int32_t steps, int64_t max_batch, int64_t n_ent, int32_t ld, void *plan, size_t plan_bytes, void *stream) {
-    OEA_REQUIRE(pos_all && offsets_dev && plan && (neg_all || k == 0), "null pointer");
+}
+
+namespace oea {
+namespace {
+
+template <typename K>
+int plan_sort_and_finish(const StepPlanView &v, const int64_t *offsets_dev, int64_t n_total, int32_t steps, int64_t n_ent, hipStream_t st) {
+    const size_t m = (size_t)(2 * n_total);
+    const K *keys_a = reinterpret_cast<const K *>(v.keys_a);
+    K *keys_b = reinterpret_cast<K *>(v.keys_b);
+    const int end_bit = std::min<int>(8 * sizeof(K), v.row_bits + bits_for((uint64_t)steps));
+    size_t tb = v.temp_bytes;
+    OEA_CHECK_HIP(rocprim::radix_sort_pairs<PlanSortConfig>(v.temp, tb, keys_a, keys_b, (const uint32_t *)v.vals_a, v.vals_b, m, 0, (unsigned)end_bit, st));
+    OEA_CHECK_HIP(hipMemsetAsync(v.inplan, 0, (size_t)steps * (size_t)n_ent, st));
+    static const bool onepass = env_on("OEA_PLAN_ONEPASS");
+    if (onepass) {
+        tb = v.temp_bytes;
+        OEA_CHECK_HIP(plan_rank_heads<K>(v.temp, tb, keys_b, v.ucount, m, st));
+        plan_finish_kernel<K><<<(unsigned)ceil_div((int64_t)m, 256), 256, 0, st>>>(keys_b, v.vals_b, v.ucount, (int64_t)m, offsets_dev, steps, v.row_bits, n_ent,
+                                                                                  v.ukeys, v.uoff, v.n_unique, v.step_first, v.recs, v.inplan, v.pflags);
+        OEA_CHECK_HIP(hipGetLastError());
+        return OEA_OK;
+    }
+    K *uk = sizeof(K) == sizeof(uint64_t) ? reinterpret_cast<K *>(v.ukeys) : reinterpret_cast<K *>(v.keys_a);
+    OEA_CHECK_HIP(hipMemsetAsync(v.ucount, 0, sizeof(uint32_t) * (m + 1), st));
+    tb = v.temp_bytes;
+    OEA_CHECK_HIP(rocprim::run_length_encode(v.temp, tb, (const K *)keys_b, m, uk, v.ucount, v.n_unique, st));
+    tb = v.temp_bytes;
+    OEA_CHECK_HIP(rocprim::exclusive_scan(v.temp, tb, (const uint32_t *)v.ucount, v.uoff, 0u, m + 1, rocprim::plus<uint32_t>(), st));
+    plan_step_first_kernel<K><<<(unsigned)ceil_div(steps + 1, 256), 256, 0, st>>>(uk, v.n_unique, steps, v.row_bits, v.step_first);
+    plan_records_kernel<K><<<(unsigned)std::min<int64_t>(ceil_div((int64_t)m, 256), 4096), 256, 0, st>>>(
+        uk, v.ukeys, v.uoff, v.vals_b, v.n_unique, steps, v.row_bits, n_ent, v.recs, v.inplan);
+    plan_hub_kernel<K><<<(unsigned)ceil_div((int64_t)m, 256), 256, 0, st>>>(keys_b, v.vals_b, (int64_t)m, offsets_dev, steps, v.row_bits, v.pflags);
+    OEA_CHECK_HIP(hipGetLastError());
+    return OEA_OK;
+}
+
+int plan_build_impl(const int32_t *pos_all, const int32_t *neg_all, bool emitted, int32_t k, const int64_t *offsets_dev, int64_t n_total,
+                    int32_t steps, int64_t max_batch, int64_t n_ent, int32_t ld, void *plan, size_t plan_bytes, void *stream) {
+    OEA_REQUIRE(pos_all && offsets_dev && plan && (emitted || neg_all || k == 0), "null pointer");
     OEA_REQUIRE(n_total >= 0 && steps >= 1 && k >= 0 && n_ent > 0 && ld > 0, "sizes");
     OEA_REQUIRE(2 * n_total < ((int64_t)1 << 31) && 2 * max_batch < ((int64_t)1 << 31), "entries and slots are 31-bit");
-    oea::StepPlanView v;
-    const size_t need = oea::step_plan_layout(n_total, steps, max_batch, n_ent, ld, plan, &v);
+    StepPlanView v;
+    const size_t need = step_plan_layout(n_total, steps, max_batch, n_ent, ld, plan, &v);
     OEA_REQUIRE(plan_bytes >= need, "plan workspace smaller than oea_step_plan_bytes");
-    hipStream_t st = oea::as_stream(stream);
-    const size_t m = (size_t)(2 * n_total);
-    if (m == 0) {
+    hipStream_t st = as_stream(stream);
+    if (n_total == 0) {
         OEA_CHECK_HIP(hipMemsetAsync(v.n_unique, 0, sizeof(int32_t), st));
         OEA_CHECK_HIP(hipMemsetAsync(v.step_first, 0, sizeof(int32_t) * ((size_t)steps + 1), st));
         return OEA_OK;
     }
-    oea::plan_rel_order_kernel<<<(unsigned)steps, oea::kRelSortWaves * 64, 0, st>>>(pos_all, offsets_dev, (uint32_t *)v.temp, v.rel_order);
-    oea::plan_emit_kernel<<<(unsigned)oea::ceil_div(n_total, 256), 256, 0, st>>>(pos_all, neg_all, k, offsets_dev, steps, n_total, v.row_bits,
-                                                                                 v.keys_a, v.vals_a);
-    const int end_bit = std::min(64, v.row_bits + oea::bits_for((uint64_t)steps));
-    size_t tb = v.temp_bytes;
-    OEA_CHECK_HIP(rocprim::radix_sort_pairs(v.temp, tb, (const uint64_t *)v.keys_a, v.keys_b, (const uint32_t *)v.vals_a, v.vals_b, m, 0,
-                                            (unsigned)end_bit, st));
-    OEA_CHECK_HIP(hipMemsetAsync(v.ucount, 0, sizeof(uint32_t) * (m + 1), st));
-    tb = v.temp_bytes;
-    OEA_CHECK_HIP(rocprim::run_length_encode(v.temp, tb, (const uint64_t *)v.keys_b, m, v.ukeys, v.ucount, v.n_unique, st));
-    tb = v.temp_bytes;
-    OEA_CHECK_HIP(rocprim::exclusive_scan(v.temp, tb, (const uint32_t *)v.ucount, v.uoff, 0u, m + 1, rocprim::plus<uint32_t>(), st));
-    oea::plan_step_first_kernel<<<(unsigned)oea::ceil_div(steps + 1, 256), 256, 0, st>>>(v.ukeys, v.n_unique, steps, v.row_bits, v.step_first);
-    OEA_CHECK_HIP(hipMemsetAsync(v.pflags, 0, sizeof(uint32_t) * (size_t)n_total, st));
-    OEA_CHECK_HIP(hipMemsetAsync(v.inplan, 0, (size_t)steps * (size_t)n_ent, st));
-    oea::plan_records_kernel<<<(unsigned)std::min<int64_t>(oea::ceil_div((int64_t)m, 256), 4096), 256, 0, st>>>(
-        v.ukeys, v.uoff, v.vals_b, v.n_unique, steps, v.row_bits, n_ent, v.recs, v.inplan);
-    oea::plan_hub_kernel<<<(unsigned)oea::ceil_div((int64_t)m, 256), 256, 0, st>>>(v.keys_b, v.vals_b, (int64_t)m, offsets_dev, steps, v.row_bits,
-                                                                                   v.pflags);
+    static const int rel_cache = env_on("OEA_PLAN_REL_LDS") ? 1 : 0;
+    plan_rel_order_kernel<<<(unsigned)steps, kRelSortWaves * 64, 0, st>>>(pos_all, offsets_dev, (uint32_t *)v.temp, v.rel_order, rel_cache);
+    if (!emitted)
+        plan_emit_kernel<<<(unsigned)ceil_div(n_total, 256), 256, 0, st>>>(pos_all, neg_all, k, offsets_dev, steps, n_total, v.row_bits, v.key32,
+                                                                           v.keys_a, v.vals_a, v.pflags);
     OEA_CHECK_HIP(hipGetLastError());
+    return v.key32 ? plan_sort_and_finish<uint32_t>(v, offsets_dev, n_total, steps, n_ent, st)
+                   : plan_sort_and_finish<uint64_t>(v, offsets_dev, n_total, steps, n_ent, st);
+}
+
+}
+}
+
+extern "C" {
+
+int oea_step_plan_build(const int32_t *pos_all, const int32_t *neg_all, int32_t k, const int64_t *offsets_dev, int64_t n_total,
+                        int32_t steps, int64_t max_batch, int64_t n_ent, int32_t ld, void *plan, size_t plan_bytes, void *stream) {
+    return oea::plan_build_impl(pos_all, neg_all, false, k, offsets_dev, n_total, steps, max_batch, n_ent, ld, plan, plan_bytes, stream);
+}
+
+int oea_step_plan_build_emitted(const int32_t *pos_all, const int64_t *offsets_dev, int64_t n_total, int32_t steps, int64_t max_batch,
+                                int64_t n_ent, int32_t ld, void *plan, size_t plan_bytes, void *stream) {
+    return oea::plan_build_impl(pos_all, nullptr, true, 0, offsets_dev, n_total, steps, max_batch, n_ent, ld, plan, plan_bytes, stream);
+}
+
+int32_t oea_step_plan_fused_emit(void) {
+    static const bool on = oea::env_on("OEA_PLAN_FUSED_EMIT");
+    return on ? 1 : 0;
+}
+
+int oea_step_plan_emit_offsets(int64_t n_total, int32_t steps, int64_t max_batch, int64_t n_ent, int32_t ld, int64_t *out) {
+    OEA_REQUIRE(out && n_total >= 0 && steps >= 0 && n_ent > 0 && ld > 0, "arguments");
+    oea::StepPlanView v;
+    char *base = reinterpret_cast<char *>(4096);
+    (void)oea::step_plan_layout(n_total, steps, max_batch, n_ent, ld, base, &v);
+    out[0] = (char *)v.keys_a - base; out[1] = (char *)v.vals_a - base; out[2] = v.key32;
     return OEA_OK;
 }
 
diff --git a/openea_amd/csrc/triple_step.hip b/openea_amd/csrc/triple_step.hip
--- a/openea_amd/csrc/triple_step.hip
+++ b/openea_amd/csrc/triple_step.hip
@@ -2294,21 +2294,26 @@
     OEA_REQUIRE(k == 0 || (neg_buf && (presampled || (err_flag && side0 && side1))), "sampling needs neg_buf, err_flag and both sides");
     const bool ahead = k > 0 && offsets_dev != nullptr && steps > 0;
     const bool sample_all = ahead && !presampled && step_begin == 0;
-    if (sample_all) {
-        const int rc = oea_sample_negatives_epoch(pos_all, offsets_host[steps], offsets_dev, splits_dev, steps, k, side0,
-                                                  side1, seed, step_base, 10, neg_buf, err_flag, stream);
-        if (rc != OEA_OK) return rc;
-    }
     oea::StepPlanView pv;
     const bool use_plan = plan && world == 1 && ahead && (presampled || sample_all) && oea_step_plan_supported(cfg, n_ent, n_rel, ld, k);
+    int64_t max_batch = 0;
+    for (int32_t s = 0; s < steps; ++s) max_batch = std::max(max_batch, offsets_host[s + 1] - offsets_host[s]);
+    const bool fused_emit = sample_all && use_plan && !plan_built && oea_step_plan_fused_emit();
+    if (sample_all) {
+        const int rc = fused_emit ? oea_sample_negatives_epoch_plan(pos_all, offsets_host[steps], offsets_dev, splits_dev, steps, k, side0, side1, seed,
+                                                                    step_base, 10, neg_buf, err_flag, max_batch, n_ent, ld, plan, plan_bytes, stream)
+                                  : oea_sample_negatives_epoch(pos_all, offsets_host[steps], offsets_dev, splits_dev, steps, k, side0,
+                                                               side1, seed, step_base, 10, neg_buf, err_flag, stream);
+        if (rc != OEA_OK) return rc;
+    }
     if (use_plan) {
-        int64_t max_batch = 0;
-        for (int32_t s = 0; s < steps; ++s) max_batch = std::max(max_batch, offsets_host[s + 1] - offsets_host[s]);
         const size_t need = oea::step_plan_layout(offsets_host[steps], steps, max_batch, n_ent, ld, plan, &pv);
         OEA_REQUIRE(plan_bytes >= need, "plan workspace smaller than oea_step_plan_bytes");
         if (!plan_built) {
-            const int rc = oea_step_plan_build(pos_all, neg_buf, k, offsets_dev, offsets_host[steps], steps, max_batch, n_ent, ld, plan,
-                                               plan_bytes, stream);
+            const int rc = fused_emit ? oea_step_plan_build_emitted(pos_all, offsets_dev, offsets_host[steps], steps, max_batch, n_ent, ld, plan,
+                                                                    plan_bytes, stream)
+                                      : oea_step_plan_build(pos_all, neg_buf, k, offsets_dev, offsets_host[steps], steps, max_batch, n_ent, ld,
+                                                            plan, plan_bytes, stream);
             if (rc != OEA_OK) return rc;
         }
     }
diff --git a/openea_amd/models/trainer.py b/openea_amd/models/trainer.py
--- a/openea_amd/models/trainer.py
+++ b/openea_amd/models/trainer.py
@@ -469,16 +469,22 @@
         side.wait_event(ev_start)
         with torch.cuda.stream(side):
             self.batches.shuffle(self.gen, into_next=True)
-            if self.k:
-                ops.sample_negatives_epoch(self.batches.dall_next, self._off_dev, self._spl_dev, len(self.batches.splits), self.k,
-                                           self._sides[0], self._sides[1], self.seed, next_base, self._neg_next, self.err)
-            planned = False
-            if (self.k and trainer is not None and self.world == 1 and not getattr(trainer, "local_epochs", False)
-                    and getattr(trainer, "part", None) is None and self._plan_wanted(trainer)):
+            planned = bool(self.k and trainer is not None and self.world == 1 and not getattr(trainer, "local_epochs", False)
+                           and getattr(trainer, "part", None) is None and self._plan_wanted(trainer))
+            if planned and ops.step_plan_fused_emit():
                 n_total, steps, mb, n_ent, ld = self._plan_dims
-                ops.step_plan_build(self.batches.dall_next, self._neg_next, self.k, self._off_dev, n_total, steps, mb, n_ent, ld,
-                                    self._plan_next)
-                planned = True
+                ops.sample_negatives_epoch_plan(self.batches.dall_next, self._off_dev, self._spl_dev, steps, self.k, self._sides[0],
+                                                self._sides[1], self.seed, next_base, self._neg_next, self.err, mb, n_ent, ld,
+                                                self._plan_next)
+                ops.step_plan_build_emitted(self.batches.dall_next, self._off_dev, n_total, steps, mb, n_ent, ld, self._plan_next)
+            else:
+                if self.k:
+                    ops.sample_negatives_epoch(self.batches.dall_next, self._off_dev, self._spl_dev, len(self.batches.splits), self.k,
+                                               self._sides[0], self._sides[1], self.seed, next_base, self._neg_next, self.err)
+                if planned:
+                    n_total, steps, mb, n_ent, ld = self._plan_dims
+                    ops.step_plan_build(self.batches.dall_next, self._neg_next, self.k, self._off_dev, n_total, steps, mb, n_ent, ld,
+                                        self._plan_next)
             self._prefetch_ev = torch.cuda.Event()
             self._prefetch_ev.record(side)
         self._prefetch = (self._sides, next_base, planned)
diff --git a/openea_amd/ops.py b/openea_amd/ops.py
--- a/openea_amd/ops.py
+++ b/openea_amd/ops.py
@@ -378,6 +378,14 @@
     check(lib().oea_sample_negatives_epoch(_p(pos_all), pos_all.shape[0], _p(offsets_dev), _p(splits_dev), int(steps), int(k),
                                            C.byref(side0), C.byref(side1), int(seed), int(step_base), int(max_try), _p(out),
                                            _p(err_flag), _stream()))
+    return out
+
+
+def sample_negatives_epoch_plan(pos_all, offsets_dev, splits_dev, steps, k, side0, side1, seed, step_base, out, err_flag, max_batch, n_ent,
+                                ld, plan, max_try=10):
+    check(lib().oea_sample_negatives_epoch_plan(_p(pos_all), pos_all.shape[0], _p(offsets_dev), _p(splits_dev), int(steps), int(k),
+                                                C.byref(side0), C.byref(side1), int(seed), int(step_base), int(max_try), _p(out),
+                                                _p(err_flag), int(max_batch), int(n_ent), int(ld), _p(plan), plan.numel(), _stream()))
     return out
 
 
@@ -426,6 +434,36 @@
 def step_plan_build(pos_all, neg_all, k, offsets_dev, n_total, steps, max_batch, n_ent, ld, plan):
     check(lib().oea_step_plan_build(_p(pos_all), _p(neg_all), int(k), _p(offsets_dev), int(n_total), int(steps), int(max_batch),
                                     int(n_ent), int(ld), _p(plan), plan.numel(), _stream()))
+
+
+def step_plan_build_emitted(pos_all, offsets_dev, n_total, steps, max_batch, n_ent, ld, plan):
+    check(lib().oea_step_plan_build_emitted(_p(pos_all), _p(offsets_dev), int(n_total), int(steps), int(max_batch), int(n_ent), int(ld),
+                                            _p(plan), plan.numel(), _stream()))
+
+
+def step_plan_fused_emit():
+    return bool(lib().oea_step_plan_fused_emit())
+
+
+def step_plan_emitted(plan, n_total, steps, max_batch, n_ent, ld):
+    off = (C.c_int64 * 3)()
+    check(lib().oea_step_plan_emit_offsets(int(n_total), int(steps), int(max_batch), int(n_ent), int(ld), C.cast(off, C.c_void_p)))
+    m = 2 * int(n_total)
+    kb = 4 if off[2] else 8
+    keys = plan[off[0]: off[0] + kb * m].cpu().numpy().view(np.uint32 if off[2] else np.uint64).astype(np.uint64)
+    return dict(keys=keys, vals=plan[off[1]: off[1] + 4 * m].cpu().numpy().view(np.uint32).copy(), key32=bool(off[2]))
+
+
+def step_plan_records(plan, n_total, steps, max_batch, n_ent, ld):
+    off = (C.c_int64 * 9)()
+    check(lib().oea_step_plan_offsets(int(n_total), int(steps), int(max_batch), int(n_ent), int(ld), C.cast(off, C.c_void_p)))
+    al = lambda x: (x + 255) // 256 * 256
+    m = max(2 * int(n_total), 1)
+    r0 = off[8] + al(4 * max(int(n_total), 1))
+    i0 = r0 + al(16 * m)
+    nu = int(plan[off[3]: off[3] + 4].cpu().numpy().view(np.int32)[0])
+    return dict(recs=plan[r0: r0 + 16 * nu].cpu().numpy().view(np.uint32).reshape(nu, 4).copy(),
+                inplan=plan[i0: i0 + int(steps) * int(n_ent)].cpu().numpy().reshape(int(steps), int(n_ent)).copy())
 
 
 def step_plan_arrays(plan, n_total, steps, max_batch, n_ent, ld):
```

After: 283.1 million triples/s (median of 6 runs). 1.01x the previous value.
